# mprib/caliscope

Hardware: NVIDIA H100
Metric: lm_iterations_per_sec (higher is better)
Workload: dtype f64

## Files before the change

caliscope_b200/_lib.py:

```python
from __future__ import annotations

import ctypes as C
import os
from pathlib import Path

PKG_DIR = Path(__file__).resolve().parent
LIB_NAME = "libcaliscope_b200.so"

CB_CAM_FREE_INTRINSICS = 1
CB_CAM_FISHEYE = 2
LOSS_IDS = {"linear": 0, "soft_l1": 1, "huber": 2, "cauchy": 3, "arctan": 4}


class EngineUnavailable(RuntimeError):
    """libcaliscope_b200.so is missing / unloadable, or no CUDA device is usable."""


class EngineError(RuntimeError):
    def __init__(self, code: int, what: str, detail: str):
        super().__init__(f"{what} failed: {detail} (code {code})")
        self.code = code


class ProblemDesc(C.Structure):
    _fields_ = [
        ("n_cams", C.c_int32),
        ("n_pts", C.c_int32),
        ("n_obs", C.c_int64),
        ("cam_flags", C.c_void_p),
        ("cam_const", C.c_void_p),
        ("obs_cam", C.c_void_p),
        ("obs_pt", C.c_void_p),
        ("obs_xy", C.c_void_p),
        ("obs_on_device", C.c_int32),
        ("obs_cam_bits", C.c_int32),
        ("cam_order", C.c_void_p),
        ("n_constraints", C.c_int64),
        ("groups_a", C.c_void_p),
        ("groups_b", C.c_void_p),
        ("distances", C.c_void_p),
        ("weights", C.c_void_p),
    ]


ALLREDUCE_FN = C.CFUNCTYPE(C.c_int, C.c_void_p, C.c_void_p, C.c_int64, C.c_void_p)


class Options(C.Structure):
    _fields_ = [
        ("ftol", C.c_double),
        ("xtol", C.c_double),
        ("gtol", C.c_double),
        ("max_nfev", C.c_int64),
        ("loss", C.c_int32),
        ("f_scale", C.c_double),
        ("verbose", C.c_int32),
        ("use_bounds", C.c_int32),
        ("lambda0", C.c_double),
        ("pcg_tol", C.c_double),
        ("pcg_max_iter", C.c_int32),
        ("allreduce", ALLREDUCE_FN),
        ("allreduce_user", C.c_void_p),
        ("nccl_comm", C.c_void_p),
        ("peer_group", C.c_void_p),
        ("rank", C.c_int32),
        ("world_size", C.c_int32),
        ("time_kernels", C.c_int32),
        ("pad_", C.c_int32),
    ]


class Result(C.Structure):
    _fields_ = [
        ("status", C.c_int32),
        ("nfev", C.c_int64),
        ("njev", C.c_int64),
        ("nit", C.c_int64),
        ("cost", C.c_double),
        ("initial_cost", C.c_double),
        ("optimality", C.c_double),
        ("lambda_final", C.c_double),
        ("pcg_iterations", C.c_int64),
        ("kernel_launches", C.c_int64),
        ("solve_ms", C.c_double),
        ("rj_ms", C.c_double),
        ("rj_launches", C.c_int64),
        ("syrk_ms", C.c_double),
        ("syrk_launches", C.c_int64),
        ("trials_queued", C.c_int64),
        ("used_graph", C.c_int32),
        ("pad_", C.c_int32),
    ]


class TriStats(C.Structure):
    _fields_ = [
        ("group_ms", C.c_double),
        ("dlt_ms", C.c_double),
        ("total_ms", C.c_double),
        ("kernel_launches", C.c_int32),
        ("pad_", C.c_int32),
    ]


class TriRefineStats(C.Structure):
    _fields_ = [
        ("group_ms", C.c_double),
        ("dlt_ms", C.c_double),
        ("refine_ms", C.c_double),
        ("cov_ms", C.c_double),
        ("total_ms", C.c_double),
        ("kernel_launches", C.c_int32),
        ("pad_", C.c_int32),
    ]


class TriRobustStats(C.Structure):
    _fields_ = [
        ("group_ms", C.c_double),
        ("consensus_ms", C.c_double),
        ("refine_ms", C.c_double),
        ("cov_ms", C.c_double),
        ("total_ms", C.c_double),
        ("kernel_launches", C.c_int32),
        ("pad_", C.c_int32),
    ]


class ResectStats(C.Structure):
    _fields_ = [
        ("group_ms", C.c_double),
        ("consensus_ms", C.c_double),
        ("refine_ms", C.c_double),
        ("cov_ms", C.c_double),
        ("total_ms", C.c_double),
        ("kernel_launches", C.c_int32),
        ("pad_", C.c_int32),
    ]


_P = C.c_void_p
_D = C.POINTER(C.c_double)
SYMBOLS = {
    "cb_ba_abi_version": (C.c_int, []),
    "cb_ba_error_string": (C.c_char_p, [C.c_int]),
    "cb_ba_last_error": (C.c_char_p, []),
    "cb_ba_default_options": (None, [C.POINTER(Options)]),
    "cb_ba_problem_create": (C.c_int, [C.POINTER(ProblemDesc), C.c_int, _P, C.POINTER(_P)]),
    "cb_ba_problem_destroy": (C.c_int, [_P]),
    "cb_ba_problem_n_params": (C.c_int64, [_P]),
    "cb_ba_problem_stat": (C.c_double, [_P, C.c_int]),
    "cb_ba_constraint_rows": (C.c_int, [_P, _P, _P, _P, _P]),
    "cb_ba_solve": (C.c_int, [_P, C.POINTER(Options), _P, C.POINTER(Result), _P]),
    "cb_ba_residuals": (C.c_int, [_P, _P, _P, _P]),
    "cb_ba_jacobian_blocks": (C.c_int, [_P, _P, _P, _P, _P]),
    "cb_ba_reproj_errors_px": (C.c_int, [_P, _P, _P, _P]),
    "cb_ba_cam_stride": (C.c_int, [_P]),
    "cb_ba_normal_equations": (
        C.c_int,
        [_P, _P, C.c_double, C.c_int32, C.c_double, _P, _P, _P, _P, _P, _P, _P, _P, _P, _P],
    ),
    "cb_ba_covariance": (
        C.c_int,
        [_P, _P, C.c_int32, C.c_double, C.c_int32, _P, C.c_double, _P, _P, _P, _P, _P, _P],
    ),
    "cb_ba_error_order_stats": (C.c_int, [_P, _P, C.c_double, _P, _P, _P, _P, _P]),
    "cb_ba_rmse_px": (C.c_int, [_P, _P, _P, _P, _P]),
    "cb_ba_cull": (C.c_int, [_P, _P, _P, C.c_int32, C.POINTER(_P), _P, _P, _P]),
    "cb_ba_debug_pcg_time": (C.c_int, [_P, C.c_int, C.c_int, _P, _P]),
    "cb_debug_fp64_peak": (C.c_int, [C.c_int, _P, _P]),
    "cb_shard_select": (C.c_int, [C.c_int64, _P, _P, _P, C.c_int32, C.c_int32, C.c_int64, _P, _P, _P, _P, _P, C.c_int32]),
    "cb_csv_write_numeric": (C.c_int, [C.c_char_p, C.c_char_p, C.c_int64, C.c_int32, _P, _P, C.c_int32]),
    "cb_csv_scan": (C.c_int, [C.c_char_p, _P, _P]),
    "cb_csv_parse_numeric": (C.c_int, [C.c_char_p, C.c_int64, C.c_int32, _P, _P, _P, C.c_int32]),
    "cb_pnp_ippe": (C.c_int, [C.c_int32, _P, _P, _P, C.c_int64, _P, _P, _P, _P, C.c_int32, C.c_int32, _P, _P, _P, _P, _P, _P, _P,
                              _P, C.c_int, _P]),
    "cb_stereo_rmse": (C.c_int, [C.c_int32, _P, _P, _P, C.c_int32, _P, _P, _P, C.c_int64, _P, _P, _P, C.c_int32, _P, _P, _P,
                                 C.c_int, _P]),
    "cb_relative_pose_network": (C.c_int, [C.c_int32, C.c_int32, _P, _P, _P, _P, _P, C.c_double, C.c_double, C.c_int32, _P, _P, _P, _P,
                                           _P, _P, C.c_int64, _P, _P, _P, C.c_int, _P]),
    "cb_undistort_points": (C.c_int, [C.c_int32, _P, _P, _P, C.c_int64, _P, _P, C.c_int, C.c_int, _P, C.c_int, _P]),
    "cb_triangulate_dlt": (
        C.c_int,
        [C.c_int32, _P, C.c_int64, _P, _P, _P, C.c_int, C.c_int32, C.POINTER(C.c_int32), _P, _P, _P, _P,
         C.POINTER(TriStats), C.c_int, _P],
    ),
    "cb_undistort_triangulate": (
        C.c_int,
        [C.c_int32, _P, _P, _P, _P, C.c_int64, _P, _P, _P, C.c_int, C.c_int32, C.POINTER(C.c_int32), _P, _P, _P, _P,
         C.POINTER(TriStats), C.c_int, _P],
    ),
    "cb_triangulate_refine": (
        C.c_int,
        [C.c_int32, _P, _P, _P, _P, C.c_int64, _P, _P, _P, C.c_int, C.c_double, C.c_int32, C.c_double, C.c_int32,
         C.POINTER(C.c_int32), _P, _P, _P, _P, _P, _P, C.POINTER(TriRefineStats), C.c_int, _P],
    ),
    "cb_triangulate_robust": (
        C.c_int,
        [C.c_int32, _P, _P, _P, _P, C.c_int64, _P, _P, _P, C.c_int, C.c_double, C.c_int32, C.c_int32, C.c_double,
         C.c_int32, C.c_double, C.c_int32, C.POINTER(C.c_int32), _P, _P, _P, _P, _P, _P, _P, _P,
         C.POINTER(TriRobustStats), C.c_int, _P],
    ),
    "cb_resect_robust": (
        C.c_int,
        [C.c_int32, _P, _P, _P, C.c_int32, _P, _P, C.c_int64, _P, _P, _P, _P, C.c_int, C.c_double, C.c_int32, C.c_int32,
         C.c_int32, C.c_double, C.c_int32, C.c_double, C.c_int32, C.POINTER(C.c_int32), _P, _P, _P, _P, _P, _P, _P, _P,
         _P, C.POINTER(ResectStats), C.c_int, _P],
    ),
    "cb_peer_create": (C.c_int, [C.c_int, C.c_int, C.c_int, C.c_int64, C.POINTER(_P), _P]),
    "cb_peer_connect": (C.c_int, [_P, _P]),
    "cb_peer_destroy": (C.c_int, [_P]),
    "cb_nccl_unique_id": (C.c_int, [_P]),
    "cb_nccl_comm_create": (C.c_int, [_P, C.c_int, C.c_int, C.c_int, C.POINTER(_P)]),
    "cb_nccl_comm_destroy": (C.c_int, [_P]),
    "cb_ba_launch_count": (C.c_int64, []),
}

_lib = None


def lib_path() -> Path:
    return Path(os.environ.get("CALISCOPE_B200_LIB", PKG_DIR / LIB_NAME))


def load() -> C.CDLL:
    global _lib
    if _lib is not None:
        return _lib
    path = lib_path()
    if not path.exists():
        raise EngineUnavailable(
            f"{path} not found -- build it with `python -c 'import __graft_entry__ as g; g.build()'` "
            "(nvcc, sm_90a).  caliscope_b200 has no CPU fallback."
        )
    try:
        lib = C.CDLL(str(path))
    except OSError as e:
        raise EngineUnavailable(f"cannot load {path}: {e}") from e
    for name, (res, args) in SYMBOLS.items():
        fn = getattr(lib, name)
        fn.restype = res
        fn.argtypes = args
    _lib = lib
    return lib


def check(code: int, what: str) -> None:
    if code == 0:
        return
    lib = load()
    detail = (lib.cb_ba_last_error() or b"").decode() or (lib.cb_ba_error_string(code) or b"").decode()
    if code == -3:
        raise EngineUnavailable(f"{what}: {detail}")
    raise EngineError(code, what, detail)
```

caliscope_b200/csrc/cb_engine.cu:

```cuda
#include <cuda_runtime.h>
#include <dlfcn.h>
#if defined(__x86_64__)
#include <emmintrin.h>
#endif
#include <nvtx3/nvToolsExt.h>

#include <algorithm>
#include <atomic>
#include <chrono>
#include <cmath>
#include <cstdio>
#include <cstdlib>
#include <cstring>
#include <condition_variable>
#include <cub/cub.cuh>
#include <deque>
#include <functional>
#include <map>
#include <memory>
#include <mutex>
#include <string>
#include <thread>
#include <type_traits>
#include <vector>
// ... 314 lines not shown
      std::lock_guard<std::mutex> lk(mu_);
      q_.push_back(std::move(f));
    }
    cv_.notify_one();
  }

 private:
  WorkerPool() {
    unsigned hw = std::thread::hardware_concurrency();
    int n = (int)std::min<unsigned>(hw > 2 ? hw - 1 : 1, 12u);
    for (int i = 0; i < n; ++i) {
      threads_.emplace_back([this] {
        for (;;) {
          std::function<void()> f;
          {
            std::unique_lock<std::mutex> lk(mu_);
            cv_.wait(lk, [this] { return !q_.empty(); });
            f = std::move(q_.front());
            q_.pop_front();
          }
          f();
        }
      });
      threads_.back().detach();
    }
  }
  std::mutex mu_;
  std::condition_variable cv_;
  std::deque<std::function<void()>> q_;
  std::vector<std::thread> threads_;
};

int staged_h2d(void* d_dst, const void* h_src, size_t bytes, cudaStream_t st, ScopedFree& sf, int n_threads = 6) {
  if (bytes == 0) return CB_OK;
  char* pin = nullptr;
  CB_TRY(sf.alloc_pinned(&pin, bytes));
  const size_t unit = (size_t)512 << 10, units_per_block = 8;
  const size_t n_units = (bytes + unit - 1) / unit;
  const size_t n_blocks = (n_units + units_per_block - 1) / units_per_block;
  struct Shared {
    std::atomic<size_t> next{0};
    std::vector<std::atomic<unsigned char>> done;
    explicit Shared(size_t n) : done(n) { for (auto& d : done) d.store(0, std::memory_order_relaxed); }
  };
  auto sh = std::make_shared<Shared>(n_units);
  auto copy_one = [sh, pin, h_src, bytes, unit, n_units]() -> bool {
    const size_t c = sh->next.fetch_add(1);
    if (c >= n_units) return false;
    const size_t off = c * unit, sz = std::min(unit, bytes - off);
    stream_copy((char*)pin + off, (const char*)h_src + off, sz);
    sh->done[c].store(1, std::memory_order_release);
    return true;
  };
  static const bool prof = std::getenv("CB_PROFILE_CREATE") != nullptr;
  const auto t0 = std::chrono::steady_clock::now();
  const int helpers = (int)std::min<size_t>((size_t)std::max(0, std::min(n_threads, WorkerPool::get().size())), n_units > 1 ? n_units - 1 : 0);
  for (int t = 0; t < helpers; ++t)
    WorkerPool::get().submit([copy_one] { while (copy_one()) {} });
  bool failed = false;
  double wait_ms = 0.0, issue_ms = 0.0;
  size_t own = 0;
  cudaEvent_t pe0 = nullptr, pe1 = nullptr;
  if (prof) { cudaEventCreate(&pe0); cudaEventCreate(&pe1); cudaEventRecord(pe0, st); }
  for (size_t blk = 0; blk < n_blocks; ++blk) {
    const size_t u0 = blk * units_per_block, u1 = std::min(n_units, u0 + units_per_block);
    const auto a = std::chrono::steady_clock::now();
    for (size_t c = u0; c < u1; ++c)
      while (!sh->done[c].load(std::memory_order_acquire)) {
        if (copy_one()) ++own; else std::this_thread::yield();
      }
    const auto b = std::chrono::steady_clock::now();
    const size_t off = u0 * unit, sz = std::min(bytes, u1 * unit) - off;
    if (!failed && cudaMemcpyAsync((char*)d_dst + off, (char*)pin + off, sz, cudaMemcpyHostToDevice, st) != cudaSuccess) failed = true;
    if (prof) {
      const auto e = std::chrono::steady_clock::now();
      wait_ms += std::chrono::duration<double, std::milli>(b - a).count();
      issue_ms += std::chrono::duration<double, std::milli>(e - b).count();
    }
  }
  if (prof) {
    const double host_ms = std::chrono::duration<double, std::milli>(std::chrono::steady_clock::now() - t0).count();
    cudaEventRecord(pe1, st);
    cudaEventSynchronize(pe1);
    float dma_ms = 0.f;
    cudaEventElapsedTime(&dma_ms, pe0, pe1);
    const double all_ms = std::chrono::duration<double, std::milli>(std::chrono::steady_clock::now() - t0).count();
    cudaEventDestroy(pe0); cudaEventDestroy(pe1);
    std::fprintf(stderr, "[stage] %6.1f MB, %d helpers, %zu DMA blocks: host %.3f ms (units %.3f, %zu by the issuer; cudaMemcpyAsync calls %.3f); "
                         "device first->last copy %.3f ms = %.1f GB/s; staged + landed %.3f ms\n",
                 bytes / 1e6, helpers, n_blocks, host_ms, wait_ms, own, issue_ms, dma_ms, bytes / 1e6 / std::max(dma_ms, 1e-3f), all_ms);
  }
  if (failed) { g_last_error = std::string("staged host-to-device copy: ") + cudaGetErrorString(cudaGetLastError()); return CB_E_CUDA; }
  return CB_OK;
}

int select_device(int device) {
  int ndev = 0;
  if (cudaGetDeviceCount(&ndev) != cudaSuccess || ndev == 0) {
    cudaGetLastError();
    g_last_error = "no CUDA device";
    return CB_E_NO_DEVICE;
  }
  if (device < 0 || device >= ndev) { g_last_error = "device index out of range"; return CB_E_INVALID; }
  CB_CUDA(cudaSetDevice(device));
  return CB_OK;
}

}

struct TrialGraph {
  struct Key {
    void *nccl, *peer; int rank, world;
    bool operator==(const Key& o) const { return nccl == o.nccl && peer == o.peer && rank == o.rank && world == o.world; }
  };
  cudaGraph_t graph = nullptr;
  cudaGraphExec_t exec = nullptr;
  Key key = {};
  bool valid = false, failed = false;
  int n_kernels = 0;
};

struct CbBaProblem {
  int device = 0, num_sms = 132;
  int n_cams = 0, n_pts = 0, P = 6, nP = 0, n_obs = 0, n_params = 0;
  int LD = 0, n_blk = 0, n_tiles = 0, n_split = 1, k_chunks = 0, K_pad = 0;
  int n_chunks = 0, pt_grid = 0, pt_lanes = 32, n_dups = 0;
  int cam_in_smem = 0;
  size_t pt_smem = 0, bs_smem = 0;
  std::vector<int> h_cam_off;
  std::vector<int> h_perm, h_slot;
  std::vector<int> h_iflags;
  bool order_auto = false, order_identity = true;
  int ncp = 0;
  int *d_cam_xoff = nullptr, *d_cam_slot = nullptr, *d_klist = nullptr;
  bool schur_sparse = false;
  double schur_flop_issued = 0.0;
  std::vector<void*> allocs;
  int* d_cam_flags = nullptr;
  double* d_cam_const = nullptr;
  double2 *d_cm_xy = nullptr, *d_pm_xy = nullptr;
  int *d_cm_pt = nullptr, *d_cm_orig = nullptr, *d_cam_start = nullptr;
  int *d_chunk_cam = nullptr, *d_chunk_begin = nullptr, *d_chunk_end = nullptr, *d_cam_chunk_start = nullptr;
  int *d_pt_start = nullptr, *d_pm_orig = nullptr, *d_pm_cam = nullptr, *d_pm_pt = nullptr;
  const int *d_obs_cam = nullptr, *d_obs_pt = nullptr;
  const double* d_obs_xy = nullptr;
  std::vector<int> h_cam_flags;
  std::vector<double> h_cam_const;
  int *d_tile_of = nullptr, *d_tile_slot_start = nullptr, *d_tile_slots = nullptr;
  cb::SyItem* d_items = nullptr;
  int n_items = 0, n_slots = 0;
  CUtensorMap zt_map{};
  unsigned char* d_active = nullptr;
  double *d_lo = nullptr, *d_hi = nullptr;
  double *d_x = nullptr, *d_xc[2] = {nullptr, nullptr}, *d_xp4[2] = {nullptr, nullptr};
  double *d_camtab[2] = {nullptr, nullptr}, *d_Upk[2] = {nullptr, nullptr}, *d_gc[2] = {nullptr, nullptr},
         *d_costsum[2] = {nullptr, nullptr};
  double *d_partial = nullptr, *d_camcost = nullptr, *d_V6 = nullptr, *d_gp = nullptr, *d_Dp2 = nullptr,
         *d_Dc2 = nullptr, *d_Linv6 = nullptr, *d_tvec = nullptr, *d_Zt = nullptr, *d_part = nullptr,
         *d_tpart = nullptr, *d_red = nullptr, *d_Minv = nullptr, *d_dc = nullptr, *d_dp = nullptr,
         *d_bpart = nullptr, *d_sc = nullptr, *d_red2 = nullptr, *d_out2 = nullptr;
  unsigned long long* d_gmax = nullptr;
  unsigned int* d_counter = nullptr;
  cb::LmState* d_state = nullptr;
  cb::LmState* h_state = nullptr;
  cb::LmLogRow* d_log = nullptr;
  int log_cap = 4096;
  double* h_x = nullptr;
  cudaEvent_t ev0 = nullptr, ev1 = nullptr, ev2 = nullptr, ev3 = nullptr, ev_state[2] = {nullptr, nullptr};
  cudaEvent_t ev_pp[2][4] = {{nullptr, nullptr, nullptr, nullptr}, {nullptr, nullptr, nullptr, nullptr}};
  cudaStream_t cap_stream = nullptr;
  TrialGraph trial_graph;
  TrialGraph loop_graph;
  int pcg_cs = 1, pcg_rows = 0, pcg_mode = 2, pcg_cl = 1, pcg_npa = 0;
  bool direct_solve = false;
  size_t direct_smem = 0;
  size_t pcg_smem = 0;
  int n_c = 0, n_comp = 0, n_dim_max = 0, n_cblk = 0;
  cb::ConstraintTables ct = {};
  double *d_c_rs[2] = {nullptr, nullptr}, *d_c_dirw[2] = {nullptr, nullptr}, *d_compL = nullptr, *d_gpt = nullptr;
  int* d_pt_comp = nullptr;
  size_t comp_build_smem = 0, comp_back_smem = 0;
  std::vector<int> h_ga, h_gb;
  std::vector<double> h_cdist, h_cw;
  int red_slots = 64;
  CbPeerGroup* peer = nullptr;
  int cov_n = 0;
  double *d_covA = nullptr, *d_covC = nullptr, *d_covD = nullptr, *d_covS = nullptr, *d_covDiag = nullptr,
         *d_covR = nullptr, *d_covPt = nullptr;
  int *d_covRank = nullptr, *d_covFail = nullptr;
  unsigned char* d_covFree = nullptr;
  float cov_ms[3] = {0.f, 0.f, 0.f};
  size_t red_len() const { return (size_t)nP * nP + 3 * (size_t)nP + 1 + red_slots; }
  cb::CPtr2 c_camtab() const { return {{d_camtab[0], d_camtab[1]}}; }
  cb::Ptr2 m_camtab() const { return {{d_camtab[0], d_camtab[1]}}; }
  cb::CPtr2 c_xp() const { return {{d_xp4[0], d_xp4[1]}}; }
  cb::Ptr2 m_xp() const { return {{d_xp4[0], d_xp4[1]}}; }
  cb::Ptr2 m_xc() const { return {{d_xc[0], d_xc[1]}}; }
  cb::CPtr2 c_Upk() const { return {{d_Upk[0], d_Upk[1]}}; }
  cb::Ptr2 m_Upk() const { return {{d_Upk[0], d_Upk[1]}}; }
  cb::CPtr2 c_gc() const { return {{d_gc[0], d_gc[1]}}; }
  cb::Ptr2 m_gc() const { return {{d_gc[0], d_gc[1]}}; }
  cb::CPtr2 c_costsum() const { return {{d_costsum[0], d_costsum[1]}}; }
  cb::Ptr2 m_costsum() const { return {{d_costsum[0], d_costsum[1]}}; }
  cb::CPtr2 c_crs() const { return {{d_c_rs[0], d_c_rs[1]}}; }
  cb::Ptr2 m_crs() const { return {{d_c_rs[0], d_c_rs[1]}}; }
  cb::CPtr2 c_cdirw() const { return {{d_c_dirw[0], d_c_dirw[1]}}; }
  cb::Ptr2 m_cdirw() const { return {{d_c_dirw[0], d_c_dirw[1]}}; }
};

namespace {

template <typename T>
int palloc(CbBaProblem* p, T** ptr, size_t n) {
  CB_TRY(dalloc(ptr, n));
  p->allocs.push_back((void*)*ptr);
  return CB_OK;
}

int bits_for(unsigned long long v) {
  int b = 1;
  while (b < 64 && (v >> b) != 0ull) ++b;
  return b;
}

void destroy_graph(TrialGraph& g) {
  if (g.exec) cudaGraphExecDestroy(g.exec);
  if (g.graph) cudaGraphDestroy(g.graph);
  g.exec = nullptr; g.graph = nullptr; g.valid = false; g.n_kernels = 0;
}

cudaStream_t side_stream() {
  thread_local std::map<int, cudaStream_t> streams;
  int dev = 0;
  cudaGetDevice(&dev);
  auto it = streams.find(dev);
  if (it != streams.end()) return it->second;
  cudaStream_t s = nullptr;
  cudaStreamCreateWithFlags(&s, cudaStreamNonBlocking);
  streams[dev] = s;
  return s;
}

int choose_camera_order(CbBaProblem* p, const int* cam_order, cudaStream_t st) {
  const int nc = p->n_cams;
  p->h_perm.resize(nc); p->h_slot.resize(nc);
  for (int i = 0; i < nc; ++i) p->h_perm[i] = i;
  p->order_auto = false;
  if (cam_order) {
    std::vector<char> seen(nc, 0);
    for (int i = 0; i < nc; ++i) {
      const int c = cam_order[i];
      if (c < 0 || c >= nc || seen[c]) { g_last_error = "cam_order is not a permutation of 0..n_cams-1"; return CB_E_INVALID; }
      seen[c] = 1;
      p->h_perm[i] = c;
    }
  } else {
    const int cams_per_tile = std::max(1, cb::SY_TILE / p->P);
    const double avg = (double)p->n_obs / std::max(p->n_pts, 1);
    if (p->n_blk >= 3 && avg <= nc / 3.0) {
      p->order_auto = true;
      const int stride = std::max(1, p->n_pts / 8192), ns = cdiv(p->n_pts, stride);
      unsigned int* d_W;
      ScopedFree sf(st);
      CB_TRY(sf.alloc(&d_W, (size_t)nc * nc));
      CB_CUDA(cudaMemsetAsync(d_W, 0, sizeof(unsigned int) * nc * nc, st));
      CB_LAUNCH(cb::covis_kernel, cdiv((long long)ns * 32, 256), 256, 0, st, p->d_pt_start, p->d_pm_cam, p->n_pts, stride, nc, d_W);
      std::vector<unsigned int> W((size_t)nc * nc);
      CB_CUDA(cudaMemcpyAsync(W.data(), d_W, sizeof(unsigned int) * nc * nc, cudaMemcpyDeviceToHost, st));
      CB_CUDA(cudaStreamSynchronize(st));
      std::vector<char> placed(nc, 0);
      std::vector<int> order;
      int start = 0;
      unsigned long long best = ~0ull;
      for (int c = 0; c < nc; ++c) {
        unsigned long long tot = 0;
        for (int q = 0; q < nc; ++q) if (q != c) tot += W[(size_t)c * nc + q];
        if (tot < best) { best = tot; start = c; }
      }
      order.push_back(start); placed[start] = 1;
      while ((int)order.size() < nc) {
        int pick = -1;
        unsigned long long bw = 0;
        const int lo = std::max(0, (int)order.size() - cams_per_tile);
        for (int c = 0; c < nc; ++c) {
          if (placed[c]) continue;
          unsigned long long w = 0;
          for (int k = lo; k < (int)order.size(); ++k) w += W[(size_t)c * nc + order[k]];
          if (pick < 0 || w > bw) { pick = c; bw = w; }
        }
        order.push_back(pick); placed[pick] = 1;
      }
      auto off_mass = [&](const std::vector<int>& ord) {
        std::vector<int> tile(nc);
        for (int i = 0; i < nc; ++i) tile[ord[i]] = (i * p->P) / cb::SY_TILE;
        unsigned long long m = 0;
        for (int a = 0; a < nc; ++a)
          for (int b = 0; b < nc; ++b)
            if (tile[a] != tile[b]) m += W[(size_t)a * nc + b];
        return m;
      };
      std::vector<int> ident(nc);
      for (int i = 0; i < nc; ++i) ident[i] = i;
      if (off_mass(order) < 0.8 * off_mass(ident)) p->h_perm = order;
    }
  }
  p->order_identity = true;
  for (int i = 0; i < nc; ++i) {
    p->h_slot[p->h_perm[i]] = i;
    if (p->h_perm[i] != i) p->order_identity = false;
  }
  CB_CUDA(cudaMemcpyAsync(p->d_cam_slot, p->h_slot.data(), sizeof(int) * nc, cudaMemcpyHostToDevice, st));
  return CB_OK;
}

struct XyUpload {
  bool started = false;
  std::atomic<int> finished{0};
  cudaEvent_t ev = nullptr;
  int rc = CB_OK;
  std::string err;
  ScopedFree pinned;
  void join() {
    if (!started) return;
    while (!finished.load(std::memory_order_acquire)) std::this_thread::yield();
    started = false;
  }
  int wait(cudaStream_t st) {
    join();
    if (rc != CB_OK) { g_last_error = err; return rc; }
    if (ev) CB_CUDA(cudaStreamWaitEvent(st, ev, 0));
    return CB_OK;
  }
  ~XyUpload() {
    join();
    if (ev) { cudaEventSynchronize(ev); cudaEventDestroy(ev); }
  }
};

int build_indices(CbBaProblem* p, const int* d_obs_cam, const int* d_obs_pt, const double* d_obs_xy,
                  const int* cam_order, cudaStream_t st, XyUpload* xy_upload) {
  const int n = p->n_obs;
  const int TB = 256, G = cdiv(std::max(n, 1), TB);
  ScopedFree sf(st);
  int* d_bad;
// ... 87 lines not shown
            COV ? p->d_covRank : nullptr)
#define CB_PT_PASS2(LANES, DUPS) do { if (p->cam_in_smem) CB_PT_PASS(LANES, DUPS, true); else CB_PT_PASS(LANES, DUPS, false); } while (0)
  if (p->pt_lanes == 8) { if (p->n_dups) CB_PT_PASS2(8, true); else CB_PT_PASS2(8, false); }
  else { if (p->n_dups) CB_PT_PASS2(32, true); else CB_PT_PASS2(32, false); }
#undef CB_PT_PASS2
#undef CB_PT_PASS
}

template <int P>
void launch_pt_backsub(CbBaProblem* p, double* dp_out, cudaStream_t st) {
  const int bstride = p->pt_grid + p->n_comp;
#define CB_PT_BACK(LANES, SM)                                                                                         \
  CB_LAUNCH((cb::pt_backsub_kernel<P, LANES, SM>), p->pt_grid, cb::PT_WARPS * 32, p->bs_smem, st, p->d_state,         \
            p->d_pt_start, p->d_pm_cam, p->d_pm_xy, p->d_pt_comp, p->n_pts, p->n_cams, p->nP, p->c_camtab(),           \
            p->m_xp(), p->d_dc, p->d_Linv6, p->d_tvec, p->d_gp, p->d_Dp2, dp_out, p->d_bpart, bstride)
  if (p->pt_lanes == 8) { if (p->cam_in_smem) CB_PT_BACK(8, true); else CB_PT_BACK(8, false); }
  else { if (p->cam_in_smem) CB_PT_BACK(32, true); else CB_PT_BACK(32, false); }
#undef CB_PT_BACK
}

using PcgFn = void (*)(const cb::LmState*, const double*, const double*, const double*, int, int, int, double, int,
                       double*, double*);
PcgFn pcg_fn(int mode, int P, int cl) {
  if (mode == 2) {
    if (P == 6)
      return cl == 2 ? cb::pcg_cluster_kernel<2, 6, 2> : cl == 6 ? cb::pcg_cluster_kernel<2, 6, 6>
           : cl == 12 ? cb::pcg_cluster_kernel<2, 6, 12> : cb::pcg_cluster_kernel<2, 6, 18>;
    return cl == 2 ? cb::pcg_cluster_kernel<2, 9, 2> : cl == 6 ? cb::pcg_cluster_kernel<2, 9, 6>
         : cl == 12 ? cb::pcg_cluster_kernel<2, 9, 12> : cb::pcg_cluster_kernel<2, 9, 18>;
  }
  return P == 6 ? cb::pcg_cluster_kernel<1, 6, 1> : cb::pcg_cluster_kernel<1, 9, 1>;
}

int launch_pcg(CbBaProblem* p, const cb::LmState* st_dev, double tol2, int max_iter, cudaStream_t st) {
  cudaLaunchConfig_t cfg = {};
  cfg.gridDim = dim3(p->pcg_cs);
  cfg.blockDim = dim3(cb::PCG_THREADS);
  cfg.dynamicSmemBytes = p->pcg_smem;
  cfg.stream = st;
  cudaLaunchAttribute at[1];
  at[0].id = cudaLaunchAttributeClusterDimension;
  at[0].val.clusterDim.x = p->pcg_cs;
  at[0].val.clusterDim.y = 1;
  at[0].val.clusterDim.z = 1;
  cfg.attrs = at;
  cfg.numAttrs = 1;
  const double* S = p->d_red;
  const double* b = p->d_red + (size_t)p->nP * p->nP;
  auto fn = pcg_fn(p->pcg_mode, p->P, p->pcg_cl);
  CB_CUDA(cudaLaunchKernelEx(&cfg, fn, st_dev, S, b, (const double*)p->d_Minv, p->nP, p->pcg_npa, p->pcg_rows, tol2,
                             max_iter, p->d_dc, p->d_sc));
  g_launches.fetch_add(1);
  return CB_OK;
}

template <int P>
int camera_pass(CbBaProblem* p, int flip, int mode, cudaStream_t st) {
  const int loss = 0;
  const double fscale = 1.0;
  launch_resjac<P, 0>(p, p->d_state, flip, loss, fscale, nullptr, st);
  if (p->n_c)
    CB_LAUNCH((cb::constraint_eval_kernel<false>), p->n_cblk, cb::CC_THREADS, 0, st, (const cb::LmState*)p->d_state, flip,
              p->ct, p->c_xp(), loss, fscale, p->m_crs(), p->m_cdirw(), (double*)nullptr, p->d_camcost + p->n_cams);
  CB_LAUNCH((cb::trial_reduce_kernel<P>), p->n_cams + 1, 64, 0, st, p->d_state, mode, p->n_cams, p->d_cam_chunk_start,
            p->d_partial, p->m_Upk(), p->m_gc(), p->m_costsum(), p->d_camcost, p->n_cblk, p->d_bpart,
            p->pt_grid + p->n_comp, p->pt_grid + p->n_comp, p->d_red2, p->d_counter, p->d_sc, p->d_log);
  return CB_OK;
}

template <int P>
int build_system(CbBaProblem* p, const CbBaOptions* opt, cudaStream_t st, const cudaEvent_t* ev = nullptr, bool cov = false) {
  if (ev) CB_CUDA(cudaEventRecord(ev[0], st));
  if (cov) launch_pt_pass<P, true>(p, st);
  else launch_pt_pass<P>(p, st);
  if (ev) CB_CUDA(cudaEventRecord(ev[1], st));
  if (p->n_c)
    CB_LAUNCH((cb::comp_build_kernel<P>), p->n_comp, cb::CC_THREADS, p->comp_build_smem, st, (const cb::LmState*)p->d_state,
              p->ct, p->d_pt_start, p->d_pm_cam, p->d_V6, p->d_gp, p->d_Dp2, p->d_gpt, p->c_crs(), p->c_cdirw(), p->n_cams,
              p->d_compL, p->d_tvec, p->d_Zt, (size_t)p->LD, p->d_gmax);
  if (ev) CB_CUDA(cudaEventRecord(ev[2], st));
  CB_LAUNCH(cb::schur_syrk_kernel, p->n_items, cb::SY_THREADS, sizeof(cb::SyrkSmem), st, p->zt_map,
            (const cb::LmState*)p->d_state, p->d_Zt, (size_t)p->LD, p->d_tvec, p->d_items, (const int*)p->d_klist,
            p->d_part, p->d_tpart);
  if (ev) CB_CUDA(cudaEventRecord(ev[3], st));
  const size_t nfin = (size_t)p->nP * p->nP + p->nP + 1;
  const int rank = sharded(opt) ? std::min(std::max(opt->rank, 0), p->red_slots - 1) : 0;
  if (opt && opt->peer_group) {
    CbPeerGroup* g = (CbPeerGroup*)opt->peer_group;
    int nb = 0;
    CB_CUDA(cudaOccupancyMaxActiveBlocksPerMultiprocessor(&nb, cb::schur_finalize_peer_kernel<P>, cb::PEER_THREADS, 0));
    const int grid = std::max(1, std::min(nb, 2)) * p->num_sms;
    const cb::LmState* sd = p->d_state;
    int nP = p->nP, n_blk = p->n_blk, red_slots = p->red_slots, rk = rank;
    cb::CPtr2 upk = p->c_Upk(), gc = p->c_gc(), cs = p->c_costsum();
    const double* gmax = (const double*)p->d_gmax;
    void* args[] = {&sd, &nP, &n_blk, &p->d_tile_of, &p->d_tile_slot_start, &p->d_tile_slots, &p->d_part, &p->d_tpart,
                    &upk, &gc, &cs, &gmax, &red_slots, &rk, &g->tab, &p->d_red};
    CB_CUDA(cudaLaunchCooperativeKernel((const void*)cb::schur_finalize_peer_kernel<P>, dim3(grid), dim3(cb::PEER_THREADS),
                                        args, 0, st));
    g_launches.fetch_add(1);
  } else {
    CB_LAUNCH((cb::schur_finalize_kernel<P>), cdiv((long long)std::max<size_t>(nfin, p->red_slots), 256), 256, 0, st,
              (const cb::LmState*)p->d_state, p->nP, p->n_blk, p->d_tile_of, p->d_tile_slot_start, p->d_tile_slots,
              p->d_part, p->d_tpart, p->c_Upk(), p->c_gc(), p->c_costsum(), (const double*)p->d_gmax, p->red_slots, rank,
              p->d_red);
    if (sharded(opt)) CB_TRY(do_allreduce(opt, p->d_red, (long long)p->red_len(), st));
  }
  if (!p->direct_solve && !cov)
    CB_LAUNCH((cb::reduced_prep_kernel<P>), 1, 256, 0, st, p->d_state, p->nP, p->n_cams, p->red_slots, p->d_red, p->d_Dc2,
              p->d_active, p->d_Minv, p->d_gmax, p->d_sc);
  return CB_OK;
}

template <int P>
int solve_step(CbBaProblem* p, double* dp_out, cudaStream_t st) {
  const size_t nn = (size_t)p->nP * p->nP;
  if (p->direct_solve) {
    CB_LAUNCH((cb::small_rig_step_kernel<P>), 1, cb::DIRECT_THREADS, p->direct_smem, st, p->d_state, p->nP, p->n_cams,
              p->red_slots, p->d_red, p->d_Dc2, p->d_active, p->d_gmax, p->d_sc, p->m_xc(), p->d_dc, p->d_lo, p->d_hi,
              p->d_cam_flags, p->d_cam_const, p->m_camtab());
  } else {
    CB_TRY(launch_pcg(p, p->d_state, 0.0, 0, st));
    CB_LAUNCH(cb::cam_step_kernel, 1, 256, 0, st, (const cb::LmState*)p->d_state, p->nP, p->n_cams, p->P, p->m_xc(), p->d_dc,
              p->d_lo, p->d_hi, p->d_red + nn + p->nP, p->d_Dc2, p->d_active, p->d_cam_flags, p->d_cam_const, p->m_camtab(),
              p->d_sc);
  }
  launch_pt_backsub<P>(p, dp_out, st);
  if (p->n_c)
    CB_LAUNCH(cb::comp_backsub_kernel, p->n_comp, cb::CC_THREADS, p->comp_back_smem, st, (const cb::LmState*)p->d_state,
              p->ct, p->nP, p->d_Zt, (size_t)p->LD, p->d_dc, p->d_compL, p->d_tvec, p->d_gpt, p->d_Dp2, p->m_xp(), dp_out,
              p->d_bpart, p->pt_grid + p->n_comp, p->pt_grid);
  return CB_OK;
}

template <int P>
int enqueue_trial(CbBaProblem* p, const CbBaOptions* opt, cudaStream_t st, const cudaEvent_t* ev = nullptr) {
  CB_TRY(build_system<P>(p, opt, st, ev));
  CB_TRY(solve_step<P>(p, nullptr, st));
  const bool multi = sharded(opt);
  CB_TRY(camera_pass<P>(p, 1, multi ? 2 : 1, st));
  if (multi) {
    cb::PeerTable none = {};
    if (opt->peer_group) {
      CB_LAUNCH(cb::lm_decide_kernel, 1, 32, 0, st, p->d_state, (const double*)p->d_sc, p->d_red2, p->d_log,
                ((CbPeerGroup*)opt->peer_group)->tab, 1);
    } else {
      CB_TRY(do_allreduce(opt, p->d_red2, 4, st));
      CB_LAUNCH(cb::lm_decide_kernel, 1, 32, 0, st, p->d_state, (const double*)p->d_sc, p->d_red2, p->d_log, none, 0);
    }
  }
  return CB_OK;
}

int upload_x(CbBaProblem* p, const double* x, cudaStream_t st) {
  stream_copy(p->h_x, x, sizeof(double) * p->n_params);
  CB_CUDA(cudaMemcpyAsync(p->d_x, p->h_x, sizeof(double) * p->n_params, cudaMemcpyHostToDevice, st));
  const int n = std::max(p->n_cams * p->P, p->n_pts);
  CB_LAUNCH(cb::unpack_x_kernel, cdiv(std::max(n, 1), 256), 256, 0, st, p->d_x, p->d_cam_xoff, p->d_cam_flags,
            p->d_cam_const, p->n_cams, p->P, p->n_pts, p->ncp, p->d_xc[0], p->d_xp4[0]);
  return CB_OK;
}

int download_x(CbBaProblem* p, int cur, double* x, cudaStream_t st) {
  const int n = std::max(p->n_cams * p->P, p->n_pts);
  CB_LAUNCH(cb::pack_x_kernel, cdiv(std::max(n, 1), 256), 256, 0, st, p->d_x, p->d_cam_xoff, p->d_cam_flags, p->n_cams,
            p->P, p->n_pts, p->ncp, p->d_xc[cur], p->d_xp4[cur]);
  CB_CUDA(cudaMemcpyAsync(p->h_x, p->d_x, sizeof(double) * p->n_params, cudaMemcpyDeviceToHost, st));
  CB_CUDA(cudaStreamSynchronize(st));
  std::memcpy(x, p->h_x, sizeof(double) * p->n_params);
  return CB_OK;
}

int set_bounds(CbBaProblem* p, bool use_bounds, cudaStream_t st) {
  std::vector<double> lo((size_t)p->nP, -1e300), hi((size_t)p->nP, 1e300);
  if (use_bounds && p->P == 9) {
    for (int c = 0; c < p->n_cams; ++c)
      if (p->h_iflags[c] & CB_CAM_FREE_INTRINSICS) {
        lo[c * 9 + 6] = 0.5; hi[c * 9 + 6] = 2.0;
        lo[c * 9 + 7] = -1.0; hi[c * 9 + 7] = 1.0;
        lo[c * 9 + 8] = -2.0; hi[c * 9 + 8] = 2.0;
      }
  }
  CB_CUDA(cudaMemcpyAsync(p->d_lo, lo.data(), sizeof(double) * p->nP, cudaMemcpyHostToDevice, st));
  CB_CUDA(cudaMemcpyAsync(p->d_hi, hi.data(), sizeof(double) * p->nP, cudaMemcpyHostToDevice, st));
  CB_CUDA(cudaStreamSynchronize(st));
  return CB_OK;
}

int init_state(CbBaProblem* p, const CbBaOptions* opt, double lam, long long max_nfev, cudaStream_t st) {
  cb::LmState& h = p->h_state[3];
  std::memset(&h, 0, sizeof(h));
  h.lam = lam; h.nu = 2.0;
  h.ftol = opt->ftol; h.xtol = opt->xtol; h.gtol = opt->gtol;
  h.nfev = 1; h.njev = 1; h.nit = 0; h.max_nfev = max_nfev;
  h.new_lin = 1;
  h.log_cap = p->log_cap;
  h.loss = opt->loss;
  h.fscale = opt->f_scale > 0 ? opt->f_scale : 1.0;
  const double tol = opt->pcg_tol > 0 ? opt->pcg_tol : 1e-6;
  h.pcg_tol2 = tol * tol;
  h.pcg_max_iter = opt->pcg_max_iter > 0 ? opt->pcg_max_iter : 4 * p->nP;
  if (opt->peer_group) {
    CbPeerGroup* g = (CbPeerGroup*)opt->peer_group;
    h.epoch_big = g->epoch_big; h.epoch_small = g->epoch_small;
  }
  CB_CUDA(cudaMemcpyAsync(p->d_state, &h, sizeof(h), cudaMemcpyHostToDevice, st));
  CB_CUDA(cudaMemsetAsync(p->d_gmax, 0, 2 * sizeof(unsigned long long), st));
  CB_CUDA(cudaMemsetAsync(p->d_counter, 0, 4 * sizeof(unsigned int), st));
  CB_CUDA(cudaMemsetAsync(p->d_sc, 0, sizeof(double) * cb::SC_COUNT, st));
  CB_CUDA(cudaMemsetAsync(p->d_Dc2, 0, sizeof(double) * p->nP, st));
  CB_CUDA(cudaMemsetAsync(p->d_Dp2, 0, sizeof(double) * 3 * (size_t)std::max(p->n_pts, 1), st));
  return CB_OK;
}

template <int P>
int ensure_graph(CbBaProblem* p, const CbBaOptions* opt, bool loop) {
  TrialGraph& g = loop ? p->loop_graph : p->trial_graph;
  const TrialGraph::Key key{opt->nccl_comm, opt->peer_group, opt->rank, opt->world_size};
  if (g.key == key && (g.valid || g.failed)) return g.valid ? CB_OK : CB_E_UNSUPPORTED;
  destroy_graph(g);
  g.key = key;
  g.failed = false;
  auto fail = [&](const char* what) {
    g_last_error = std::string(loop ? "device-loop graph: " : "trial graph: ") + what + ": " +
                   cudaGetErrorString(cudaGetLastError());
    destroy_graph(g);
    g.failed = true;
    return CB_E_UNSUPPORTED;
  };
  if (!p->cap_stream && cudaStreamCreateWithFlags(&p->cap_stream, cudaStreamNonBlocking) != cudaSuccess)
    return fail("cudaStreamCreateWithFlags");
  cudaGraphConditionalHandle h = {};
  cudaError_t e;
  if (loop) {
    if (cudaGraphCreate(&g.graph, 0) != cudaSuccess) return fail("cudaGraphCreate");
    if (cudaGraphConditionalHandleCreate(&h, g.graph, 1, cudaGraphCondAssignDefault) != cudaSuccess)
      return fail("cudaGraphConditionalHandleCreate");
    cudaGraphNodeParams np = {};
    np.type = cudaGraphNodeTypeConditional;
    np.conditional.handle = h;
    np.conditional.type = cudaGraphCondTypeWhile;
    np.conditional.size = 1;
    cudaGraphNode_t node;
    if (cudaGraphAddNode(&node, g.graph, nullptr, 0, &np) != cudaSuccess) return fail("cudaGraphAddNode(conditional)");
    e = cudaStreamBeginCaptureToGraph(p->cap_stream, np.conditional.phGraph_out[0], nullptr, nullptr, 0,
                                      cudaStreamCaptureModeThreadLocal);
  } else {
    e = cudaStreamBeginCapture(p->cap_stream, cudaStreamCaptureModeThreadLocal);
  }
  if (e != cudaSuccess) return fail("begin capture");
  const long long l0 = g_launches.load();
  int rc = enqueue_trial<P>(p, opt, p->cap_stream);
  if (loop && rc == CB_OK) CB_LAUNCH(cb::lm_loop_cond_kernel, 1, 1, 0, p->cap_stream, (const cb::LmState*)p->d_state, h);
  g.n_kernels = (int)(g_launches.load() - l0);
  g_launches.store(l0);
  e = loop ? cudaStreamEndCapture(p->cap_stream, nullptr) : cudaStreamEndCapture(p->cap_stream, &g.graph);
  if (rc != CB_OK || e != cudaSuccess) return fail("capture of the trial");
  if (cudaGraphInstantiate(&g.exec, g.graph, 0) != cudaSuccess) return fail("cudaGraphInstantiate");
  g.valid = true;
  return CB_OK;
}

template <int P>
int lm_solve(CbBaProblem* p, const CbBaOptions* opt, double* x_inout, CbBaResult* res, cudaStream_t st) {
  NvtxRange nvtx_solve("cb_ba_solve");
  const long long max_nfev = opt->max_nfev > 0 ? opt->max_nfev : 100ll * p->n_params;
  const bool verbose = opt->verbose >= 2 && opt->rank == 0;
  const long long launches0 = g_launches.load();
  std::memset(res, 0, sizeof(*res));

  const bool direct = opt->allreduce != nullptr || opt->time_kernels;
  bool use_loop = !direct && !sharded(opt);
  if (use_loop && ensure_graph<P>(p, opt, true) != CB_OK) { cudaGetLastError(); use_loop = false; }
  bool use_graph = !direct && !use_loop;
  if (use_graph && ensure_graph<P>(p, opt, false) != CB_OK) { cudaGetLastError(); use_graph = false; }

  CB_TRY(set_bounds(p, opt->use_bounds != 0, st));
  CB_TRY(init_state(p, opt, opt->lambda0 > 0 ? opt->lambda0 : 1e-4, max_nfev, st));
  CB_TRY(upload_x(p, x_inout, st));
  CB_CUDA(cudaEventRecord(p->ev0, st));
  CB_TRY(run_cam_prep<P>(p, p->d_xc[0], p->d_camtab[0], st));
  CB_TRY(camera_pass<P>(p, 0, 0, st));

  double pp_ms_total = 0.0;
  long long pp_launches = 0, trials = 0;
  double sy_ms_total = 0.0;
  long long sy_launches = 0;
  auto read_pp = [&](long long t) {
    float ms = 0.f;
    const cudaEvent_t* ev = p->ev_pp[t & 1];
    if (cudaEventElapsedTime(&ms, ev[0], ev[1]) == cudaSuccess) { pp_ms_total += ms; ++pp_launches; }
    else cudaGetLastError();
    if (cudaEventElapsedTime(&ms, ev[2], ev[3]) == cudaSuccess) { sy_ms_total += ms; ++sy_launches; }
    else cudaGetLastError();
  };
  bool done = false;
  long long t = 0;
  int rc = CB_OK;
  if (use_loop) {
    cudaError_t e = cudaGraphLaunch(p->loop_graph.exec, st);
    if (e != cudaSuccess) {
      cudaGetLastError();
      p->loop_graph.failed = true;
      p->loop_graph.valid = false;
      use_loop = false;
    } else {
      cudaMemcpyAsync(&p->h_state[1], p->d_state, sizeof(cb::LmState), cudaMemcpyDeviceToHost, st);
      t = 2;
      done = true;
    }
  }
  while (!done) {
    if (use_graph) {
      cudaError_t e = cudaGraphLaunch(p->trial_graph.exec, st);
      if (e != cudaSuccess) { g_last_error = std::string("cudaGraphLaunch: ") + cudaGetErrorString(e); rc = CB_E_CUDA; break; }
      g_launches.fetch_add(p->trial_graph.n_kernels);
    } else {
      NvtxRange nvtx_trial("lm_trial (direct launches)");
      rc = enqueue_trial<P>(p, opt, st, p->ev_pp[t & 1]);
      if (rc != CB_OK) break;
    }
    cudaMemcpyAsync(&p->h_state[t & 1], p->d_state, sizeof(cb::LmState), cudaMemcpyDeviceToHost, st);
    cudaEventRecord(p->ev_state[t & 1], st);
    ++trials;
    if (t >= 1) {
      cudaError_t e = cudaEventSynchronize(p->ev_state[(t - 1) & 1]);
      if (e != cudaSuccess) { g_last_error = std::string("LM trial: ") + cudaGetErrorString(e); rc = CB_E_CUDA; break; }
      if (!use_graph) read_pp(t - 1);
      if (p->h_state[(t - 1) & 1].done) done = true;
    }
    ++t;
  }
  cudaError_t e = cudaStreamSynchronize(st);
  if (rc == CB_OK && e != cudaSuccess) { g_last_error = std::string("LM solve: ") + cudaGetErrorString(e); rc = CB_E_CUDA; }
  if (rc != CB_OK) { if (p->peer) p->peer->poisoned = true; return rc; }
  const cb::LmState fin = p->h_state[(t - 1) & 1];
  if (p->peer) {
    int peer_err = 0;
    CB_CUDA(cudaMemcpy(&peer_err, p->peer->tab.err, sizeof(int), cudaMemcpyDeviceToHost));
    p->peer->epoch_big = fin.epoch_big;
    p->peer->epoch_small = fin.epoch_small;
    if (peer_err) {
      p->peer->poisoned = true;
      g_last_error = "peer all-reduce timed out waiting for another rank";
      return CB_E_CALLBACK;
    }
  }
  if (fin.err == cb::LM_ERR_NONFINITE_X0) {
    g_last_error = "Residuals are not finite in the initial point.";
    return CB_E_INVALID;
  }
  if (verbose) {
    const int nl = std::min(fin.n_log, p->log_cap);
    std::vector<cb::LmLogRow> rows((size_t)std::max(nl, 1));
    if (nl) CB_CUDA(cudaMemcpy(rows.data(), p->d_log, sizeof(cb::LmLogRow) * nl, cudaMemcpyDeviceToHost));
    std::fprintf(stderr, "%5s %5s %22s %22s %9s %10s %10s %10s %5s\n", "nit", "nfev", "cost", "cost_new", "ratio", "lambda",
                 "|step|", "|g|inf", "pcg");
    for (int i = 0; i < nl; ++i)
      std::fprintf(stderr, "%5lld %5lld %22.15e %22.15e %+9.3f %10.2e %10.2e %10.2e %5d\n", (long long)rows[i].nit,
                   (long long)rows[i].nfev, rows[i].cost, rows[i].cost_new, rows[i].ratio, rows[i].lam, rows[i].step,
                   rows[i].gnorm, (int)rows[i].pcg);
  }
  CB_CUDA(cudaEventRecord(p->ev1, st));
  CB_TRY(download_x(p, fin.cur, x_inout, st));
  float ms = 0.f;
  CB_CUDA(cudaEventElapsedTime(&ms, p->ev0, p->ev1));
  res->status = fin.status;
  res->nfev = fin.nfev;
  res->njev = fin.njev;
  res->nit = fin.nit;
  res->cost = fin.cost;
  res->initial_cost = fin.initial_cost;
  res->optimality = fin.gnorm;
  res->lambda_final = fin.lam;
  res->pcg_iterations = fin.pcg_total;
  res->kernel_launches = g_launches.load() - launches0;
  res->solve_ms = ms;
  res->rj_ms = pp_ms_total;
  res->rj_launches = pp_launches;
  res->syrk_ms = sy_ms_total;
  res->syrk_launches = sy_launches;
  if (use_loop) {
    trials = fin.nfev - 1 + ((fin.status == 1 || fin.err) ? 1 : 0);
    g_launches.fetch_add((long long)p->loop_graph.n_kernels * trials);
    res->kernel_launches = g_launches.load() - launches0;
  }
  res->trials_queued = trials;
  res->used_graph = use_loop ? 2 : use_graph ? 1 : 0;
  if (fin.err == cb::LM_ERR_STUCK_NONFINITE)
    g_last_error = "every trial step is non-finite with the damping at its cap; stopped with status 0";
  if (opt->verbose >= 1 && opt->rank == 0)
    std::fprintf(stderr,
                 "[caliscope_b200] status %d nfev %lld njev %lld nit %lld cost %.15e -> %.15e |g| %.2e  %.3f ms (%lld trials queued, %s)\n",
                 fin.status, (long long)fin.nfev, (long long)fin.njev, (long long)fin.nit, fin.initial_cost, fin.cost,
                 fin.gnorm, ms, trials, use_loop ? "device loop" : use_graph ? "graph" : "direct");
  return CB_OK;
}

int choose_pcg_config(CbBaProblem* p) {
  const int nP = p->nP, P = p->P;
  int max_optin = 0;
  cudaDeviceGetAttribute(&max_optin, cudaDevAttrMaxSharedMemoryPerBlockOptin, p->device);
  const size_t budget = (size_t)std::max(max_optin, 48 * 1024);
  const size_t minv = (((size_t)(nP / P) * P * P + 7) & ~(size_t)7);
  const int nw = cb::PCG_THREADS / 32;
  auto try_config = [&](int mode, int cs, int cl) -> bool {
    const int rows = (nP + cs - 1) / cs;
    const int npa = std::max((nP + 7) & ~7, mode == 2 ? cl * 32 : 0);
    const size_t smem = (9 * (size_t)npa + 2 * nw + 2 * 16 * nw + minv) * sizeof(double);
    if (smem > budget) return false;
    if (mode == 2 && rows > 3 * nw) return false;
    const void* fn = (const void*)pcg_fn(mode, P, cl);
    cudaFuncSetAttribute(fn, cudaFuncAttributeNonPortableClusterSizeAllowed, 1);
    if (cudaFuncSetAttribute(fn, cudaFuncAttributeMaxDynamicSharedMemorySize, (int)smem) != cudaSuccess) {
      cudaGetLastError();
      return false;
    }
    cudaLaunchConfig_t cfg = {};
    cfg.gridDim = dim3(cs);
    cfg.blockDim = dim3(cb::PCG_THREADS);
    cfg.dynamicSmemBytes = smem;
    cudaLaunchAttribute at[1];
    at[0].id = cudaLaunchAttributeClusterDimension;
    at[0].val.clusterDim.x = cs; at[0].val.clusterDim.y = 1; at[0].val.clusterDim.z = 1;
    cfg.attrs = at;
    cfg.numAttrs = 1;
    int ncl = 0;
    if (cudaOccupancyMaxActiveClusters(&ncl, fn, &cfg) != cudaSuccess || ncl < 1) {
      cudaGetLastError();
      return false;
    }
    p->pcg_cs = cs; p->pcg_rows = rows; p->pcg_mode = mode; p->pcg_cl = cl; p->pcg_npa = npa; p->pcg_smem = smem;
    return true;
  };
  p->direct_solve = false;
  if (nP <= cb::DIRECT_MAX_N) {
    const size_t smem = ((size_t)(nP + 1) * (nP | 1) + nP) * sizeof(double);
    const void* fn = P == 6 ? (const void*)cb::small_rig_step_kernel<6> : (const void*)cb::small_rig_step_kernel<9>;
    if (smem <= budget && cudaFuncSetAttribute(fn, cudaFuncAttributeMaxDynamicSharedMemorySize, (int)smem) == cudaSuccess) {
      p->direct_solve = true;
      p->direct_smem = smem;
    } else {
      cudaGetLastError();
    }
  }
  if (nP <= 576) {
    const int cl = nP <= 64 ? 2 : nP <= 192 ? 6 : nP <= 384 ? 12 : 18;
    const int cs = (nP + 3 * nw - 1) / (3 * nw);
    if (cs <= 16 && try_config(2, cs, cl)) return CB_OK;
  }
  if (try_config(1, 8, 1)) return CB_OK;
  g_last_error = "no feasible PCG cluster configuration for n_camera_params = " + std::to_string(nP);
  return CB_E_UNSUPPORTED;
}

}

extern "C" {

int cb_ba_abi_version(void) { return CB_BA_ABI_VERSION; }

const char* cb_ba_error_string(int code) {
  switch (code) {
    case CB_OK: return "ok";
    case CB_E_INVALID: return "invalid argument";
    case CB_E_CUDA: return "CUDA runtime error";
    case CB_E_NO_DEVICE: return "no CUDA device";
    case CB_E_UNSUPPORTED: return "unsupported configuration";
    case CB_E_CALLBACK: return "all-reduce callback failed";
    case CB_E_NOMEM: return "out of device memory";
    default: return "unknown error";
  }
}

const char* cb_ba_last_error(void) { return g_last_error.c_str(); }

void cb_ba_default_options(CbBaOptions* o) {
  if (!o) return;
  std::memset(o, 0, sizeof(*o));
  o->ftol = 1e-8; o->xtol = 1e-8; o->gtol = 1e-8;
  o->max_nfev = 0;
  o->loss = CB_LOSS_LINEAR;
  o->f_scale = 1.0;
  o->verbose = 0;
  o->use_bounds = 1;
  o->lambda0 = 1e-4;
  o->pcg_tol = 1e-6;
  o->pcg_max_iter = 0;
  o->allreduce = nullptr;
  o->allreduce_user = nullptr;
  o->nccl_comm = nullptr;
  o->peer_group = nullptr;
  o->rank = 0;
  o->world_size = 1;
  o->time_kernels = 0;
}

int64_t cb_ba_launch_count(void) { return (int64_t)g_launches.load(); }

int cb_peer_create(int rank, int world_size, int device, int64_t capacity_doubles, CbPeerGroup** out,
                   char handle_out[64]) {
  static_assert(sizeof(cudaIpcMemHandle_t) == 64, "IPC handle size");
  if (!out || !handle_out || rank < 0 || rank >= world_size || world_size > cb::PEER_MAXW || capacity_doubles <= 0) {
    g_last_error = "cb_peer_create: bad argument (world_size <= 16)";
    return CB_E_INVALID;
  }
  int ndev = 0;
  if (cudaGetDeviceCount(&ndev) != cudaSuccess || ndev == 0) { cudaGetLastError(); g_last_error = "no CUDA device"; return CB_E_NO_DEVICE; }
  CB_CUDA(cudaSetDevice(device));
  auto* g = new CbPeerGroup();
  g->rank = rank; g->world = world_size; g->device = device;
  g->cap = ((size_t)capacity_doubles + 31) / 32 * 32;
  g->bytes = cb::PEER_OFF_DATA + 2 * g->cap * sizeof(double);
  cudaError_t e = cudaMalloc(&g->base, g->bytes);
  if (e != cudaSuccess) { g_last_error = std::string("cudaMalloc: ") + cudaGetErrorString(e); delete g; return CB_E_NOMEM; }
  e = cudaMemset(g->base, 0, g->bytes);
  if (e == cudaSuccess) e = cudaDeviceSynchronize();
  cudaIpcMemHandle_t h;
  if (e == cudaSuccess) e = cudaIpcGetMemHandle(&h, g->base);
  if (e != cudaSuccess) {
    g_last_error = std::string("cb_peer_create: ") + cudaGetErrorString(e);
    cudaFree(g->base);
    delete g;
    return CB_E_CUDA;
  }
  std::memcpy(handle_out, &h, 64);
  *out = g;
  return CB_OK;
}

int cb_peer_connect(CbPeerGroup* g, const char* handles) {
  if (!g || !handles) { g_last_error = "cb_peer_connect: null argument"; return CB_E_INVALID; }
  if (g->connected) return CB_OK;
  CB_CUDA(cudaSetDevice(g->device));
  for (int r = 0; r < g->world; ++r) {
    if (r == g->rank) { g->peer_base[r] = g->base; continue; }
    cudaIpcMemHandle_t h;
    std::memcpy(&h, handles + 64 * (size_t)r, 64);
    cudaError_t e = cudaIpcOpenMemHandle(&g->peer_base[r], h, cudaIpcMemLazyEnablePeerAccess);
    if (e != cudaSuccess) {
      g_last_error = "cudaIpcOpenMemHandle(rank " + std::to_string(r) + "): " + cudaGetErrorString(e);
      cudaGetLastError();
      for (int q = 0; q < r; ++q)
        if (q != g->rank && g->peer_base[q]) { cudaIpcCloseMemHandle(g->peer_base[q]); g->peer_base[q] = nullptr; }
      return CB_E_UNSUPPORTED;
    }
  }
  cb::PeerTable& t = g->tab;
  t.rank = g->rank; t.world = g->world;
  for (int r = 0; r < g->world; ++r) {
    char* b = (char*)g->peer_base[r];
    t.data[r][0] = (const double*)(b + cb::PEER_OFF_DATA);
    t.data[r][1] = (const double*)(b + cb::PEER_OFF_DATA) + g->cap;
    t.flags_big_of[r] = (unsigned long long*)(b + cb::PEER_OFF_FLAGS_BIG);
    t.flags_small_of[r] = (unsigned long long*)(b + cb::PEER_OFF_FLAGS_SMALL);
    t.small_of[r] = (double*)(b + cb::PEER_OFF_SMALL);
  }
  char* mine = (char*)g->base;
  t.my_data[0] = (double*)(mine + cb::PEER_OFF_DATA);
  t.my_data[1] = (double*)(mine + cb::PEER_OFF_DATA) + g->cap;
  t.my_flags_big = (unsigned long long*)(mine + cb::PEER_OFF_FLAGS_BIG);
  t.my_flags_small = (unsigned long long*)(mine + cb::PEER_OFF_FLAGS_SMALL);
  t.my_small = (double*)(mine + cb::PEER_OFF_SMALL);
  t.done = (unsigned int*)(mine + cb::PEER_OFF_DONE);
  t.err = (int*)(mine + cb::PEER_OFF_ERR);
  g->connected = true;
  return CB_OK;
}

int cb_peer_destroy(CbPeerGroup* g) {
  if (!g) return CB_OK;
  cudaSetDevice(g->device);
  cudaDeviceSynchronize();
  if (g->connected)
    for (int r = 0; r < g->world; ++r)
      if (r != g->rank && g->peer_base[r]) cudaIpcCloseMemHandle(g->peer_base[r]);
  if (g->base) cudaFree(g->base);
  cudaGetLastError();
  delete g;
  return CB_OK;
}

int cb_nccl_unique_id(char id_out[128]) {
  NcclApi& a = nccl();
  if (!a.ok) { g_last_error = a.err; return CB_E_UNSUPPORTED; }
  UidBlob u;
  const int rc = a.GetUniqueId(&u);
  if (rc != 0) { g_last_error = "ncclGetUniqueId failed"; return CB_E_CALLBACK; }
  std::memcpy(id_out, u.internal, 128);
  return CB_OK;
}

int cb_nccl_comm_create(const char id[128], int rank, int world_size, int device, void** comm_out) {
  if (!id || !comm_out || rank < 0 || rank >= world_size) { g_last_error = "cb_nccl_comm_create: bad argument"; return CB_E_INVALID; }
  NcclApi& a = nccl();
  if (!a.ok) { g_last_error = a.err; return CB_E_UNSUPPORTED; }
  CB_CUDA(cudaSetDevice(device));
  UidBlob u;
  std::memcpy(u.internal, id, 128);
  void* comm = nullptr;
  const int rc = a.CommInitRank(&comm, world_size, u, rank);
  if (rc != 0) {
    g_last_error = std::string("ncclCommInitRank: ") + (a.GetErrorString ? a.GetErrorString(rc) : "error");
    return CB_E_CALLBACK;
  }
  *comm_out = comm;
  return CB_OK;
}

int cb_nccl_comm_destroy(void* comm) {
  if (!comm) return CB_OK;
  NcclApi& a = nccl();
  if (!a.ok) return CB_E_UNSUPPORTED;
  return a.CommDestroy(comm) == 0 ? CB_OK : CB_E_CALLBACK;
}

int cb_ba_problem_destroy(CbBaProblem* p) {
  if (!p) return CB_OK;
  cudaSetDevice(p->device);
  destroy_graph(p->trial_graph);
  destroy_graph(p->loop_graph);
  if (p->cap_stream) cudaStreamDestroy(p->cap_stream);
  for (void* a : p->allocs) cached_free(a);
  cached_free_host(p->h_state);
  cached_free_host(p->h_x);
  for (cudaEvent_t e : {p->ev0, p->ev1, p->ev2, p->ev3, p->ev_state[0], p->ev_state[1], p->ev_pp[0][0], p->ev_pp[0][1],
                        p->ev_pp[0][2], p->ev_pp[0][3], p->ev_pp[1][0], p->ev_pp[1][1], p->ev_pp[1][2], p->ev_pp[1][3]})
    if (e) cudaEventDestroy(e);
  delete p;
  return CB_OK;
}

int64_t cb_ba_problem_n_params(const CbBaProblem* p) { return p ? p->n_params : -1; }
int cb_ba_cam_stride(const CbBaProblem* p) { return p ? p->P : -1; }
double cb_ba_problem_stat(const CbBaProblem* p, int what) {
  if (!p) return -1.0;
  switch (what) {
    case 0: return p->schur_sparse ? 1.0 : 0.0;
    case 1: return p->schur_flop_issued;
    case 2: return p->direct_solve ? 1.0 : 0.0;
    case 3: return (double)p->n_items;
    case 4: case 5: case 6: return (double)p->cov_ms[what - 4];
    case 7: return (double)p->pt_lanes;
    case 8: return p->n_dups ? 1.0 : 0.0;
    case 9: return (double)p->cam_in_smem;
    case 10: return p->direct_solve ? 0.0 : (double)p->pcg_mode;
    case 11: return (double)p->pcg_cs;
    case 12: return p->pcg_mode == 2 ? (double)p->pcg_cl : 0.0;
    case 13: return p->order_identity ? 0.0 : 1.0;
    default: return -1.0;
  }
}

static int build_schur_items(CbBaProblem* p, cudaStream_t st) {
  const int nb = p->n_blk;
  std::vector<int> tof((size_t)nb * nb, -1);
  int nt = 0;
  for (int I = 0; I < nb; ++I)
    for (int J = I; J < nb; ++J) tof[(size_t)I * nb + J] = nt++;
  const double w_pair = 2.07;
  const double w_single = 1.46;
  const double w_list_single = 1.04;

  std::vector<long long> pair_koff, pair_cnt;
  bool sparse = false;
  int want_sparse = -1;
  if (const char* ev = std::getenv("CB_SY_SPARSE")) want_sparse = std::atoi(ev);
  if (nb >= 2 && nb <= 64 && p->n_pts > 0 && want_sparse != 0) {
    unsigned long long* d_mask;
    ScopedFree sf(st);
    CB_TRY(sf.alloc(&d_mask, (size_t)p->n_pts));
    CB_LAUNCH(cb::pt_tile_mask_kernel, cdiv(p->n_pts, 256), 256, 0, st, p->d_pt_start, p->d_pm_cam, p->n_pts, p->P, d_mask);
    if (p->n_comp)
      CB_LAUNCH(cb::comp_tile_mask_kernel, cdiv(p->n_comp, 256), 256, 0, st, p->ct.comp_pt_start, p->ct.comp_pts, p->n_comp,
                d_mask);
    unsigned long long* d_cnt;
    CB_TRY(sf.alloc(&d_cnt, (size_t)nt));
    CB_CUDA(cudaMemsetAsync(d_cnt, 0, sizeof(unsigned long long) * nt, st));
    CB_LAUNCH(cb::tile_pair_count_kernel, cdiv(p->n_pts, 256), 256, sizeof(unsigned) * nt, st, d_mask, p->n_pts, nb, d_cnt);
    std::vector<unsigned long long> cnt_u((size_t)nt);
    CB_CUDA(cudaMemcpyAsync(cnt_u.data(), d_cnt, sizeof(unsigned long long) * nt, cudaMemcpyDeviceToHost, st));
    CB_CUDA(cudaStreamSynchronize(st));
    std::vector<long long> cnt(cnt_u.begin(), cnt_u.end());
    double listed = 0.0, dense = 0.0;
    for (int I = 0; I < nb; ++I)
      for (int J = I; J < nb; ++J) {
        const double w = (I == J) ? w_list_single : 1.0;
        listed += w * (double)cnt[tof[(size_t)I * nb + J]];
        dense += w * (double)p->n_pts;
      }
    sparse = want_sparse == 1 || listed < 0.7 * dense;
    if (sparse) {
      const int zero_row = p->K_pad;
      std::vector<long long> pair_start((size_t)nt + 1, 0), koff_h((size_t)nt, -1);
      long long klen = 0;
      for (int t = 0; t < nt; ++t) {
        pair_start[(size_t)t + 1] = pair_start[(size_t)t] + cnt[(size_t)t];
        if (cnt[(size_t)t] == 0) continue;
        koff_h[(size_t)t] = klen;
        klen += cdiv(3 * cnt[(size_t)t], (long long)cb::SY_KC) * cb::SY_KC;
      }
      const long long n_inc = pair_start[(size_t)nt];
      if (klen > 0x7fffffffLL || n_inc > 0x7fffffffLL) { g_last_error = "Schur row lists exceed 2^31 entries"; return CB_E_UNSUPPORTED; }
      pair_koff.assign(koff_h.begin(), koff_h.end());
      pair_cnt.assign(cnt.begin(), cnt.end());
      int *d_ninc = nullptr, *d_incoff = nullptr;
      unsigned long long *d_keys = nullptr, *d_keys_s = nullptr;
      long long *d_pair_start = nullptr, *d_koff = nullptr;
      CB_TRY(sf.alloc(&d_ninc, (size_t)p->n_pts + 1));
      CB_TRY(sf.alloc(&d_incoff, (size_t)p->n_pts + 1));
      CB_TRY(sf.alloc(&d_keys, (size_t)n_inc));
      CB_TRY(sf.alloc(&d_keys_s, (size_t)n_inc));
      CB_TRY(sf.alloc(&d_pair_start, (size_t)nt + 1));
      CB_TRY(sf.alloc(&d_koff, (size_t)nt));
      CB_TRY(palloc(p, &p->d_klist, (size_t)klen));
      CB_CUDA(cudaMemsetAsync(d_ninc + p->n_pts, 0, sizeof(int), st));
      CB_LAUNCH(cb::inc_count_kernel, cdiv(p->n_pts, 256), 256, 0, st, (const unsigned long long*)d_mask, p->n_pts, d_ninc);
      const int key_bits = bits_for((unsigned long long)nt * (unsigned long long)p->n_pts);
      CB_CUB(sf, cub::DeviceScan::ExclusiveSum, d_ninc, d_incoff, p->n_pts + 1, st);
      CB_LAUNCH(cb::inc_emit_kernel, cdiv(p->n_pts, 256), 256, 0, st, (const unsigned long long*)d_mask, (const int*)d_incoff,
                p->n_pts, nb, d_keys);
      CB_CUB(sf, cub::DeviceRadixSort::SortKeys, d_keys, d_keys_s, (int)n_inc, 0, key_bits, st);
      g_launches.fetch_add(5);
      CB_CUDA(cudaMemcpyAsync(d_pair_start, pair_start.data(), sizeof(long long) * pair_start.size(), cudaMemcpyHostToDevice, st));
      CB_CUDA(cudaMemcpyAsync(d_koff, koff_h.data(), sizeof(long long) * koff_h.size(), cudaMemcpyHostToDevice, st));
      CB_LAUNCH(cb::fill_int_kernel, cdiv(klen, 256), 256, 0, st, p->d_klist, klen, zero_row);
      CB_LAUNCH(cb::klist_expand_kernel, cdiv(n_inc, 256), 256, 0, st, (const unsigned long long*)d_keys_s, n_inc, p->n_pts,
                (const long long*)d_pair_start, (const long long*)d_koff, p->d_klist);
      CB_CUDA(cudaStreamSynchronize(st));
    }
  }
  p->schur_sparse = sparse;

  struct Group { int kind, I, J; double w; int chunks; int koff; };
  std::vector<Group> groups;
  if (!sparse) {
    for (int I = 0; I < nb; ++I)
      for (int J = I + 1; J < nb; ++J) groups.push_back({0, I, J, 1.0, p->k_chunks, -1});
    for (int I = 0; I < nb; I += 2) {
      if (I + 1 < nb) groups.push_back({1, I, I + 1, w_pair, p->k_chunks, -1});
      else groups.push_back({1, I, -1, w_single, p->k_chunks, -1});
    }
  } else {
    for (int I = 0; I < nb; ++I)
      for (int J = I; J < nb; ++J) {
        const int t = tof[(size_t)I * nb + J];
        if (pair_cnt[(size_t)t] == 0) continue;
        const int koff = (int)pair_koff[(size_t)t];
        const int chunks = (int)cdiv(3 * pair_cnt[(size_t)t], (long long)cb::SY_KC);
        if (I == J) groups.push_back({1, I, -1, w_list_single, chunks, koff});
        else groups.push_back({0, I, J, 1.0, chunks, koff});
      }
  }
  double W = 0.0;
  for (auto& g : groups) W += g.w * g.chunks;
  p->schur_flop_issued = 0.0;
  for (auto& g : groups) {
    const double cols2 = g.kind == 0 ? 96.0 * 96.0 : (g.J >= 0 ? 2.0 : 1.0) * 42.0 * 16.0 * 8.0;
    p->schur_flop_issued += 2.0 * cols2 * (double)g.chunks * cb::SY_KC;
  }
  std::vector<cb::SyItem> items;
  std::vector<std::vector<int>> slots_of(nt);
  int slot = 0;
  constexpr int SY_MIN_CHUNKS = 8;
  auto cap_of = [&](const Group& g) { return std::max(1, g.chunks / SY_MIN_CHUNKS); };
  std::vector<int> n_of(groups.size(), 1);
  {
    int used = 0;
    for (size_t gi = 0; gi < groups.size(); ++gi) {
      const Group& g = groups[gi];
      int n = (int)std::floor(p->num_sms * (g.w * g.chunks) / std::max(W, 1.0));
      n_of[gi] = std::max(1, std::min(n, cap_of(g)));
      used += n_of[gi];
    }
    while (used < p->num_sms) {
      int best = -1;
      double load = 0.0;
      for (size_t gi = 0; gi < groups.size(); ++gi) {
        if (n_of[gi] >= cap_of(groups[gi])) continue;
        const double l = groups[gi].w * groups[gi].chunks / n_of[gi];
        if (l > load) { load = l; best = (int)gi; }
      }
      if (best < 0) break;
      ++n_of[(size_t)best];
      ++used;
    }
  }
  for (size_t gi = 0; gi < groups.size(); ++gi) {
    const Group& g = groups[gi];
    const int n = n_of[gi];
    for (int s2 = 0; s2 < n; ++s2) {
      cb::SyItem it;
      it.kind = g.kind; it.I = g.I; it.J = g.J; it.koff = g.koff;
      it.c0 = (int)(((long long)g.chunks * s2) / n);
      it.c1 = (int)(((long long)g.chunks * (s2 + 1)) / n);
      it.slotA = slot++;
      it.slotB = -1;
      if (g.kind == 0) {
        slots_of[tof[(size_t)g.I * nb + g.J]].push_back(it.slotA);
      } else {
        slots_of[tof[(size_t)g.I * nb + g.I]].push_back(it.slotA);
        if (g.J >= 0) {
// ... 161 lines not shown
  bool any_free = false;
  for (int c = 0; c < p->n_cams; ++c) {
    const int f = d->cam_flags[c];
    if ((f & CB_CAM_FREE_INTRINSICS) && (f & CB_CAM_FISHEYE)) {
      g_last_error = "fisheye cameras cannot have free intrinsics (bundle_parameterization.py:76-94)";
      return CB_E_INVALID;
    }
    any_free = any_free || (f & CB_CAM_FREE_INTRINSICS);
    p->h_cam_off[c + 1] = p->h_cam_off[c] + ((f & CB_CAM_FREE_INTRINSICS) ? 9 : 6);
    if (!(d->cam_const[c * 9] != 0.0)) { g_last_error = "fx_initial must be non-zero"; return CB_E_INVALID; }
  }
  p->P = any_free ? 9 : 6;
  p->nP = p->n_cams * p->P;
  p->ncp = p->h_cam_off[p->n_cams];
  p->n_params = p->ncp + 3 * p->n_pts;
  p->n_blk = cdiv(p->nP, cb::SY_TILE);
  p->LD = p->n_blk * cb::SY_TILE;
  p->n_tiles = p->n_blk * (p->n_blk + 1) / 2;
  p->K_pad = cdiv(3ll * std::max(p->n_pts, 1), cb::SY_KC) * cb::SY_KC;
  p->k_chunks = p->K_pad / cb::SY_KC;
  p->n_split = std::max(1, std::min(p->k_chunks, p->num_sms / std::max(p->n_tiles, 1)));
  p->pt_lanes = ((double)p->n_obs / std::max(p->n_pts, 1) <= 96.0) ? 8 : 32;
  {
    const int per_block = cb::PT_WARPS * (32 / p->pt_lanes);
    p->pt_grid = std::max(1, std::min(cdiv(std::max(p->n_pts, 1), per_block), 2 * p->num_sms));
    const size_t tab_bytes = sizeof(double) * cb::CT_SMEM * (size_t)p->n_cams;
    p->cam_in_smem = tab_bytes <= 64 * 1024 ? 1 : 0;
    p->pt_smem = p->cam_in_smem ? tab_bytes : 0;
    p->bs_smem = sizeof(double) * (((size_t)p->nP + 3) & ~(size_t)3) + (p->cam_in_smem ? tab_bytes : 0);
  }

  const int n = p->n_obs;
  CB_TRY(palloc(p, &p->d_cam_xoff, p->n_cams)); CB_TRY(palloc(p, &p->d_cam_slot, p->n_cams));
  CB_TRY(palloc(p, &p->d_cam_flags, p->n_cams));
  CB_TRY(palloc(p, &p->d_cam_const, (size_t)p->n_cams * 9));
  CB_TRY(palloc(p, &p->d_cm_xy, n)); CB_TRY(palloc(p, &p->d_cm_pt, n)); CB_TRY(palloc(p, &p->d_pm_xy, n));
  CB_TRY(palloc(p, &p->d_cm_orig, n)); CB_TRY(palloc(p, &p->d_cam_start, p->n_cams + 1));
  CB_TRY(palloc(p, &p->d_cam_chunk_start, p->n_cams + 1));
  CB_TRY(palloc(p, &p->d_pt_start, p->n_pts + 1)); CB_TRY(palloc(p, &p->d_pm_orig, n));
  CB_TRY(palloc(p, &p->d_pm_cam, n));
  CB_TRY(palloc(p, &p->d_pm_pt, n));
  const int *d_cam = d->obs_cam, *d_pt = d->obs_pt;
  const double* d_xy = d->obs_xy;
  int *t_cam = nullptr, *t_pt = nullptr;
  double* t_xy = nullptr;
  ScopedFree stage(st);
  XyUpload xy_up;
  if (!d->obs_on_device) {
    CB_TRY(dalloc(&t_cam, n)); CB_TRY(dalloc(&t_pt, n)); CB_TRY(dalloc(&t_xy, 2 * (size_t)n));
    p->allocs.push_back(t_cam); p->allocs.push_back(t_pt); p->allocs.push_back(t_xy);
    CB_CUDA(cudaEventCreateWithFlags(&xy_up.ev, cudaEventDisableTiming));
    {
      cudaStream_t side = side_stream();
      const double* src = d->obs_xy;
      const size_t bytes = sizeof(double) * 2 * (size_t)n;
      const int dev = p->device;
      xy_up.started = true;
      WorkerPool::get().submit([&xy_up, t_xy, src, bytes, side, dev] {
        cudaSetDevice(dev);
        xy_up.rc = staged_h2d(t_xy, src, bytes, side, xy_up.pinned, 8);
        if (xy_up.rc == CB_OK && cudaEventRecord(xy_up.ev, side) != cudaSuccess) xy_up.rc = CB_E_CUDA;
        if (xy_up.rc != CB_OK) xy_up.err = "staged upload of obs_xy failed";
        xy_up.finished.store(1, std::memory_order_release);
      });
    }
    if (d->obs_cam_bits == 16) {
      short* t16 = nullptr;
      CB_TRY(stage.alloc(&t16, n));
      CB_TRY(staged_h2d(t16, d->obs_cam, sizeof(short) * (size_t)n, st, stage));
      CB_LAUNCH(cb::widen_i16_kernel, cdiv(n, 256), 256, 0, st, (const short*)t16, n, t_cam);
    } else {
      CB_TRY(staged_h2d(t_cam, d->obs_cam, sizeof(int) * (size_t)n, st, stage));
    }
    CB_TRY(staged_h2d(t_pt, d->obs_pt, sizeof(int) * (size_t)n, st, stage));
    d_cam = t_cam; d_pt = t_pt; d_xy = t_xy;
  } else if (d->obs_cam_bits == 16) {
    CB_TRY(dalloc(&t_cam, n));
    p->allocs.push_back(t_cam);
    CB_LAUNCH(cb::widen_i16_kernel, cdiv(n, 256), 256, 0, st, (const short*)d->obs_cam, n, t_cam);
    d_cam = t_cam;
  }
  p->d_obs_cam = d_cam; p->d_obs_pt = d_pt; p->d_obs_xy = d_xy;
  p->h_cam_flags.assign(d->cam_flags, d->cam_flags + p->n_cams);
  p->h_cam_const.assign(d->cam_const, d->cam_const + 9 * (size_t)p->n_cams);
  lap("alloc + staged upload");
  CB_TRY(build_indices(p, d_cam, d_pt, d_xy, d->cam_order, st, xy_up.started ? &xy_up : nullptr));
  if (!p->n_dups)
    p->pt_smem += p->P == 6 ? (p->pt_lanes == 8 ? cb::pt_stage_bytes<6, 8>() : cb::pt_stage_bytes<6, 32>())
                            : (p->pt_lanes == 8 ? cb::pt_stage_bytes<9, 8>() : cb::pt_stage_bytes<9, 32>());
  {
    std::vector<int> xoff(p->n_cams);
    std::vector<double> iconst((size_t)p->n_cams * 9);
    p->h_iflags.resize(p->n_cams);
    for (int i = 0; i < p->n_cams; ++i) {
      const int c = p->h_perm[i];
      xoff[i] = p->h_cam_off[c];
      p->h_iflags[i] = d->cam_flags[c];
      std::memcpy(&iconst[(size_t)i * 9], d->cam_const + (size_t)c * 9, 9 * sizeof(double));
    }
    CB_CUDA(cudaMemcpyAsync(p->d_cam_xoff, xoff.data(), sizeof(int) * p->n_cams, cudaMemcpyHostToDevice, st));
    CB_CUDA(cudaMemcpyAsync(p->d_cam_flags, p->h_iflags.data(), sizeof(int) * p->n_cams, cudaMemcpyHostToDevice, st));
    CB_CUDA(cudaMemcpyAsync(p->d_cam_const, iconst.data(), sizeof(double) * 9 * p->n_cams, cudaMemcpyHostToDevice, st));
    CB_CUDA(cudaStreamSynchronize(st));
  }

  lap("index build + camera tables");
  CB_TRY(build_components(p, d, st));
  CB_TRY(build_schur_items(p, st));
  lap("schur work items");
  std::vector<unsigned char> act((size_t)p->nP, 0);
  for (int c = 0; c < p->n_cams; ++c)
    for (int a = 0; a < ((p->h_iflags[c] & CB_CAM_FREE_INTRINSICS) ? 9 : 6); ++a) act[(size_t)c * p->P + a] = 1;
  CB_TRY(palloc(p, &p->d_active, p->nP));
  CB_CUDA(cudaMemcpyAsync(p->d_active, act.data(), p->nP, cudaMemcpyHostToDevice, st));
  CB_CUDA(cudaStreamSynchronize(st));
  CB_TRY(palloc(p, &p->d_lo, p->nP)); CB_TRY(palloc(p, &p->d_hi, p->nP));

  const int NACC = (p->P == 6) ? 28 : 55, NU = (p->P == 6) ? 21 : 45;
  const size_t npts = (size_t)std::max(p->n_pts, 1);
  CB_TRY(palloc(p, &p->d_x, (size_t)p->n_params + 1));
  for (int k = 0; k < 2; ++k) {
    CB_TRY(palloc(p, &p->d_xc[k], p->nP)); CB_TRY(palloc(p, &p->d_xp4[k], 4 * npts));
    CB_TRY(palloc(p, &p->d_camtab[k], (size_t)p->n_cams * cb::CT_SIZE));
    CB_TRY(palloc(p, &p->d_Upk[k], (size_t)p->n_cams * NU)); CB_TRY(palloc(p, &p->d_gc[k], p->nP));
    CB_TRY(palloc(p, &p->d_costsum[k], 4));
  }
  CB_TRY(palloc(p, &p->d_partial, (size_t)std::max(p->n_chunks, 1) * NACC + p->n_cblk));
  CB_TRY(palloc(p, &p->d_camcost, (size_t)p->n_cams + p->n_cblk));
  CB_TRY(palloc(p, &p->d_gpt, 3 * npts));
  CB_TRY(palloc(p, &p->d_V6, 6 * npts)); CB_TRY(palloc(p, &p->d_gp, 3 * npts)); CB_TRY(palloc(p, &p->d_Dp2, 3 * npts));
  CB_TRY(palloc(p, &p->d_Dc2, p->nP)); CB_TRY(palloc(p, &p->d_Linv6, 6 * npts));
  CB_TRY(palloc(p, &p->d_tvec, (size_t)p->K_pad + cb::SY_KC));
  CB_TRY(palloc(p, &p->d_Zt, ((size_t)p->K_pad + cb::SY_KC) * p->LD));
  CB_CUDA(cb::make_zt_tensor_map(&p->zt_map, p->d_Zt, (size_t)p->LD, (size_t)p->K_pad + cb::SY_KC));
  CB_TRY(palloc(p, &p->d_part, (size_t)p->n_slots * cb::SY_TILE * cb::SY_TILE));
  CB_TRY(palloc(p, &p->d_tpart, (size_t)p->n_slots * cb::SY_TILE));
  CB_TRY(palloc(p, &p->d_red, p->red_len()));
  CB_TRY(palloc(p, &p->d_Minv, (size_t)p->n_cams * p->P * p->P));
  CB_TRY(palloc(p, &p->d_dc, p->nP)); CB_TRY(palloc(p, &p->d_dp, 3 * npts));
  CB_TRY(palloc(p, &p->d_bpart, 3 * ((size_t)p->pt_grid + p->n_comp)));
  CB_TRY(palloc(p, &p->d_sc, cb::SC_COUNT)); CB_TRY(palloc(p, &p->d_red2, 8));
  CB_TRY(palloc(p, &p->d_gmax, 2));
  CB_TRY(palloc(p, &p->d_counter, 4));
  CB_TRY(palloc(p, &p->d_state, 1));
  CB_TRY(palloc(p, &p->d_log, (size_t)p->log_cap));
  CB_TRY(palloc(p, &p->d_out2, 2 * (size_t)std::max(n, 1)));
  CB_CUDA(cudaMemsetAsync(p->d_Zt, 0, sizeof(double) * ((size_t)p->K_pad + cb::SY_KC) * p->LD, st));
  CB_CUDA(cudaMemsetAsync(p->d_tvec, 0, sizeof(double) * ((size_t)p->K_pad + cb::SY_KC), st));
  CB_CUDA(cudaMemsetAsync(p->d_tpart, 0, sizeof(double) * (size_t)p->n_slots * cb::SY_TILE, st));
  CB_CUDA(cudaMemsetAsync(p->d_part, 0, sizeof(double) * (size_t)p->n_slots * cb::SY_TILE * cb::SY_TILE, st));
  CB_CUDA(cudaMemsetAsync(p->d_red2, 0, sizeof(double) * 8, st));
  CB_CUDA(cudaMemsetAsync(p->d_Linv6, 0, sizeof(double) * 6 * npts, st));
  CB_TRY(cached_malloc_host((void**)&p->h_state, sizeof(cb::LmState) * 4));
  CB_TRY(cached_malloc_host((void**)&p->h_x, sizeof(double) * ((size_t)p->n_params + 1)));
  for (cudaEvent_t* e : {&p->ev0, &p->ev1, &p->ev2, &p->ev3, &p->ev_pp[0][0], &p->ev_pp[0][1], &p->ev_pp[0][2], &p->ev_pp[0][3],
                         &p->ev_pp[1][0], &p->ev_pp[1][1], &p->ev_pp[1][2], &p->ev_pp[1][3]})
    CB_CUDA(cudaEventCreate(e));
  for (cudaEvent_t* e : {&p->ev_state[0], &p->ev_state[1]}) CB_CUDA(cudaEventCreateWithFlags(e, cudaEventDisableTiming));
  CB_CUDA(cudaFuncSetAttribute(cb::schur_syrk_kernel, cudaFuncAttributeMaxDynamicSharedMemorySize,
                               (int)sizeof(cb::SyrkSmem)));
  if (p->pt_smem > 48 * 1024 || p->bs_smem > 48 * 1024) {
    const int a = (int)p->pt_smem, b2 = (int)p->bs_smem;
#define CB_SMEM_ATTR(PP)                                                                                           \
    do {                                                                                                             \
      cudaFuncSetAttribute(cb::pt_pass_kernel<PP, 8, false, true>, cudaFuncAttributeMaxDynamicSharedMemorySize, a);  \
      cudaFuncSetAttribute(cb::pt_pass_kernel<PP, 8, true, true>, cudaFuncAttributeMaxDynamicSharedMemorySize, a);   \
      cudaFuncSetAttribute(cb::pt_pass_kernel<PP, 32, false, true>, cudaFuncAttributeMaxDynamicSharedMemorySize, a); \
      cudaFuncSetAttribute(cb::pt_pass_kernel<PP, 32, true, true>, cudaFuncAttributeMaxDynamicSharedMemorySize, a);  \
      cudaFuncSetAttribute(cb::pt_pass_kernel<PP, 8, false, true, true>, cudaFuncAttributeMaxDynamicSharedMemorySize, a); \
      cudaFuncSetAttribute(cb::pt_pass_kernel<PP, 8, true, true, true>, cudaFuncAttributeMaxDynamicSharedMemorySize, a); \
      cudaFuncSetAttribute(cb::pt_pass_kernel<PP, 32, false, true, true>, cudaFuncAttributeMaxDynamicSharedMemorySize, a); \
      cudaFuncSetAttribute(cb::pt_pass_kernel<PP, 32, true, true, true>, cudaFuncAttributeMaxDynamicSharedMemorySize, a); \
      cudaFuncSetAttribute(cb::pt_pass_kernel<PP, 8, false, false>, cudaFuncAttributeMaxDynamicSharedMemorySize, a); \
      cudaFuncSetAttribute(cb::pt_pass_kernel<PP, 8, true, false>, cudaFuncAttributeMaxDynamicSharedMemorySize, a);  \
      cudaFuncSetAttribute(cb::pt_pass_kernel<PP, 32, false, false>, cudaFuncAttributeMaxDynamicSharedMemorySize, a); \
      cudaFuncSetAttribute(cb::pt_pass_kernel<PP, 32, true, false>, cudaFuncAttributeMaxDynamicSharedMemorySize, a); \
      cudaFuncSetAttribute(cb::pt_pass_kernel<PP, 8, false, false, true>, cudaFuncAttributeMaxDynamicSharedMemorySize, a); \
      cudaFuncSetAttribute(cb::pt_pass_kernel<PP, 8, true, false, true>, cudaFuncAttributeMaxDynamicSharedMemorySize, a); \
      cudaFuncSetAttribute(cb::pt_pass_kernel<PP, 32, false, false, true>, cudaFuncAttributeMaxDynamicSharedMemorySize, a); \
      cudaFuncSetAttribute(cb::pt_pass_kernel<PP, 32, true, false, true>, cudaFuncAttributeMaxDynamicSharedMemorySize, a); \
      cudaFuncSetAttribute(cb::pt_backsub_kernel<PP, 8, true>, cudaFuncAttributeMaxDynamicSharedMemorySize, b2);     \
      cudaFuncSetAttribute(cb::pt_backsub_kernel<PP, 32, true>, cudaFuncAttributeMaxDynamicSharedMemorySize, b2);    \
      cudaFuncSetAttribute(cb::pt_backsub_kernel<PP, 8, false>, cudaFuncAttributeMaxDynamicSharedMemorySize, b2);    \
      cudaFuncSetAttribute(cb::pt_backsub_kernel<PP, 32, false>, cudaFuncAttributeMaxDynamicSharedMemorySize, b2);   \
    } while (0)
    if (p->P == 6) CB_SMEM_ATTR(6); else CB_SMEM_ATTR(9);
#undef CB_SMEM_ATTR
    CB_CUDA(cudaGetLastError());
  }
  lap("work buffers + memsets");
  CB_TRY(choose_pcg_config(p));
  CB_CUDA(cudaStreamSynchronize(st));
  lap("pcg config");
  return CB_OK;
}

int cb_ba_problem_create(const CbBaProblemDesc* d, int device, void* stream, CbBaProblem** out) {
  if (d && d->n_obs == 0) {
    g_last_error = "No image observations provided";
    return CB_E_INVALID;
  }
  if (d && d->obs_cam_bits != 0 && d->obs_cam_bits != 16 && d->obs_cam_bits != 32) {
    g_last_error = "obs_cam_bits must be 0, 16 or 32";
    return CB_E_INVALID;
  }
  if (!d || !out || d->n_cams <= 0 || d->n_pts <= 0 || d->n_obs < 0 || d->n_obs > (1ll << 30) || !d->cam_flags ||
      !d->cam_const || (d->n_obs > 0 && (!d->obs_cam || !d->obs_pt || !d->obs_xy)) || d->n_constraints < 0 ||
      (d->n_constraints > 0 && (!d->groups_a || !d->groups_b || !d->distances || !d->weights))) {
    g_last_error = "cb_ba_problem_create: bad descriptor";
    return CB_E_INVALID;
  }
  *out = nullptr;
  CbBaProblem* p = new CbBaProblem();
  int rc = problem_create_impl(d, device, (cudaStream_t)stream, p);
  if (rc != CB_OK) {
    std::string keep = g_last_error;
    cb_ba_problem_destroy(p);
    g_last_error = keep;
    return rc;
  }
  *out = p;
  return CB_OK;
}

int cb_ba_solve(CbBaProblem* p, const CbBaOptions* opt, double* x_inout, CbBaResult* result, void* stream) {
  if (!p || !opt || !x_inout || !result) { g_last_error = "cb_ba_solve: null argument"; return CB_E_INVALID; }
  if (opt->loss < 0 || opt->loss > CB_LOSS_ARCTAN) { g_last_error = "unknown loss id"; return CB_E_INVALID; }
  CB_CUDA(cudaSetDevice(p->device));
  cudaStream_t st = (cudaStream_t)stream;
  p->peer = nullptr;
  if (opt->peer_group) {
    CbPeerGroup* g = (CbPeerGroup*)opt->peer_group;
    if (!g->connected || g->device != p->device) { g_last_error = "peer group is not connected on this device"; return CB_E_INVALID; }
    if (g->cap < p->red_len()) {
      g_last_error = "peer group capacity " + std::to_string(g->cap) + " doubles < " + std::to_string(p->red_len());
      return CB_E_INVALID;
    }
    if (opt->rank != g->rank || opt->world_size != g->world) { g_last_error = "rank / world_size differ from the peer group's"; return CB_E_INVALID; }
    if (g->poisoned) {
      g_last_error = "peer group is unusable after a failed solve (the ranks' sequence numbers may differ): re-create it";
      return CB_E_INVALID;
    }
    p->peer = g;
  }
  if (sharded(opt) && p->order_auto && !p->order_identity) {
    g_last_error = "sharded solve on a problem whose camera order was chosen from this rank's observations only: pass "
                   "CbBaProblemDesc.cam_order (the same on every rank)";
    return CB_E_INVALID;
  }
  const int rc = p->P == 6 ? lm_solve<6>(p, opt, x_inout, result, st) : lm_solve<9>(p, opt, x_inout, result, st);
  p->peer = nullptr;
  return rc;
}

}
namespace {
template <int P, int MODE>
int eval_mode(CbBaProblem* p, const double* x, cudaStream_t st) {
  CB_TRY(upload_x(p, x, st));
  CB_TRY(run_cam_prep<P>(p, p->d_xc[0], p->d_camtab[0], st));
  launch_resjac<P, MODE>(p, nullptr, 0, 0, 1.0, p->d_out2, st);
  return CB_OK;
}
}
extern "C" {

int cb_ba_residuals(CbBaProblem* p, const double* x, double* r_out, void* stream) {
  if (!p || !x || !r_out) { g_last_error = "cb_ba_residuals: null argument"; return CB_E_INVALID; }
  CB_CUDA(cudaSetDevice(p->device));
  cudaStream_t st = (cudaStream_t)stream;
  CB_TRY(p->P == 6 ? (eval_mode<6, 2>(p, x, st)) : (eval_mode<9, 2>(p, x, st)));
  CB_CUDA(cudaMemcpyAsync(r_out, p->d_out2, sizeof(double) * 2 * (size_t)p->n_obs, cudaMemcpyDeviceToHost, st));
  CB_CUDA(cudaStreamSynchronize(st));
  return CB_OK;
}

int cb_ba_reproj_errors_px(CbBaProblem* p, const double* x, double* err_xy, void* stream) {
  if (!p || !x || !err_xy) { g_last_error = "cb_ba_reproj_errors_px: null argument"; return CB_E_INVALID; }
  CB_CUDA(cudaSetDevice(p->device));
  cudaStream_t st = (cudaStream_t)stream;
  CB_TRY(p->P == 6 ? (eval_mode<6, 3>(p, x, st)) : (eval_mode<9, 3>(p, x, st)));
  CB_CUDA(cudaMemcpyAsync(err_xy, p->d_out2, sizeof(double) * 2 * (size_t)p->n_obs, cudaMemcpyDeviceToHost, st));
  CB_CUDA(cudaStreamSynchronize(st));
  return CB_OK;
}

int cb_ba_jacobian_blocks(CbBaProblem* p, const double* x, double* Jc, double* Jp, void* stream) {
  if (!p || !x || !Jc || !Jp) { g_last_error = "cb_ba_jacobian_blocks: null argument"; return CB_E_INVALID; }
  CB_CUDA(cudaSetDevice(p->device));
  cudaStream_t st = (cudaStream_t)stream;
  const int n = p->n_obs;
  CB_TRY(upload_x(p, x, st));
  ScopedFree sf(st);
  double *dJc, *dJp;
  CB_TRY(sf.alloc(&dJc, 18 * (size_t)std::max(n, 1)));
  CB_TRY(sf.alloc(&dJp, 6 * (size_t)std::max(n, 1)));
  if (p->P == 6) {
    CB_TRY(run_cam_prep<6>(p, p->d_xc[0], p->d_camtab[0], st));
    if (n) CB_LAUNCH((cb::jac_blocks_kernel<6>), cdiv(n, 128), 128, 0, st, p->d_obs_cam, (const int*)p->d_cam_slot, p->d_obs_pt,
                     reinterpret_cast<const double2*>(p->d_obs_xy), n, (const double*)p->d_camtab[0], (const double*)p->d_xp4[0], dJc, dJp);
  } else {
    CB_TRY(run_cam_prep<9>(p, p->d_xc[0], p->d_camtab[0], st));
    if (n) CB_LAUNCH((cb::jac_blocks_kernel<9>), cdiv(n, 128), 128, 0, st, p->d_obs_cam, (const int*)p->d_cam_slot, p->d_obs_pt,
                     reinterpret_cast<const double2*>(p->d_obs_xy), n, (const double*)p->d_camtab[0], (const double*)p->d_xp4[0], dJc, dJp);
  }
  CB_CUDA(cudaMemcpyAsync(Jc, dJc, sizeof(double) * 18 * (size_t)n, cudaMemcpyDeviceToHost, st));
  CB_CUDA(cudaMemcpyAsync(Jp, dJp, sizeof(double) * 6 * (size_t)n, cudaMemcpyDeviceToHost, st));
  CB_CUDA(cudaStreamSynchronize(st));
  return CB_OK;
}

}
namespace {
template <int P>
int normal_eq_impl(CbBaProblem* p, const double* x, double lam, int loss, double fs, double* cost, double* U,
                          double* gc, double* V, double* gp, double* S, double* b, double* dc, double* dp,
                          cudaStream_t st) {
  using RT = cb::RowT<P>;
  CbBaOptions opt;
  cb_ba_default_options(&opt);
  opt.loss = loss; opt.f_scale = fs;
  opt.ftol = opt.xtol = opt.gtol = 0.0;
  CB_TRY(set_bounds(p, false, st));
  CB_TRY(init_state(p, &opt, lam, 1ll << 40, st));
  CB_TRY(upload_x(p, x, st));
  CB_TRY(run_cam_prep<P>(p, p->d_xc[0], p->d_camtab[0], st));
  CB_TRY(camera_pass<P>(p, 0, 0, st));
  CB_TRY(build_system<P>(p, &opt, st));
  CB_TRY(solve_step<P>(p, p->d_dp, st));
  const size_t nn = (size_t)p->nP * p->nP;
  std::vector<double> hS(nn + 3 * (size_t)p->nP + 1);
  CB_CUDA(cudaMemcpyAsync(hS.data(), p->d_red, sizeof(double) * hS.size(), cudaMemcpyDeviceToHost, st));
  std::vector<double> hU((size_t)p->n_cams * RT::NU), hV(6 * (size_t)std::max(p->n_pts, 1));
  CB_CUDA(cudaMemcpyAsync(hU.data(), p->d_Upk[0], sizeof(double) * hU.size(), cudaMemcpyDeviceToHost, st));
  CB_CUDA(cudaMemcpyAsync(hV.data(), p->d_V6, sizeof(double) * hV.size(), cudaMemcpyDeviceToHost, st));
  if (gc) CB_CUDA(cudaMemcpyAsync(gc, p->d_gc[0], sizeof(double) * p->nP, cudaMemcpyDeviceToHost, st));
  if (gp) CB_CUDA(cudaMemcpyAsync(gp, p->d_gp, sizeof(double) * 3 * (size_t)p->n_pts, cudaMemcpyDeviceToHost, st));
  if (dc) CB_CUDA(cudaMemcpyAsync(dc, p->d_dc, sizeof(double) * p->nP, cudaMemcpyDeviceToHost, st));
  if (dp) CB_CUDA(cudaMemcpyAsync(dp, p->d_dp, sizeof(double) * 3 * (size_t)p->n_pts, cudaMemcpyDeviceToHost, st));
  CB_CUDA(cudaStreamSynchronize(st));
  if (cost) *cost = hS[nn + 3 * (size_t)p->nP];
  const int nP = p->nP;
  if (S)
    for (int i = 0; i < nP; ++i)
      for (int j = 0; j < nP; ++j)
        S[((size_t)p->h_perm[i / P] * P + i % P) * nP + (size_t)p->h_perm[j / P] * P + j % P] = hS[(size_t)i * nP + j];
  if (b)
    for (int i = 0; i < nP; ++i) b[(size_t)p->h_perm[i / P] * P + i % P] = hS[nn + i];
  if (!p->order_identity) {
    std::vector<double> tmp(nP);
    for (double* v : {gc, dc})
      if (v) {
        std::memcpy(tmp.data(), v, sizeof(double) * nP);
        for (int i = 0; i < nP; ++i) v[(size_t)p->h_perm[i / P] * P + i % P] = tmp[i];
      }
  }
  if (U)
    for (int i = 0; i < p->n_cams; ++i) {
      const int c = p->h_perm[i];
      int u = 0;
      for (int a = 0; a < P; ++a)
        for (int bb = a; bb < P; ++bb, ++u) {
          U[((size_t)c * P + a) * P + bb] = hU[(size_t)i * RT::NU + u];
          U[((size_t)c * P + bb) * P + a] = hU[(size_t)i * RT::NU + u];
        }
    }
  if (V)
    for (int j = 0; j < p->n_pts; ++j) {
      const double* v = &hV[6 * (size_t)j];
      double* o = V + 9 * (size_t)j;
      o[0] = v[0]; o[1] = v[1]; o[2] = v[2]; o[3] = v[1]; o[4] = v[3]; o[5] = v[4]; o[6] = v[2]; o[7] = v[4]; o[8] = v[5];
    }
  return CB_OK;
}
}
extern "C" {

int cb_ba_normal_equations(CbBaProblem* p, const double* x, double lambda, int32_t loss, double f_scale, double* cost,
                           double* U, double* gc, double* V, double* gp, double* S, double* b, double* dc, double* dp,
                           void* stream) {
  if (!p || !x) { g_last_error = "cb_ba_normal_equations: null argument"; return CB_E_INVALID; }
  CB_CUDA(cudaSetDevice(p->device));
  cudaStream_t st = (cudaStream_t)stream;
  return p->P == 6 ? normal_eq_impl<6>(p, x, lambda, loss, f_scale, cost, U, gc, V, gp, S, b, dc, dp, st)
                   : normal_eq_impl<9>(p, x, lambda, loss, f_scale, cost, U, gc, V, gp, S, b, dc, dp, st);
}

}
namespace {
template <int P>
int covariance_impl(CbBaProblem* p, const double* x, int loss, double fs, int n_fixed, const int32_t* fixed, double vf,
                    double* cam_cov, double* pt_cov, double* s2_out, int64_t* dof_out, int32_t* pt_rank, cudaStream_t st) {
  const int nP = p->nP, nc = p->n_cams, npts = std::max(p->n_pts, 1);
  const size_t nn = (size_t)nP * nP;
  std::vector<int> cs(nc + 1);
  CB_CUDA(cudaMemcpyAsync(cs.data(), p->d_cam_start, sizeof(int) * (nc + 1), cudaMemcpyDeviceToHost, st));
  CB_CUDA(cudaStreamSynchronize(st));
  std::vector<char> is_fixed((size_t)p->ncp, 0);
  for (int i = 0; i < n_fixed; ++i) is_fixed[fixed[i]] = 1;
  std::vector<unsigned char> fr((size_t)nP, 0);
  std::vector<int> xidx((size_t)nP, -1);
  long long n_masked = 0, n_fix = 0;
  for (int i = 0; i < nc; ++i) {
    const int c = p->h_perm[i], w = p->h_cam_off[c + 1] - p->h_cam_off[c];
    const bool observed = cs[i + 1] > cs[i];
    for (int a = 0; a < w; ++a) {
      const int xi = p->h_cam_off[c] + a;
      xidx[(size_t)i * P + a] = xi;
      if (!observed) ++n_masked;
      else if (is_fixed[xi]) ++n_fix;
      else fr[(size_t)i * P + a] = 1;
    }
  }
  if (!p->d_covA) {
    const int n = (int)cdiv(nP, cb::CV_B) * cb::CV_B;
    CB_TRY(palloc(p, &p->d_covA, (size_t)n * n));
    CB_TRY(palloc(p, &p->d_covC, (size_t)n * cb::CV_B));
    CB_TRY(palloc(p, &p->d_covD, (size_t)cb::CV_B * cb::CV_B));
    CB_TRY(palloc(p, &p->d_covDiag, (size_t)n));
    CB_TRY(palloc(p, &p->d_covS, nn));
    CB_TRY(palloc(p, &p->d_covR, 9 * (size_t)npts));
    CB_TRY(palloc(p, &p->d_covPt, 9 * (size_t)npts));
    CB_TRY(palloc(p, &p->d_covRank, (size_t)npts));
    CB_TRY(palloc(p, &p->d_covFail, 2));
    CB_TRY(palloc(p, &p->d_covFree, (size_t)nP));
    p->cov_n = n;
  }
  const int n = p->cov_n;
  CbBaOptions opt;
  cb_ba_default_options(&opt);
  opt.loss = loss; opt.f_scale = fs;
  opt.ftol = opt.xtol = opt.gtol = 0.0;
  CB_CUDA(cudaEventRecord(p->ev0, st));
  CB_TRY(init_state(p, &opt, 0.0, 1ll << 40, st));
  CB_CUDA(cudaMemsetAsync(p->d_covRank, 0, sizeof(int) * npts, st));
  const int big[2] = {INT32_MAX, INT32_MAX};
  CB_CUDA(cudaMemcpyAsync(p->d_covFail, big, sizeof(big), cudaMemcpyHostToDevice, st));
  CB_CUDA(cudaMemcpyAsync(p->d_covFree, fr.data(), nP, cudaMemcpyHostToDevice, st));
  CB_TRY(upload_x(p, x, st));
  CB_TRY(run_cam_prep<P>(p, p->d_xc[0], p->d_camtab[0], st));
  CB_TRY(camera_pass<P>(p, 0, 0, st));
  CB_TRY(build_system<P>(p, &opt, st, nullptr, true));
  if (p->n_c) CB_LAUNCH(cb::comp_failed_kernel, cdiv(p->n_comp, 128), 128, 0, st, p->ct, (const double*)p->d_compL, p->d_covFail + 1);
  CB_CUDA(cudaEventRecord(p->ev1, st));
  CB_LAUNCH(cb::cov_prep_kernel, cdiv((long long)n * n, 256), 256, 0, st, (const double*)p->d_red, nP,
            (const unsigned char*)p->d_covFree, n, p->d_covA, p->d_covDiag);
  for (int kb = 0; kb < n; kb += cb::CV_B) {
    CB_LAUNCH(cb::cov_sweep_pivot_kernel, 1, cb::CV_B * cb::CV_B, 0, st, (const double*)p->d_covA, n, kb,
              (const double*)p->d_covDiag, CB_COV_PIVOT_RTOL, p->d_covD, p->d_covC, p->d_covFail);
    CB_LAUNCH(cb::cov_sweep_update_kernel, dim3(n / cb::CV_B, n / cb::CV_B), cb::CV_B * cb::CV_B, 0, st, p->d_covA, n, kb,
              (const double*)p->d_covD, (const double*)p->d_covC);
  }
  CB_LAUNCH(cb::cov_finish_kernel, cdiv((long long)nn, 256), 256, 0, st, (const double*)p->d_covA, n, nP,
            (const unsigned char*)p->d_covFree, p->d_covS);
  CB_CUDA(cudaEventRecord(p->ev2, st));
  double cost = 0.0;
  int fail[2];
  std::vector<int> rank((size_t)npts);
  CB_CUDA(cudaMemcpyAsync(&cost, p->d_red + nn + 3 * (size_t)nP, sizeof(double), cudaMemcpyDeviceToHost, st));
  CB_CUDA(cudaMemcpyAsync(fail, p->d_covFail, sizeof(fail), cudaMemcpyDeviceToHost, st));
  CB_CUDA(cudaMemcpyAsync(rank.data(), p->d_covRank, sizeof(int) * npts, cudaMemcpyDeviceToHost, st));
  CB_CUDA(cudaStreamSynchronize(st));
  char msg[256];
  if (fail[1] != INT32_MAX) {
    std::snprintf(msg, sizeof msg, "cb_ba_covariance: constraint component %d is not positive definite at lambda = 0", fail[1]);
    g_last_error = msg;
    return CB_E_INVALID;
  }
  if (fail[0] != INT32_MAX) {
    const int slot = fail[0] / P, a = fail[0] % P;
    std::snprintf(msg, sizeof msg,
                  "cb_ba_covariance: the gauge-fixed reduced camera system is singular: the pivot of camera %d parameter %d "
                  "(x index %d) collapsed below %.0e of its diagonal; fix more parameters (see default_gauge)",
                  p->h_perm[slot], a, xidx[fail[0]], CB_COV_PIVOT_RTOL);
    g_last_error = msg;
    return CB_E_INVALID;
  }
  long long null_pts = 0;
  for (int j = 0; j < p->n_pts; ++j)
    if (rank[j] >= 0) null_pts += 3 - rank[j];
  const long long m = 2ll * p->n_obs + p->n_c;
  const long long rk = (long long)p->n_params - n_fix - n_masked - null_pts;
  const long long dof = m - rk;
  const double s2 = vf > 0.0 ? vf : (dof > 0 ? 2.0 * cost / (double)dof : std::nan(""));
  if (s2_out) *s2_out = s2;
  if (dof_out) *dof_out = dof;
  if (pt_rank) std::memcpy(pt_rank, rank.data(), sizeof(int) * p->n_pts);
  if (pt_cov && p->n_pts > 0) {
    CB_LAUNCH((cb::cov_point_kernel<P>), 4 * p->num_sms, 256, 0, st, (const int*)p->d_pt_start, (const int*)p->d_pm_cam,
              p->n_pts, (const double*)p->d_Zt, (size_t)p->LD, (const double*)p->d_covS, nP, (const double*)p->d_covR,
              (const int*)p->d_covRank, s2, p->d_covPt);
  }
  CB_CUDA(cudaEventRecord(p->ev3, st));
  if (pt_cov && p->n_pts > 0)
    CB_CUDA(cudaMemcpyAsync(pt_cov, p->d_covPt, sizeof(double) * 9 * p->n_pts, cudaMemcpyDeviceToHost, st));
  std::vector<double> hS;
  if (cam_cov) {
    hS.resize(nn);
    CB_CUDA(cudaMemcpyAsync(hS.data(), p->d_covS, sizeof(double) * nn, cudaMemcpyDeviceToHost, st));
  }
  CB_CUDA(cudaStreamSynchronize(st));
  CB_CUDA(cudaEventElapsedTime(&p->cov_ms[0], p->ev0, p->ev1));
  CB_CUDA(cudaEventElapsedTime(&p->cov_ms[1], p->ev1, p->ev2));
  CB_CUDA(cudaEventElapsedTime(&p->cov_ms[2], p->ev2, p->ev3));
  if (cam_cov) {
    const size_t ncp = (size_t)p->ncp;
    std::vector<double> rowv(ncp);
    for (int i = 0; i < nc; ++i) {
      const bool observed = cs[i + 1] > cs[i];
      const int c = p->h_perm[i];
      for (int a = p->h_cam_off[c]; a < p->h_cam_off[c + 1]; ++a) rowv[a] = observed ? 0.0 : std::nan("");
    }
    for (size_t i = 0; i < ncp; ++i)
      for (size_t j = 0; j < ncp; ++j) cam_cov[i * ncp + j] = std::isnan(rowv[i]) ? rowv[i] : rowv[j];
    for (int i = 0; i < nP; ++i) {
      if (!fr[i]) continue;
      for (int j = 0; j < nP; ++j)
        if (fr[j]) cam_cov[(size_t)xidx[i] * ncp + xidx[j]] = s2 * hS[(size_t)i * nP + j];
    }
  }
  return CB_OK;
}
}
extern "C" {

int cb_ba_covariance(CbBaProblem* p, const double* x, int32_t loss, double f_scale, int32_t n_fixed, const int32_t* fixed,
                     double variance_factor, double* cam_cov, double* pt_cov, double* s2_out, int64_t* dof_out,
                     int32_t* pt_rank, void* stream) {
  if (!p || !x || (n_fixed > 0 && !fixed) || n_fixed < 0) { g_last_error = "cb_ba_covariance: null argument"; return CB_E_INVALID; }
  if (loss < CB_LOSS_LINEAR || loss > CB_LOSS_ARCTAN) { g_last_error = "cb_ba_covariance: unknown loss"; return CB_E_INVALID; }
  for (int i = 0; i < n_fixed; ++i)
    if (fixed[i] < 0 || fixed[i] >= p->ncp) {
      g_last_error = "cb_ba_covariance: fixed index " + std::to_string(fixed[i]) + " is outside the camera section of x";
      return CB_E_INVALID;
    }
  CB_CUDA(cudaSetDevice(p->device));
  cudaStream_t st = (cudaStream_t)stream;
  return p->P == 6 ? covariance_impl<6>(p, x, loss, f_scale, n_fixed, fixed, variance_factor, cam_cov, pt_cov, s2_out, dof_out, pt_rank, st)
                   : covariance_impl<9>(p, x, loss, f_scale, n_fixed, fixed, variance_factor, cam_cov, pt_cov, s2_out, dof_out, pt_rank, st);
}

int cb_ba_debug_pcg_time(CbBaProblem* p, int max_iter, int reps, double* ms_per_launch, void* stream) {
  if (!p || !ms_per_launch || reps <= 0) { g_last_error = "cb_ba_debug_pcg_time: bad argument"; return CB_E_INVALID; }
  if (p->direct_solve) { g_last_error = "cb_ba_debug_pcg_time: this problem is solved directly, not by PCG"; return CB_E_UNSUPPORTED; }
  CB_CUDA(cudaSetDevice(p->device));
  cudaStream_t st = (cudaStream_t)stream;
  CB_TRY(launch_pcg(p, nullptr, 0.0, max_iter, st));
  CB_CUDA(cudaEventRecord(p->ev2, st));
  for (int r = 0; r < reps; ++r) CB_TRY(launch_pcg(p, nullptr, 0.0, max_iter, st));
  CB_CUDA(cudaEventRecord(p->ev3, st));
  CB_CUDA(cudaEventSynchronize(p->ev3));
  float ms = 0.f;
  CB_CUDA(cudaEventElapsedTime(&ms, p->ev2, p->ev3));
  *ms_per_launch = ms / reps;
  double t[cb::SC_COUNT];
  CB_CUDA(cudaMemcpy(t, p->d_sc, sizeof(t), cudaMemcpyDeviceToHost));
  std::fprintf(stderr, "[pcg profile] cycles/iteration on CTA 0 thread 0: A(update+precond) %.0f block-barrier %.0f B(matvec) %.0f cluster-barrier %.0f C(dots) %.0f\n",
               t[cb::SC_PCG_T0] / max_iter, t[cb::SC_PCG_T0 + 1] / max_iter, t[cb::SC_PCG_T0 + 2] / max_iter,
               t[cb::SC_PCG_T0 + 3] / max_iter, t[cb::SC_PCG_T0 + 4] / max_iter);
  return CB_OK;
}

}
namespace {
template <int NT>
__global__ void fp64_dmma_peak_kernel(double* out, int iters, double a0, double b0) {
  double c[NT][2];
#pragma unroll
  for (int i = 0; i < NT; ++i) { c[i][0] = threadIdx.x; c[i][1] = i; }
  double a = a0 + threadIdx.x * 1e-9, b = b0;
  for (int it = 0; it < iters; ++it) {
#pragma unroll
    for (int i = 0; i < NT; ++i) cb::dmma884(c[i][0], c[i][1], a, b);
  }
  double s = 0;
#pragma unroll
  for (int i = 0; i < NT; ++i) s += c[i][0] + c[i][1];
  out[blockIdx.x * blockDim.x + threadIdx.x] = s;
}
template <int NT>
__global__ void fp64_dmma16816_peak_kernel(double* out, int iters, double a0, double b0) {
  double c[NT][4], a[8], b[4];
#pragma unroll
  for (int i = 0; i < NT; ++i) { c[i][0] = threadIdx.x; c[i][1] = i; c[i][2] = 0.0; c[i][3] = 1.0; }
#pragma unroll
  for (int i = 0; i < 8; ++i) a[i] = a0 + threadIdx.x * 1e-9 + i * 1e-12;
#pragma unroll
  for (int j = 0; j < 4; ++j) b[j] = b0;
  for (int it = 0; it < iters; ++it) {
#pragma unroll
    for (int i = 0; i < NT; ++i) cb::dmma16816(c[i], a, b);
  }
// ... 392 lines not shown
  const int* d_cam = nullptr;
  const long long* d_key = nullptr;
  const double* d_xy = nullptr;
  CB_TRY(to_device(obs_cam, (size_t)n, obs_on_device, &d_cam, sf, st));
  CB_TRY(to_device((const long long*)obs_key, (size_t)n, obs_on_device, &d_key, sf, st));
  CB_TRY(validate_rows(d_cam, d_key, n, n_cams, who, sf, st));
  if (undist) {
    const cb::UndistCam* d_tab = nullptr;
    CB_TRY(upload_undist_table(*undist, sf, st, &d_tab));
    double* d_und = nullptr;
    CB_TRY(sf.alloc(&d_und, 2 * (size_t)n));
    if (obs_on_device) {
      CB_LAUNCH(cb::undistort_kernel<double>, G, TB, 0, st, d_tab, d_cam, obs_xy, d_und, (long long)n, 0);
    } else {
      const float* d_px = nullptr;
      CB_TRY(to_device_f32(obs_xy, 2 * (size_t)n, &d_px, sf, st));
      CB_LAUNCH(cb::undistort_kernel<float>, G, TB, 0, st, d_tab, d_cam, d_px, d_und, (long long)n, 0);
    }
    d_xy = d_und;
  } else {
    CB_TRY(to_device(obs_xy, 2 * (size_t)n, obs_on_device, &d_xy, sf, st));
  }

  int *v_out = nullptr, *d_start = nullptr, n_groups = 0;
  CB_TRY(group_by_key(d_key, n, st, sf, &v_out, &d_start, &n_groups));
  CB_CUDA(cudaEventRecord(ev, st));
  *n_groups_out = n_groups;
  if (n_groups > max_groups) {
    g_last_error = std::string(who) + ": " + std::to_string(n_groups) + " groups but room for " + std::to_string(max_groups);
    return CB_E_INVALID;
  }
  out->cam = d_cam;
  out->xy = d_xy;
  out->rows = v_out;
  out->start = d_start;
  out->n_groups = n_groups;
  return CB_OK;
}

int tri_lanes(int n, int n_groups) { return (n / std::max(n_groups, 1) > 96) ? 32 : 8; }

template <typename F>
void with_lanes(int lanes, F&& f) {
  if (lanes == 32) f(std::integral_constant<int, 32>{});
  else f(std::integral_constant<int, 8>{});
}

struct TriDlt {
  double* xyz = nullptr;
  int* count = nullptr;
  int* rep = nullptr;
  unsigned long long* sig = nullptr;
};

int tri_dlt_launch(int32_t n_cams, const double* d_proj, const ObsGroups& g, int lanes, cudaEvent_t ev_a,
                   cudaEvent_t ev_b, ScopedFree& sf, cudaStream_t st, TriDlt* t) {
  const int n_groups = g.n_groups;
  CB_TRY(sf.alloc(&t->xyz, 3 * (size_t)n_groups));
  CB_TRY(sf.alloc(&t->count, (size_t)n_groups));
  CB_TRY(sf.alloc(&t->rep, (size_t)n_groups));
  CB_TRY(sf.alloc(&t->sig, 2 * (size_t)n_groups));
  const size_t proj_bytes = sizeof(double) * 13 * (size_t)n_cams;
  const int in_smem = proj_bytes <= 40 * 1024 ? 1 : 0;
  const long long threads = (long long)n_groups * lanes;
  CB_CUDA(cudaEventRecord(ev_a, st));
  with_lanes(lanes, [&](auto L) {
    CB_LAUNCH(cb::tri_dlt_kernel<L.value>, cdiv(threads, cb::TRI_THREADS), cb::TRI_THREADS, in_smem ? proj_bytes : 0, st,
              d_proj, n_cams, in_smem, g.start, g.rows, g.cam, g.xy, n_groups, t->xyz, t->count, t->rep, t->sig);
  });
  CB_CUDA(cudaGetLastError());
  CB_CUDA(cudaEventRecord(ev_b, st));
  return CB_OK;
}

struct TriCams {
  std::vector<int> xoff;
  int ncp = 0;
  int P = 6;
  std::vector<double> proj;
  std::vector<cb::UndistCam> tab;
  double* camtab = nullptr;
};

int tri_cams_prepare(int32_t n_cams, const int32_t* cam_flags, const double* cam_const, const double* cam_x,
                     const char* who, TriCams* out) {
  std::vector<int>& xoff = out->xoff;
  xoff.assign(n_cams + 1, 0);
  bool any_free = false;
  for (int c = 0; c < n_cams; ++c) {
    if (cam_flags[c] < 0 || cam_flags[c] > 3) {
      g_last_error = std::string(who) + ": camera flags must be a combination of bits 0 and 1";
      return CB_E_INVALID;
    }
    any_free = any_free || (cam_flags[c] & 1);
    xoff[c + 1] = xoff[c] + ((cam_flags[c] & 1) ? 9 : 6);
  }
  out->ncp = xoff[n_cams];
  out->P = any_free ? 9 : 6;
  std::vector<double>& proj = out->proj;
  std::vector<cb::UndistCam>& tab = out->tab;
  proj.assign(12 * (size_t)n_cams, 0.0);
  tab.assign(n_cams, cb::UndistCam{});
  for (int c = 0; c < n_cams; ++c) {
    const double* q = cam_x + xoff[c];
    const double* k = cam_const + 9 * (size_t)c;
    const bool free_i = cam_flags[c] & 1;
    const double th = std::sqrt(q[0] * q[0] + q[1] * q[1] + q[2] * q[2]);
    double R[9];
    if (th < 1e-12) {
      const double r[9] = {1, -q[2], q[1], q[2], 1, -q[0], -q[1], q[0], 1};
      std::memcpy(R, r, sizeof(R));
    } else {
      const double kx = q[0] / th, ky = q[1] / th, kz = q[2] / th, s = std::sin(th), co = std::cos(th), c1 = 1.0 - co;
      const double r[9] = {co + c1 * kx * kx,      c1 * kx * ky - s * kz, c1 * kx * kz + s * ky,
                           c1 * ky * kx + s * kz, co + c1 * ky * ky,      c1 * ky * kz - s * kx,
                           c1 * kz * kx - s * ky, c1 * kz * ky + s * kx, co + c1 * kz * kz};
      std::memcpy(R, r, sizeof(R));
    }
    for (int i = 0; i < 3; ++i) {
      for (int j = 0; j < 3; ++j) proj[12 * (size_t)c + 4 * i + j] = R[3 * i + j];
      proj[12 * (size_t)c + 4 * i + 3] = q[3 + i];
    }
    const double sc = free_i ? q[6] : 1.0, k1 = free_i ? q[7] : k[4], k2 = free_i ? q[8] : k[5];
    cb::UndistCam& u = tab[c];
    std::memset(&u, 0, sizeof(u));
    u.fx = sc * k[0]; u.fy = sc * k[1]; u.cx = k[2]; u.cy = k[3]; u.skew = 0.0;
    u.fisheye = (cam_flags[c] & 2) ? 1 : 0;
    u.d[0] = k1; u.d[1] = k2; u.d[2] = k[6]; u.d[3] = k[7];
    if (!u.fisheye) u.d[4] = k[8];
    if (!(k[0] != 0.0) || !(u.fx != 0.0) || !(u.fy != 0.0)) {
      g_last_error = std::string(who) + ": zero focal length in the camera table";
      return CB_E_INVALID;
    }
  }
  return CB_OK;
}

int tri_cams_upload(int32_t n_cams, const int32_t* cam_flags, const double* cam_const, const double* cam_x,
                    TriCams* c, ScopedFree& sf, cudaStream_t st) {
  const int P = c->P, ncp = c->ncp;
  int *d_flags = nullptr, *d_xoff = nullptr;
  double *d_const = nullptr, *d_x = nullptr, *d_xc = nullptr, *d_camtab = nullptr;
  CB_TRY(sf.alloc(&d_flags, (size_t)n_cams));
  CB_TRY(sf.alloc(&d_xoff, (size_t)n_cams));
  CB_TRY(sf.alloc(&d_const, 9 * (size_t)n_cams));
  CB_TRY(sf.alloc(&d_x, (size_t)ncp));
  CB_TRY(sf.alloc(&d_xc, (size_t)P * n_cams));
  CB_TRY(sf.alloc(&d_camtab, (size_t)cb::CT_SIZE * n_cams));
  CB_CUDA(cudaMemcpyAsync(d_flags, cam_flags, sizeof(int) * n_cams, cudaMemcpyHostToDevice, st));
  CB_CUDA(cudaMemcpyAsync(d_xoff, c->xoff.data(), sizeof(int) * n_cams, cudaMemcpyHostToDevice, st));
  CB_CUDA(cudaMemcpyAsync(d_const, cam_const, sizeof(double) * 9 * n_cams, cudaMemcpyHostToDevice, st));
  CB_CUDA(cudaMemcpyAsync(d_x, cam_x, sizeof(double) * ncp, cudaMemcpyHostToDevice, st));
  CB_LAUNCH(cb::unpack_x_kernel, cdiv((long long)n_cams * P, 256), 256, 0, st, d_x, d_xoff, d_flags, d_const, n_cams, P,
            0, ncp, d_xc, nullptr);
  CB_LAUNCH(cb::cam_prep_kernel, cdiv(n_cams, 64), 64, 0, st, d_xc, d_flags, d_const, n_cams, P, d_camtab);
  c->camtab = d_camtab;
  return CB_OK;
}

size_t tri_camtab_smem(int32_t n_cams) {
  const size_t cam_bytes = sizeof(double) * cb::CT_SMEM * (size_t)n_cams;
  return cam_bytes <= 40 * 1024 ? cam_bytes : 0;
}

struct TriConsensusArgs {
  double threshold_px;
  int32_t min_inliers, max_pairs;
  int32_t* n_inliers_out;
  uint8_t* inlier_out;
};

struct Consensus {
  double* hyp = nullptr;
  int* cam = nullptr;
  int *count = nullptr, *rep = nullptr, *status = nullptr;
  int* nin = nullptr;
  unsigned char* flag = nullptr;
  unsigned char* inl = nullptr;
  int *rows = nullptr, *start = nullptr;
  int* n_rows = nullptr;
};

int consensus_alloc(int n_groups, int n, int hyp_width, bool with_cam, ScopedFree& sf, cudaStream_t st, Consensus* c) {
  CB_TRY(sf.alloc(&c->hyp, (size_t)hyp_width * n_groups));
  if (with_cam) CB_TRY(sf.alloc(&c->cam, (size_t)n_groups));
  CB_TRY(sf.alloc(&c->count, (size_t)n_groups));
  CB_TRY(sf.alloc(&c->rep, (size_t)n_groups));
  CB_TRY(sf.alloc(&c->nin, (size_t)n_groups + 1));
  CB_TRY(sf.alloc(&c->status, (size_t)n_groups));
  CB_TRY(sf.alloc(&c->flag, (size_t)n));
  CB_TRY(sf.alloc(&c->inl, (size_t)n));
  CB_TRY(sf.alloc(&c->rows, (size_t)n));
  CB_TRY(sf.alloc(&c->start, (size_t)n_groups + 1));
  CB_TRY(sf.alloc(&c->n_rows, 1));
  CB_CUDA(cudaMemsetAsync(c->nin + n_groups, 0, sizeof(int), st));
  return CB_OK;
}

int consensus_compact(int* rows, int n, int n_groups, ScopedFree& sf, cudaStream_t st, Consensus* c) {
  CB_CUB(sf, cub::DeviceSelect::Flagged, rows, c->flag, c->rows, c->n_rows, n, st);
  CB_CUB(sf, cub::DeviceScan::ExclusiveSum, c->nin, c->start, n_groups + 1, st);
  g_launches.fetch_add(4);
  return CB_OK;
}

int tri_consensus_launch(int32_t n_cams, const TriCams& cams, const double* d_proj, const ObsGroups& g, int lanes, int n,
                         const double* px, const TriConsensusArgs& a, cudaEvent_t ev_a, cudaEvent_t ev_b, ScopedFree& sf,
                         cudaStream_t st, Consensus* c) {
  const int n_groups = g.n_groups;
  CB_TRY(consensus_alloc(n_groups, n, 3, false, sf, st, c));

  const size_t cam_smem = tri_camtab_smem(n_cams);
  const size_t proj_bytes = sizeof(double) * 13 * (size_t)n_cams;
  const size_t proj_smem = proj_bytes <= 40 * 1024 ? proj_bytes : 0;
  const size_t smem = cam_smem + proj_smem;
  if (smem > 48 * 1024) {
    CB_CUDA(cudaFuncSetAttribute(cb::tri_consensus_kernel<8>, cudaFuncAttributeMaxDynamicSharedMemorySize, (int)smem));
    CB_CUDA(cudaFuncSetAttribute(cb::tri_consensus_kernel<32>, cudaFuncAttributeMaxDynamicSharedMemorySize, (int)smem));
  }
  const int blocks = cdiv((long long)n_groups * lanes, cb::TRI_THREADS);
  CB_CUDA(cudaEventRecord(ev_a, st));
  with_lanes(lanes, [&](auto L) {
    CB_LAUNCH(cb::tri_consensus_kernel<L.value>, blocks, cb::TRI_THREADS, smem, st, cams.camtab, cam_smem ? 1 : 0,
              d_proj, proj_smem ? 1 : 0, n_cams, g.start, g.rows, g.cam, g.xy, px, n_groups, a.threshold_px,
              a.min_inliers, a.max_pairs, c->hyp, c->count, c->rep, c->nin, c->status, c->flag, c->inl);
  });
  CB_CUDA(cudaGetLastError());
  CB_TRY(consensus_compact(g.rows, n, n_groups, sf, st, c));
  CB_CUDA(cudaEventRecord(ev_b, st));
  return CB_OK;
}

int tri_refine_launch(int32_t n_cams, const TriCams& c, int lanes, const int* start, const int* rows, const int* cam,
                      const double* px, int n_groups, const double* xyz0, int32_t max_iter, double xtol, double* xyz,
                      double* rmse, int* status, cudaStream_t st) {
  const size_t smem = tri_camtab_smem(n_cams);
  const int cam_in_smem = smem ? 1 : 0;
  const int blocks = cdiv((long long)n_groups * lanes, cb::TRI_THREADS);
  with_lanes(lanes, [&](auto L) {
    CB_LAUNCH(cb::tri_refine_kernel<L.value>, blocks, cb::TRI_THREADS, smem, st, c.camtab, n_cams, cam_in_smem, start,
              rows, cam, px, n_groups, xyz0, max_iter, xtol, xyz, rmse, status);
  });
  CB_CUDA(cudaGetLastError());
  return CB_OK;
}

int tri_cov_launch(int32_t n_cams, const TriCams& c, const double* cam_cov, double pixel_sigma, int lanes,
                   const int* start, const int* rows, const int* cam, const double* px, int n, int n_groups,
                   const double* xyz, const int* status, cudaEvent_t ev_a, cudaEvent_t ev_b, ScopedFree& sf,
                   cudaStream_t st, double** d_cov_out) {
  const int P = c.P, ncp = c.ncp;
  const std::vector<int>& xoff = c.xoff;
  double* d_sig = nullptr;
  double* d_B = nullptr;
  int* d_first = nullptr;
  if (cam_cov) {
    const size_t nP = (size_t)n_cams * P;
    std::vector<double> sig(nP * nP, 0.0);
    for (int a = 0; a < n_cams; ++a)
      for (int p = 0; p < xoff[a + 1] - xoff[a]; ++p)
        for (int d = 0; d < n_cams; ++d)
          for (int q = 0; q < xoff[d + 1] - xoff[d]; ++q)
            sig[((size_t)a * P + p) * nP + (size_t)d * P + q] = cam_cov[(size_t)(xoff[a] + p) * ncp + xoff[d] + q];
    CB_TRY(sf.alloc(&d_sig, nP * nP));
    CB_CUDA(cudaMemcpyAsync(d_sig, sig.data(), sizeof(double) * nP * nP, cudaMemcpyHostToDevice, st));
    CB_TRY(sf.alloc(&d_B, 3 * (size_t)P * n));
    CB_TRY(sf.alloc(&d_first, (size_t)n));
    CB_CUDA(cudaStreamSynchronize(st));
  }
  double* d_cov = nullptr;
  CB_TRY(sf.alloc(&d_cov, 9 * (size_t)n_groups));
  const double s2 = pixel_sigma * pixel_sigma;
  const size_t smem = tri_camtab_smem(n_cams);
  const int cam_in_smem = smem ? 1 : 0;
  const int blocks = cdiv((long long)n_groups * lanes, cb::TRI_THREADS);
  CB_CUDA(cudaEventRecord(ev_a, st));
  with_lanes(lanes, [&](auto L) {
    if (P == 9)
      CB_LAUNCH((cb::tri_cov_kernel<9, L.value>), blocks, cb::TRI_THREADS, smem, st, c.camtab, n_cams, cam_in_smem,
                start, rows, cam, px, n_groups, xyz, status, d_sig, s2, d_B, d_first, d_cov);
    else
      CB_LAUNCH((cb::tri_cov_kernel<6, L.value>), blocks, cb::TRI_THREADS, smem, st, c.camtab, n_cams, cam_in_smem,
                start, rows, cam, px, n_groups, xyz, status, d_sig, s2, d_B, d_first, d_cov);
  });
  CB_CUDA(cudaGetLastError());
  CB_CUDA(cudaEventRecord(ev_b, st));
  *d_cov_out = d_cov;
  return CB_OK;
}

int triangulate_impl(int32_t n_cams, const std::vector<cb::UndistCam>* undist, const double* proj, int64_t n_obs,
                     const int32_t* obs_cam, const int64_t* obs_key, const double* obs_xy, int obs_on_device,
                     int32_t max_groups, int32_t* n_groups_out, double* xyz_out, int32_t* count_out,
                     int32_t* rep_row_out, uint64_t* camset_sig_out, CbTriStats* stats, int device, void* stream) {
  if (n_cams <= 0 || !proj || n_obs < 0 || n_obs > 0x7fffffffLL || !n_groups_out || max_groups < 0 ||
      (n_obs > 0 && (!obs_cam || !obs_key || !obs_xy)) ||
      (max_groups > 0 && (!xyz_out || !count_out || !rep_row_out || !camset_sig_out))) {
    g_last_error = "cb_triangulate_dlt: bad argument";
    return CB_E_INVALID;
  }
  CB_TRY(select_device(device));
  *n_groups_out = 0;
  if (stats) std::memset(stats, 0, sizeof(*stats));
  if (n_obs == 0) return CB_OK;
  const long long launches0 = g_launches.load();
  const int n = (int)n_obs;
  cudaStream_t st = (cudaStream_t)stream;
// ... 966 lines not shown
```

caliscope_b200/csrc/cb_kernels.cuh:

```cuda
#pragma once
#include <cooperative_groups.h>

#include "cb_device.cuh"

namespace cb {
namespace cg = cooperative_groups;

constexpr int RJ_THREADS = 128;
constexpr int RJ_CHUNK = 2048;
constexpr int PT_WARPS = 8;
constexpr int SY_TILE = 96;
constexpr int SY_KC = 32;
constexpr int SY_STAGES = 4;
constexpr int SY_CONSUMER_WARPS = 8;
constexpr int SY_THREADS = 32 * (SY_CONSUMER_WARPS + 1);
constexpr int PCG_THREADS = 512;

template <int P>
struct RowT {
  static constexpr int NU = P * (P + 1) / 2;
  static constexpr int NACC = NU + P + 1;
};

enum {
  SC_COST = 0, SC_GNORM_C, SC_COST_NEW, SC_PRED_C, SC_STEP2_C, SC_X2_C, SC_PRED_P, SC_STEP2_P, SC_X2_P,
  SC_PCG_ITS, SC_PCG_REL, SC_PCG_FLAG, SC_GNORM_P, SC_PCG_T0 = 16, SC_COUNT = 24
};

__global__ void unpack_x_kernel(const double* __restrict__ x, const int* __restrict__ cam_xoff,
                                const int* __restrict__ cam_flags, const double* __restrict__ cam_const,
                                int n_cams, int P, int n_pts, int ncp, double* __restrict__ xc, double* __restrict__ xp4) {
  int i = blockIdx.x * blockDim.x + threadIdx.x;
  if (i < n_cams * P) {
    int c = i / P, p = i % P;
    int w = (cam_flags[c] & 1) ? 9 : 6;
    double v;
    if (p < w) v = x[cam_xoff[c] + p];
    else v = (p == 6) ? 1.0 : cam_const[c * 9 + 4 + (p - 7)];
    xc[i] = v;
  }
  if (i < n_pts) {
    xp4[4 * (size_t)i + 0] = x[ncp + 3 * (size_t)i + 0];
    xp4[4 * (size_t)i + 1] = x[ncp + 3 * (size_t)i + 1];
    xp4[4 * (size_t)i + 2] = x[ncp + 3 * (size_t)i + 2];
    xp4[4 * (size_t)i + 3] = 0.0;
  }
}

__global__ void pack_x_kernel(double* __restrict__ x, const int* __restrict__ cam_xoff, const int* __restrict__ cam_flags,
                              int n_cams, int P, int n_pts, int ncp, const double* __restrict__ xc,
                              const double* __restrict__ xp4) {
  int i = blockIdx.x * blockDim.x + threadIdx.x;
  if (i < n_cams * P) {
    int c = i / P, p = i % P;
    if (p < ((cam_flags[c] & 1) ? 9 : 6)) x[cam_xoff[c] + p] = xc[i];
  }
  if (i < n_pts) {
    x[ncp + 3 * (size_t)i + 0] = xp4[4 * (size_t)i + 0];
    x[ncp + 3 * (size_t)i + 1] = xp4[4 * (size_t)i + 1];
    x[ncp + 3 * (size_t)i + 2] = xp4[4 * (size_t)i + 2];
  }
}

struct LmState {
  double lam, nu, cost, gnorm, initial_cost;
  double ftol, xtol, gtol;
  long long nfev, njev, nit, max_nfev, pcg_total;
  unsigned long long epoch_big, epoch_small;
  double fscale, pcg_tol2;
  int cur, done, status, new_lin, err, bad_streak, n_log, log_cap;
  int loss, pcg_max_iter;
};
struct Ptr2 {
  double* p[2];
};
struct CPtr2 {
  const double* p[2];
};

__device__ __forceinline__ void cam_prep_rot(double r0, double r1, double r2, double* __restrict__ o) {
  const double th2 = r0 * r0 + r1 * r1 + r2 * r2, th = sqrt(th2);
  double R[9];
  double s = 0.0, co = 1.0;
  if (th >= 1e-12) sincos(th, &s, &co);
  if (th < 1e-12) {
    R[0] = 1; R[1] = -r2; R[2] = r1; R[3] = r2; R[4] = 1; R[5] = -r0; R[6] = -r1; R[7] = r0; R[8] = 1;
  } else {
    const double it = 1.0 / th, kx = r0 * it, ky = r1 * it, kz = r2 * it, c1 = 1.0 - co;
    R[0] = co + c1 * kx * kx;      R[1] = c1 * kx * ky - s * kz; R[2] = c1 * kx * kz + s * ky;
    R[3] = c1 * ky * kx + s * kz;  R[4] = co + c1 * ky * ky;     R[5] = c1 * ky * kz - s * kx;
    R[6] = c1 * kz * kx - s * ky;  R[7] = c1 * kz * ky + s * kx; R[8] = co + c1 * kz * kz;
  }
  double B, C;
  if (th < 1e-4) {
    B = 0.5 - th2 / 24.0 + th2 * th2 / 720.0;
    C = 1.0 / 6.0 - th2 / 120.0 + th2 * th2 / 5040.0;
  } else {
    B = (1.0 - co) / th2;
    C = (th - s) / (th2 * th);
  }
  const double K2[9] = {r0 * r0 - th2, r0 * r1, r0 * r2, r1 * r0, r1 * r1 - th2, r1 * r2, r2 * r0, r2 * r1, r2 * r2 - th2};
  const double Km[9] = {0, -r2, r1, r2, 0, -r0, -r1, r0, 0};
#pragma unroll
  for (int i = 0; i < 9; ++i) {
    o[CT_R + i] = R[i];
    o[CT_JR + i] = ((i % 4 == 0) ? 1.0 : 0.0) - B * Km[i] + C * K2[i];
  }
}

__device__ __forceinline__ void cam_prep_one(const double* __restrict__ q, const double* __restrict__ k, int flags,
                                             double* __restrict__ o) {
  const bool free_i = (flags & 1) != 0;
  cam_prep_rot(q[0], q[1], q[2], o);
  o[CT_T + 0] = q[3]; o[CT_T + 1] = q[4]; o[CT_T + 2] = q[5];
  double sc = 1.0, k1 = k[4], k2 = k[5];
  if (free_i) { sc = q[6]; k1 = q[7]; k2 = q[8]; }
  const double fx = sc * k[0], fy = sc * k[1];
  o[CT_FX] = fx; o[CT_FY] = fy; o[CT_CX] = k[2]; o[CT_CY] = k[3];
  o[CT_D + 0] = k1; o[CT_D + 1] = k2; o[CT_D + 2] = k[6]; o[CT_D + 3] = k[7]; o[CT_D + 4] = k[8];
  o[CT_IFX0] = 1.0 / k[0];
  o[CT_SX] = fx / k[0];
  o[CT_SY] = fy / k[0];
  o[CT_FYR] = k[1] / k[0];
  o[CT_FLAGS] = (double)flags;
  o[CT_FX0] = k[0];
}

__global__ void cam_prep_kernel(const double* __restrict__ xc, const int* __restrict__ cam_flags,
                                const double* __restrict__ cam_const, int n_cams, int P,
                                double* __restrict__ camtab) {
  int c = blockIdx.x * blockDim.x + threadIdx.x;
  if (c >= n_cams) return;
  cam_prep_one(xc + (size_t)c * P, cam_const + (size_t)c * 9, cam_flags[c], camtab + (size_t)c * CT_SIZE);
}

template <int P, int MODE>
__global__ void __launch_bounds__(RJ_THREADS, (MODE == 0 && P == 6) ? 3 : 1)
resjac_kernel(const LmState* __restrict__ st, int flip, const int* __restrict__ chunk_cam,
              const int* __restrict__ chunk_begin, const int* __restrict__ chunk_end,
              const double2* __restrict__ cm_xy, const int* __restrict__ cm_pt, const int* __restrict__ cm_orig,
              CPtr2 camtab2, CPtr2 xp2, int loss, double fscale, double* __restrict__ partial,
              double* __restrict__ out2) {
  using RT = RowT<P>;
  __shared__ double cam[CT_SIZE];
  __shared__ double red[(MODE == 0 ? RT::NACC : 1) * (RJ_THREADS / 32)];
  int sel = 0;
  if (st != nullptr) {
    if (st->done) return;
    sel = st->cur ^ flip;
    loss = st->loss;
    fscale = st->fscale;
  }
  const double* __restrict__ camtab = camtab2.p[sel];
  const double* __restrict__ xp4 = xp2.p[sel];
  const int chunk = blockIdx.x;
  const int c = chunk_cam[chunk];
  const int begin = chunk_begin[chunk], end = chunk_end[chunk];
  if (threadIdx.x < CT_SIZE) cam[threadIdx.x] = camtab[(size_t)c * CT_SIZE + threadIdx.x];
  __syncthreads();
  const int flags = (int)cam[CT_FLAGS];
  const bool fish = (flags & 2) != 0;

  double acc[(MODE == 0) ? RT::NACC : 1];
#pragma unroll
  for (int k = 0; k < ((MODE == 0) ? RT::NACC : 1); ++k) acc[k] = 0.0;

  int q = begin + threadIdx.x;
  double2 xy_a = make_double2(0.0, 0.0), xy_b = xy_a;
  int pt_a = 0, org_a = 0, pt_b = 0, org_b = 0;
  double Xn0 = 0.0, Xn1 = 0.0, Xn2 = 0.0, Xn3 = 0.0;
  auto load_idx = [&](int qq, double2& xy, int& pt, int& org) {
    if (qq < end) {
      xy = cm_xy[qq];
      pt = cm_pt[qq];
      if constexpr (MODE == 2 || MODE == 3) org = cm_orig[qq];
    }
  };
  load_idx(q, xy_a, pt_a, org_a);
  load_idx(q + RJ_THREADS, xy_b, pt_b, org_b);
  if (q < end) ld256nc(xp4 + 4 * (size_t)pt_a, Xn0, Xn1, Xn2, Xn3);
  for (; q < end; q += RJ_THREADS) {
    const double2 xy = xy_a;
    const int org = org_a;
    const double X0 = Xn0, X1 = Xn1, X2 = Xn2;
    (void)org;
    xy_a = xy_b; pt_a = pt_b; org_a = org_b;
    if (q + RJ_THREADS < end) ld256nc(xp4 + 4 * (size_t)pt_a, Xn0, Xn1, Xn2, Xn3);
    load_idx(q + 2 * RJ_THREADS, xy_b, pt_b, org_b);
    if constexpr (MODE == 0) {
      double f[2], JX[6], Jc[2 * P];
      acc[RT::NACC - 1] += obs_jac<P>(cam, X0, X1, X2, xy.x, xy.y, loss, fscale, f, JX, Jc);
      int u = 0;
#pragma unroll
      for (int a = 0; a < P; ++a)
#pragma unroll
        for (int b = a; b < P; ++b) {
          acc[u] = fma(Jc[a], Jc[b], fma(Jc[P + a], Jc[P + b], acc[u]));
          ++u;
        }
#pragma unroll
      for (int a = 0; a < P; ++a) acc[RT::NU + a] = fma(Jc[a], f[0], fma(Jc[P + a], f[1], acc[RT::NU + a]));
    } else {
      ProjOut o;
      project_obs<false>(cam, fish, X0, X1, X2, o);
      const double ex = o.u - xy.x, ey = o.v - xy.y;
      if constexpr (MODE == 3) {
        const size_t i = (size_t)org;
        out2[2 * i] = ex; out2[2 * i + 1] = ey;
      } else if constexpr (MODE == 4) {
        out2[q] = sqrt(__dadd_rn(__dmul_rn(ex, ex), __dmul_rn(ey, ey)));
      } else {
        const double f0 = ex * cam[CT_IFX0], f1 = ey * cam[CT_IFX0];
        if constexpr (MODE == 2) {
          const size_t i = (size_t)org;
          out2[2 * i] = f0; out2[2 * i + 1] = f1;
        } else {
          acc[0] += robust_cost_only(loss, fscale, f0) + robust_cost_only(loss, fscale, f1);
        }
      }
    }
  }
  if constexpr (MODE == 0 || MODE == 1) {
    constexpr int NA = (MODE == 0) ? RT::NACC : 1;
    const int lane = threadIdx.x & 31, wid = threadIdx.x >> 5;
#pragma unroll
    for (int k = 0; k < NA; ++k) {
      double v = warp_sum(acc[k]);
      if (lane == 0) red[wid * NA + k] = v;
    }
    __syncthreads();
    if (threadIdx.x < NA) {
// ... 913 lines not shown
```

caliscope_b200/problem.py:

```python
from __future__ import annotations

import ctypes as C
from dataclasses import dataclass

import numpy as np

from . import _lib as L


def _ptr(a: np.ndarray) -> int:
    return a.ctypes.data


def _check_device_obs(obs_cam, obs_pt, obs_xy, device: int) -> int:
    dtypes = {"obs_cam": ("torch.int32", "torch.int16"), "obs_pt": ("torch.int32",), "obs_xy": ("torch.float64",)}
    arrays = {"obs_cam": obs_cam, "obs_pt": obs_pt, "obs_xy": obs_xy}
    for name, a in arrays.items():
        dev = getattr(a, "device", None)
        if getattr(dev, "type", None) != "cuda" or dev.index != device:
            raise ValueError(f"{name} must be a CUDA tensor on cuda:{device}, got device {dev}")
        if str(getattr(a, "dtype", None)) not in dtypes[name]:
            raise ValueError(f"{name} must have dtype {' or '.join(dtypes[name])}, got {getattr(a, 'dtype', None)}")
        if not a.is_contiguous():
            raise ValueError(f"{name} must be contiguous")
# ... 163 lines not shown
    def residuals(self, x, stream: int = 0) -> np.ndarray:
        x = self._x(x)
        out = np.empty(2 * self.n_obs + self.n_constraints)
        L.check(self._lib.cb_ba_residuals(self._h, _ptr(x), _ptr(out), C.c_void_p(stream)), "residuals")
        if self.n_constraints:
            tail = out[2 * self.n_obs :]
            L.check(self._lib.cb_ba_constraint_rows(self._h, _ptr(x), _ptr(tail), None, C.c_void_p(stream)), "constraint_rows")
        return out

    def constraint_rows(self, x, stream: int = 0) -> tuple[np.ndarray, np.ndarray]:
        x = self._x(x)
        r = np.empty(self.n_constraints)
        d = np.empty((self.n_constraints, 3))
        L.check(self._lib.cb_ba_constraint_rows(self._h, _ptr(x), _ptr(r), _ptr(d), C.c_void_p(stream)), "constraint_rows")
        return r, d

    def jacobian_blocks(self, x, stream: int = 0) -> tuple[np.ndarray, np.ndarray]:
        x = self._x(x)
        Jc = np.empty((self.n_obs, 2, 9))
        Jp = np.empty((self.n_obs, 2, 3))
        L.check(
            self._lib.cb_ba_jacobian_blocks(self._h, _ptr(x), _ptr(Jc), _ptr(Jp), C.c_void_p(stream)), "jacobian_blocks"
        )
        return Jc, Jp

    def reproj_errors_px(self, x, stream: int = 0) -> np.ndarray:
        x = self._x(x)
        out = np.empty((self.n_obs, 2))
        L.check(self._lib.cb_ba_reproj_errors_px(self._h, _ptr(x), _ptr(out), C.c_void_p(stream)), "reproj_errors_px")
        return out

    def rmse_px(self, x, stream: int = 0) -> tuple[float, np.ndarray]:
        x = self._x(x)
        overall = C.c_double()
        per_cam = np.empty(self.n_cams)
        L.check(self._lib.cb_ba_rmse_px(self._h, _ptr(x), C.addressof(overall), _ptr(per_cam), C.c_void_p(stream)), "rmse_px")
        return overall.value, per_cam

    def overall_rmse_px(self, x) -> float:
        return self.rmse_px(x)[0]

    def cull(self, x, thresholds, min_per_camera: int = 10, want_mask: bool = True, stream: int = 0):
        x = self._x(x)
        thr = np.ascontiguousarray(thresholds, dtype=np.float64)
        if thr.shape != (self.n_cams,):
            raise ValueError(f"thresholds must have shape ({self.n_cams},)")
        if min_per_camera < 0:
            raise ValueError(f"min_per_camera must be >= 0 (0: thresholds only), got {min_per_camera}")
        mask = np.empty(self.n_obs, np.uint8) if want_mask else None
        h = C.c_void_p()
        n_kept = C.c_int64()
        L.check(
            self._lib.cb_ba_cull(self._h, _ptr(x), _ptr(thr), int(min_per_camera), C.byref(h), C.addressof(n_kept),
                                 _ptr(mask) if want_mask else None, C.c_void_p(stream)),
            "cull",
        )
        new = BAProblem.__new__(BAProblem)
        new._lib, new._h, new._keep = self._lib, h, ()
        new.cam_flags, new.cam_const = self.cam_flags, self.cam_const
        new.n_cams, new.n_pts, new.device, new.n_obs = self.n_cams, self.n_pts, self.device, int(n_kept.value)
        new.cam_offsets, new.n_camera_params, new.n_params = self.cam_offsets, self.n_camera_params, self.n_params
        new.cam_stride = self.cam_stride
        new.n_constraints = self.n_constraints
        if self.n_constraints:
            new.constraints = self.constraints
        return new, (mask.astype(bool) if want_mask else None)

    def normal_equations(self, x, lam: float, loss: str = "linear", f_scale: float = 1.0, stream: int = 0) -> dict:
        x = self._x(x)
        P, nc, npt = self.cam_stride, self.n_cams, self.n_pts
        nP = nc * P
        out = {
            "U": np.empty((nc, P, P)), "gc": np.empty((nc, P)), "V": np.empty((npt, 3, 3)), "gp": np.empty((npt, 3)),
            "S": np.empty((nP, nP)), "b": np.empty(nP), "dc": np.empty((nc, P)), "dp": np.empty((npt, 3)),
        }
        cost = C.c_double()
        L.check(
            self._lib.cb_ba_normal_equations(
                self._h, _ptr(x), float(lam), L.LOSS_IDS[loss], float(f_scale), C.addressof(cost),
                _ptr(out["U"]), _ptr(out["gc"]), _ptr(out["V"]), _ptr(out["gp"]), _ptr(out["S"]), _ptr(out["b"]),
                _ptr(out["dc"]), _ptr(out["dp"]), C.c_void_p(stream),
            ),
            "normal_equations",
        )
        out["cost"] = cost.value
        return out

    def covariance(self, x, *, loss: str = "linear", f_scale: float = 1.0, fixed=None, variance_factor=None,
                   points: bool = True, stream: int = 0) -> Covariance:
        from . import uncertainty

        if loss not in L.LOSS_IDS:
            raise ValueError(f"`loss` must be one of {list(L.LOSS_IDS)}")
        x = self._x(x)
        if fixed is None:
            observed = self.error_order_stats(x, 50.0, stream, want_err=False)[3] > 0
            fixed = uncertainty.default_gauge(x, self.cam_offsets, observed, self.n_constraints > 0)
        fixed = np.ascontiguousarray(fixed, dtype=np.int32).ravel()
        cam = np.empty((self.n_camera_params, self.n_camera_params))
        pts = np.empty((self.n_pts, 3, 3)) if points else None
        rank = np.empty(self.n_pts, np.int32)
        s2 = C.c_double()
        dof = C.c_int64()
        L.check(
            self._lib.cb_ba_covariance(
                self._h, _ptr(x), L.LOSS_IDS[loss], float(f_scale), len(fixed), _ptr(fixed) if len(fixed) else None,
                float(variance_factor) if variance_factor is not None else 0.0, _ptr(cam), _ptr(pts) if points else None,
                C.addressof(s2), C.addressof(dof), _ptr(rank), C.c_void_p(stream),
            ),
            "covariance",
        )
        return Covariance(cameras=cam, points=pts, point_rank=rank, variance_factor=s2.value, dof=int(dof.value),
                          fixed=fixed)

    def error_order_stats(self, x, q_percent: float, stream: int = 0, want_err: bool = True):
        x = self._x(x)
        err = np.empty(self.n_obs) if want_err else None
        lo = np.empty(self.n_cams)
        hi = np.empty(self.n_cams)
        cnt = np.empty(self.n_cams, np.int64)
        L.check(
            self._lib.cb_ba_error_order_stats(
                self._h, _ptr(x), float(q_percent), _ptr(err) if want_err else None, _ptr(lo), _ptr(hi), _ptr(cnt),
                C.c_void_p(stream)
            ),
            "error_order_stats",
        )
        return err, lo, hi, cnt

    def solve(
        self,
        x0,
        *,
        ftol: float = 1e-8,
        xtol: float = 1e-8,
        gtol: float = 1e-8,
        max_nfev: int | None = None,
        loss: str = "linear",
        f_scale: float = 1.0,
        verbose: int = 0,
        use_bounds: bool = True,
        lambda0: float = 1e-4,
        pcg_tol: float = 1e-6,
        allreduce=None,
        nccl_comm=None,
        peer_group=None,
        rank: int = 0,
        world_size: int = 1,
        stream: int = 0,
        time_kernels: bool = False,
    ) -> SolveResult:
        if loss not in L.LOSS_IDS:
            raise ValueError(f"`loss` must be one of {list(L.LOSS_IDS)}")
        x = self._x(x0).copy()
        opt = L.Options()
        self._lib.cb_ba_default_options(C.byref(opt))
        opt.ftol, opt.xtol, opt.gtol = float(ftol), float(xtol), float(gtol)
        opt.max_nfev = 0 if max_nfev is None else int(max_nfev)
        opt.loss = L.LOSS_IDS[loss]
        opt.f_scale = float(f_scale)
        opt.verbose = int(verbose)
        opt.use_bounds = 1 if use_bounds else 0
        opt.lambda0 = float(lambda0)
        opt.pcg_tol = float(pcg_tol)
        cb = None
        if allreduce is not None:
            cb = L.ALLREDUCE_FN(allreduce)
            opt.allreduce = cb
        if nccl_comm is not None:
            opt.nccl_comm = C.c_void_p(getattr(nccl_comm, "handle", nccl_comm))
        if peer_group is not None:
            opt.peer_group = C.c_void_p(getattr(peer_group, "handle", peer_group))
        opt.rank, opt.world_size = int(rank), int(world_size)
        opt.time_kernels = 1 if time_kernels else 0
        res = L.Result()
        try:
            L.check(self._lib.cb_ba_solve(self._h, C.byref(opt), _ptr(x), C.byref(res), C.c_void_p(stream)), "solve")
        except Exception:
            if peer_group is not None and hasattr(peer_group, "poisoned"):
                peer_group.poisoned = True
            raise
        del cb
        return SolveResult(
            x=x, status=res.status, nfev=res.nfev, njev=res.njev, nit=res.nit, cost=res.cost,
            initial_cost=res.initial_cost, optimality=res.optimality, lambda_final=res.lambda_final,
            pcg_iterations=res.pcg_iterations, kernel_launches=res.kernel_launches, solve_ms=res.solve_ms,
            rj_ms=res.rj_ms, rj_launches=res.rj_launches, syrk_ms=res.syrk_ms, syrk_launches=res.syrk_launches,
            trials_queued=res.trials_queued, used_graph=bool(res.used_graph), used_graph_mode=int(res.used_graph),
        )
```

include/caliscope_b200.h:

```cpp
#ifndef CALISCOPE_B200_H
#define CALISCOPE_B200_H

#include <stdint.h>

#ifdef __cplusplus
extern "C" {
#endif

#define CB_BA_ABI_VERSION 3

#define CB_CAM_FREE_INTRINSICS 1
#define CB_CAM_FISHEYE 2

#define CB_LOSS_LINEAR 0
#define CB_LOSS_SOFT_L1 1
#define CB_LOSS_HUBER 2
#define CB_LOSS_CAUCHY 3
#define CB_LOSS_ARCTAN 4

#define CB_OK 0
#define CB_E_INVALID (-1)
#define CB_E_CUDA (-2)
#define CB_E_NO_DEVICE (-3)
#define CB_E_UNSUPPORTED (-4)
#define CB_E_CALLBACK (-5)
#define CB_E_NOMEM (-6)

typedef struct CbBaProblem CbBaProblem;

typedef struct {
  int32_t n_cams;
  int32_t n_pts;
  int64_t n_obs;
  const int32_t* cam_flags;
  const double* cam_const;
  const int32_t* obs_cam;
  const int32_t* obs_pt;
  const double* obs_xy;
  int32_t obs_on_device;
  int32_t obs_cam_bits;
  const int32_t* cam_order;
  int64_t n_constraints;
  const int32_t* groups_a;
  const int32_t* groups_b;
  const double* distances;
  const double* weights;
} CbBaProblemDesc;

typedef int (*CbAllReduceSum)(void* user, double* device_buf, int64_t n, void* stream);

typedef struct {
  double ftol;
  double xtol;
  double gtol;
  int64_t max_nfev;
  int32_t loss;
  double f_scale;
  int32_t verbose;
  int32_t use_bounds;
  double lambda0;
  double pcg_tol;
  int32_t pcg_max_iter;
  CbAllReduceSum allreduce;
  void* allreduce_user;
  void* nccl_comm;
  void* peer_group;
  int32_t rank;
  int32_t world_size;
  int32_t time_kernels;
  int32_t pad_;
} CbBaOptions;

typedef struct {
  int32_t status;
  int64_t nfev;
  int64_t njev;
  int64_t nit;
  double cost;
  double initial_cost;
  double optimality;
  double lambda_final;
  int64_t pcg_iterations;
  int64_t kernel_launches;
  double solve_ms;
  double rj_ms;
  int64_t rj_launches;
  double syrk_ms;
  int64_t syrk_launches;
  int64_t trials_queued;
  int32_t used_graph;
  int32_t pad_;
} CbBaResult;

int cb_ba_abi_version(void);
const char* cb_ba_error_string(int code);
const char* cb_ba_last_error(void);
void cb_ba_default_options(CbBaOptions* opt);

int cb_ba_problem_create(const CbBaProblemDesc* desc, int device, void* stream, CbBaProblem** out);
int cb_ba_problem_destroy(CbBaProblem* p);
int64_t cb_ba_problem_n_params(const CbBaProblem* p);
double cb_ba_problem_stat(const CbBaProblem* p, int what);

int cb_ba_constraint_rows(CbBaProblem* p, const double* x, double* r_out, double* dir_out, void* stream);

int cb_ba_solve(CbBaProblem* p, const CbBaOptions* opt, double* x_inout, CbBaResult* result, void* stream);

int cb_ba_residuals(CbBaProblem* p, const double* x, double* r_out, void* stream);

int cb_ba_jacobian_blocks(CbBaProblem* p, const double* x, double* Jc, double* Jp, void* stream);

int cb_ba_reproj_errors_px(CbBaProblem* p, const double* x, double* err_xy, void* stream);

int cb_ba_cam_stride(const CbBaProblem* p);
int cb_ba_normal_equations(CbBaProblem* p, const double* x, double lambda, int32_t loss, double f_scale,
                           double* cost, double* U, double* gc, double* V, double* gp, double* S, double* b,
                           double* dc, double* dp, void* stream);

#define CB_COV_PIVOT_RTOL 1e-10
int cb_ba_covariance(CbBaProblem* p, const double* x, int32_t loss, double f_scale, int32_t n_fixed, const int32_t* fixed,
                     double variance_factor, double* cam_cov, double* pt_cov, double* s2_out, int64_t* dof_out,
                     int32_t* pt_rank, void* stream);

int cb_ba_error_order_stats(CbBaProblem* p, const double* x, double q_percent, double* err, double* lo,
                            double* hi, int64_t* count, void* stream);

int cb_ba_rmse_px(CbBaProblem* p, const double* x, double* overall, double* per_camera, void* stream);

int cb_ba_cull(CbBaProblem* p, const double* x, const double* thresholds, int32_t min_per_camera, CbBaProblem** out,
               int64_t* n_kept, uint8_t* keep_mask, void* stream);

int cb_ba_debug_pcg_time(CbBaProblem* p, int max_iter, int reps, double* ms_per_launch, void* stream);

int cb_debug_fp64_peak(int device, double* dmma_tflops, double* dfma_tflops);


int cb_undistort_points(int32_t n_cams, const int32_t* cam_fisheye, const double* cam_k, const double* cam_dist,
                        int64_t n, const int32_t* obs_cam, const double* xy_in, int on_device, int to_pixels,
                        double* xy_out, int device, void* stream);

typedef struct CbTriStats {
  double group_ms;
  double dlt_ms;
  double total_ms;
  int32_t kernel_launches;
  int32_t pad_;
} CbTriStats;

int cb_triangulate_dlt(int32_t n_cams, const double* proj, int64_t n_obs, const int32_t* obs_cam,
                       const int64_t* obs_key, const double* obs_xy, int obs_on_device, int32_t max_groups,
                       int32_t* n_groups_out, double* xyz_out, int32_t* count_out, int32_t* rep_row_out,
                       uint64_t* camset_sig_out, CbTriStats* stats, int device, void* stream);

int cb_undistort_triangulate(int32_t n_cams, const int32_t* cam_fisheye, const double* cam_k, const double* cam_dist,
                             const double* proj, int64_t n_obs, const int32_t* obs_cam, const int64_t* obs_key,
                             const double* obs_px, int obs_on_device, int32_t max_groups, int32_t* n_groups_out,
                             double* xyz_out, int32_t* count_out, int32_t* rep_row_out, uint64_t* camset_sig_out,
                             CbTriStats* stats, int device, void* stream);

typedef struct CbTriRefineStats {
  double group_ms;
  double dlt_ms;
  double refine_ms;
  double cov_ms;
  double total_ms;
  int32_t kernel_launches;
  int32_t pad_;
} CbTriRefineStats;

int cb_triangulate_refine(int32_t n_cams, const int32_t* cam_flags, const double* cam_const, const double* cam_x,
                          const double* cam_cov, int64_t n_obs, const int32_t* obs_cam, const int64_t* obs_key,
                          const double* obs_px, int obs_on_device, double pixel_sigma, int32_t max_iter, double xtol,
                          int32_t max_groups, int32_t* n_groups_out, double* xyz_out, double* cov_out,
                          double* rmse_px_out, int32_t* count_out, int32_t* rep_row_out, int32_t* status_out,
                          CbTriRefineStats* stats, int device, void* stream);

typedef struct CbTriRobustStats {
  double group_ms;
  double consensus_ms;
  double refine_ms;
  double cov_ms;
  double total_ms;
  int32_t kernel_launches;
  int32_t pad_;
} CbTriRobustStats;

int cb_triangulate_robust(int32_t n_cams, const int32_t* cam_flags, const double* cam_const, const double* cam_x,
                          const double* cam_cov, int64_t n_obs, const int32_t* obs_cam, const int64_t* obs_key,
                          const double* obs_px, int obs_on_device, double threshold_px, int32_t min_inliers,
                          int32_t max_pairs, double pixel_sigma, int32_t max_iter, double xtol, int32_t max_groups,
                          int32_t* n_groups_out, double* xyz_out, double* cov_out, double* rmse_px_out,
                          int32_t* count_out, int32_t* n_inliers_out, int32_t* rep_row_out, int32_t* status_out,
                          uint8_t* inlier_out, CbTriRobustStats* stats, int device, void* stream);

typedef struct CbResectStats {
  double group_ms;
  double consensus_ms;
  double refine_ms;
  double cov_ms;
  double total_ms;
  int32_t kernel_launches;
  int32_t pad_;
} CbResectStats;

int cb_resect_robust(int32_t n_cams, const int32_t* cam_flags, const double* cam_const, const double* cam_x,
                     int32_t n_pts, const double* pts_xyz, const double* pts_cov, int64_t n_obs, const int32_t* obs_cam,
                     const int64_t* obs_key, const int32_t* obs_pt, const double* obs_px, int obs_on_device,
                     double threshold_px, int32_t min_inliers, int32_t max_samples, int32_t use_prior,
                     double pixel_sigma, int32_t max_iter, double xtol, int32_t max_groups, int32_t* n_groups_out,
                     int32_t* cam_out, double* pose_out, double* cov_out, double* rmse_px_out, int32_t* count_out,
                     int32_t* n_inliers_out, int32_t* rep_row_out, int32_t* status_out, uint8_t* inlier_out,
                     CbResectStats* stats, int device, void* stream);

int cb_nccl_unique_id(char id_out[128]);
int cb_nccl_comm_create(const char id[128], int rank, int world_size, int device, void** comm_out);
int cb_nccl_comm_destroy(void* comm);

typedef struct CbPeerGroup CbPeerGroup;
int cb_peer_create(int rank, int world_size, int device, int64_t capacity_doubles, CbPeerGroup** out,
                   char handle_out[64]);
int cb_peer_connect(CbPeerGroup* group, const char* handles );
int cb_peer_destroy(CbPeerGroup* group);

int64_t cb_ba_launch_count(void);


int cb_pnp_ippe(int32_t n_cams, const int32_t* cam_fisheye, const double* cam_k, const double* cam_dist, int64_t n_obs,
                const int32_t* obs_cam, const int64_t* obs_key, const double* obs_px, const double* obs_obj,
                int32_t min_points, int32_t max_groups, int32_t* n_groups_out, double* R_out, double* t_out,
                double* rmse_out, int32_t* status_out, int32_t* count_out, int32_t* rep_row_out, CbTriStats* stats,
                int device, void* stream);

int cb_stereo_rmse(int32_t n_cams, const int32_t* cam_fisheye, const double* cam_k, const double* cam_dist,
                   int32_t n_pairs, const int32_t* pair_a, const int32_t* pair_b, const double* pair_Rt, int64_t n_obs,
                   const int32_t* obs_cam, const int64_t* obs_key, const double* obs_px, int32_t min_common,
                   double* rmse_out, int64_t* count_out, CbTriStats* stats, int device, void* stream);

int cb_relative_pose_network(int32_t n_groups, int32_t n_frames, const int32_t* frame_start, const int32_t* cam_id,
                             const int32_t* cam_pos, const double* R, const double* t, double rot_mult, double tr_mult,
                             int32_t max_pairs, int32_t* n_pairs_out, int32_t* pair_a, int32_t* pair_b, double* R_out,
                             double* t_out, int64_t* count_out, int64_t n_rel, uint8_t* rel_valid, uint8_t* rel_keep,
                             CbTriStats* stats, int device, void* stream);


int cb_shard_select(int64_t n_obs, const int32_t* obs_cam, const int32_t* obs_pt, const double* obs_xy, int32_t pt_lo,
                    int32_t pt_hi, int64_t capacity, int64_t* n_sel_out, int64_t* sel_index, int32_t* cam_out,
                    int32_t* pt_out, double* xy_out, int32_t n_threads);

int cb_csv_write_numeric(const char* path, const char* header, int64_t n_rows, int32_t n_cols, const int32_t* col_kind,
                         const void* const* col_data, int32_t n_threads);
int cb_csv_scan(const char* path, int64_t* n_rows, int32_t* n_cols);
int cb_csv_parse_numeric(const char* path, int64_t n_rows, int32_t n_cols, double* out, int32_t* col_all_int,
                         int32_t* col_has_empty, int32_t n_threads);

#ifdef __cplusplus
}
#endif
#endif
```

Before: 819.9.

## Trim solve prologue/epilogue host syncs, staging copies and memsets

```diff
diff --git a/caliscope_b200/_lib.py b/caliscope_b200/_lib.py
--- a/caliscope_b200/_lib.py
+++ b/caliscope_b200/_lib.py
@@ -152,6 +152,7 @@
     "cb_ba_problem_stat": (C.c_double, [_P, C.c_int]),
     "cb_ba_constraint_rows": (C.c_int, [_P, _P, _P, _P, _P]),
     "cb_ba_solve": (C.c_int, [_P, C.POINTER(Options), _P, C.POINTER(Result), _P]),
+    "cb_ba_solve_from": (C.c_int, [_P, C.POINTER(Options), _P, _P, C.POINTER(Result), _P]),
     "cb_ba_residuals": (C.c_int, [_P, _P, _P, _P]),
     "cb_ba_jacobian_blocks": (C.c_int, [_P, _P, _P, _P, _P]),
     "cb_ba_reproj_errors_px": (C.c_int, [_P, _P, _P, _P]),
diff --git a/caliscope_b200/csrc/cb_engine.cu b/caliscope_b200/csrc/cb_engine.cu
--- a/caliscope_b200/csrc/cb_engine.cu
+++ b/caliscope_b200/csrc/cb_engine.cu
@@ -490,6 +490,7 @@
   CUtensorMap zt_map{};
   unsigned char* d_active = nullptr;
   double *d_lo = nullptr, *d_hi = nullptr;
+  int bounds_for = -1;
   double *d_x = nullptr, *d_xc[2] = {nullptr, nullptr}, *d_xp4[2] = {nullptr, nullptr};
   double *d_camtab[2] = {nullptr, nullptr}, *d_Upk[2] = {nullptr, nullptr}, *d_gc[2] = {nullptr, nullptr},
          *d_costsum[2] = {nullptr, nullptr};
@@ -503,7 +504,6 @@
   cb::LmState* h_state = nullptr;
   cb::LmLogRow* d_log = nullptr;
   int log_cap = 4096;
-  double* h_x = nullptr;
   cudaEvent_t ev0 = nullptr, ev1 = nullptr, ev2 = nullptr, ev3 = nullptr, ev_state[2] = {nullptr, nullptr};
   cudaEvent_t ev_pp[2][4] = {{nullptr, nullptr, nullptr, nullptr}, {nullptr, nullptr, nullptr, nullptr}};
   cudaStream_t cap_stream = nullptr;
@@ -528,6 +528,7 @@
   int *d_covRank = nullptr, *d_covFail = nullptr;
   unsigned char* d_covFree = nullptr;
   float cov_ms[3] = {0.f, 0.f, 0.f};
+  double solve_host_us[4] = {0.0, 0.0, 0.0, 0.0};
   size_t red_len() const { return (size_t)nP * nP + 3 * (size_t)nP + 1 + red_slots; }
   cb::CPtr2 c_camtab() const { return {{d_camtab[0], d_camtab[1]}}; }
   cb::Ptr2 m_camtab() const { return {{d_camtab[0], d_camtab[1]}}; }
@@ -921,26 +922,25 @@
   return CB_OK;
 }
 
-int upload_x(CbBaProblem* p, const double* x, cudaStream_t st) {
-  stream_copy(p->h_x, x, sizeof(double) * p->n_params);
-  CB_CUDA(cudaMemcpyAsync(p->d_x, p->h_x, sizeof(double) * p->n_params, cudaMemcpyHostToDevice, st));
-  const int n = std::max(p->n_cams * p->P, p->n_pts);
-  CB_LAUNCH(cb::unpack_x_kernel, cdiv(std::max(n, 1), 256), 256, 0, st, p->d_x, p->d_cam_xoff, p->d_cam_flags,
-            p->d_cam_const, p->n_cams, p->P, p->n_pts, p->ncp, p->d_xc[0], p->d_xp4[0]);
-  return CB_OK;
-}
-
-int download_x(CbBaProblem* p, int cur, double* x, cudaStream_t st) {
+int upload_x(CbBaProblem* p, const double* x, cudaStream_t st, bool fresh = false) {
+  CB_CUDA(cudaMemcpyAsync(p->d_x, x, sizeof(double) * p->n_params, cudaMemcpyHostToDevice, st));
+  const int n = std::max(std::max(p->n_cams * p->P, p->n_pts), fresh ? (int)cb::SC_COUNT : 1);
+  const cb::FreshState z = fresh ? cb::FreshState{p->d_gmax, p->d_counter, p->d_sc, p->d_Dc2, p->d_Dp2} : cb::FreshState{};
+  CB_LAUNCH(cb::unpack_x_kernel, cdiv(n, 256), 256, 0, st, p->d_x, p->d_cam_xoff, p->d_cam_flags, p->d_cam_const,
+            p->n_cams, p->P, p->n_pts, p->ncp, p->d_xc[0], p->d_xp4[0], z);
+  return CB_OK;
+}
+
+int download_x(CbBaProblem* p, double* x, cudaStream_t st) {
   const int n = std::max(p->n_cams * p->P, p->n_pts);
   CB_LAUNCH(cb::pack_x_kernel, cdiv(std::max(n, 1), 256), 256, 0, st, p->d_x, p->d_cam_xoff, p->d_cam_flags, p->n_cams,
-            p->P, p->n_pts, p->ncp, p->d_xc[cur], p->d_xp4[cur]);
-  CB_CUDA(cudaMemcpyAsync(p->h_x, p->d_x, sizeof(double) * p->n_params, cudaMemcpyDeviceToHost, st));
-  CB_CUDA(cudaStreamSynchronize(st));
-  std::memcpy(x, p->h_x, sizeof(double) * p->n_params);
+            p->P, p->n_pts, p->ncp, (const cb::LmState*)p->d_state, cb::CPtr2{{p->d_xc[0], p->d_xc[1]}}, p->c_xp());
+  CB_CUDA(cudaMemcpyAsync(x, p->d_x, sizeof(double) * p->n_params, cudaMemcpyDeviceToHost, st));
   return CB_OK;
 }
 
 int set_bounds(CbBaProblem* p, bool use_bounds, cudaStream_t st) {
+  if (p->bounds_for == (use_bounds ? 1 : 0)) return CB_OK;
   std::vector<double> lo((size_t)p->nP, -1e300), hi((size_t)p->nP, 1e300);
   if (use_bounds && p->P == 9) {
     for (int c = 0; c < p->n_cams; ++c)
@@ -952,7 +952,7 @@
   }
   CB_CUDA(cudaMemcpyAsync(p->d_lo, lo.data(), sizeof(double) * p->nP, cudaMemcpyHostToDevice, st));
   CB_CUDA(cudaMemcpyAsync(p->d_hi, hi.data(), sizeof(double) * p->nP, cudaMemcpyHostToDevice, st));
-  CB_CUDA(cudaStreamSynchronize(st));
+  p->bounds_for = use_bounds ? 1 : 0;
   return CB_OK;
 }
 
@@ -974,11 +974,6 @@
     h.epoch_big = g->epoch_big; h.epoch_small = g->epoch_small;
   }
   CB_CUDA(cudaMemcpyAsync(p->d_state, &h, sizeof(h), cudaMemcpyHostToDevice, st));
-  CB_CUDA(cudaMemsetAsync(p->d_gmax, 0, 2 * sizeof(unsigned long long), st));
-  CB_CUDA(cudaMemsetAsync(p->d_counter, 0, 4 * sizeof(unsigned int), st));
-  CB_CUDA(cudaMemsetAsync(p->d_sc, 0, sizeof(double) * cb::SC_COUNT, st));
-  CB_CUDA(cudaMemsetAsync(p->d_Dc2, 0, sizeof(double) * p->nP, st));
-  CB_CUDA(cudaMemsetAsync(p->d_Dp2, 0, sizeof(double) * 3 * (size_t)std::max(p->n_pts, 1), st));
   return CB_OK;
 }
 
@@ -1031,7 +1026,7 @@
 }
 
 template <int P>
-int lm_solve(CbBaProblem* p, const CbBaOptions* opt, double* x_inout, CbBaResult* res, cudaStream_t st) {
+int lm_solve(CbBaProblem* p, const CbBaOptions* opt, const double* x0, double* x_out, CbBaResult* res, cudaStream_t st) {
   NvtxRange nvtx_solve("cb_ba_solve");
   const long long max_nfev = opt->max_nfev > 0 ? opt->max_nfev : 100ll * p->n_params;
   const bool verbose = opt->verbose >= 2 && opt->rank == 0;
@@ -1044,9 +1039,18 @@
   bool use_graph = !direct && !use_loop;
   if (use_graph && ensure_graph<P>(p, opt, false) != CB_OK) { cudaGetLastError(); use_graph = false; }
 
+  auto t_mark = std::chrono::steady_clock::now();
+  auto host_span = [&](int i) {
+    const auto now = std::chrono::steady_clock::now();
+    p->solve_host_us[i] = std::chrono::duration<double, std::micro>(now - t_mark).count();
+    t_mark = now;
+  };
   CB_TRY(set_bounds(p, opt->use_bounds != 0, st));
+  host_span(0);
   CB_TRY(init_state(p, opt, opt->lambda0 > 0 ? opt->lambda0 : 1e-4, max_nfev, st));
-  CB_TRY(upload_x(p, x_inout, st));
+  host_span(1);
+  CB_TRY(upload_x(p, x0, st, true));
+  host_span(2);
   CB_CUDA(cudaEventRecord(p->ev0, st));
   CB_TRY(run_cam_prep<P>(p, p->d_xc[0], p->d_camtab[0], st));
   CB_TRY(camera_pass<P>(p, 0, 0, st));
@@ -1100,7 +1104,12 @@
     }
     ++t;
   }
+  if (rc == CB_OK) {
+    cudaEventRecord(p->ev1, st);
+    rc = download_x(p, x_out, st);
+  }
   cudaError_t e = cudaStreamSynchronize(st);
+  host_span(3);
   if (rc == CB_OK && e != cudaSuccess) { g_last_error = std::string("LM solve: ") + cudaGetErrorString(e); rc = CB_E_CUDA; }
   if (rc != CB_OK) { if (p->peer) p->peer->poisoned = true; return rc; }
   const cb::LmState fin = p->h_state[(t - 1) & 1];
@@ -1130,8 +1139,6 @@
                    (long long)rows[i].nfev, rows[i].cost, rows[i].cost_new, rows[i].ratio, rows[i].lam, rows[i].step,
                    rows[i].gnorm, (int)rows[i].pcg);
   }
-  CB_CUDA(cudaEventRecord(p->ev1, st));
-  CB_TRY(download_x(p, fin.cur, x_inout, st));
   float ms = 0.f;
   CB_CUDA(cudaEventElapsedTime(&ms, p->ev0, p->ev1));
   res->status = fin.status;
@@ -1392,7 +1399,6 @@
   if (p->cap_stream) cudaStreamDestroy(p->cap_stream);
   for (void* a : p->allocs) cached_free(a);
   cached_free_host(p->h_state);
-  cached_free_host(p->h_x);
   for (cudaEvent_t e : {p->ev0, p->ev1, p->ev2, p->ev3, p->ev_state[0], p->ev_state[1], p->ev_pp[0][0], p->ev_pp[0][1],
                         p->ev_pp[0][2], p->ev_pp[0][3], p->ev_pp[1][0], p->ev_pp[1][1], p->ev_pp[1][2], p->ev_pp[1][3]})
     if (e) cudaEventDestroy(e);
@@ -1417,6 +1423,7 @@
     case 11: return (double)p->pcg_cs;
     case 12: return p->pcg_mode == 2 ? (double)p->pcg_cl : 0.0;
     case 13: return p->order_identity ? 0.0 : 1.0;
+    case 14: case 15: case 16: case 17: return p->solve_host_us[what - 14];
     default: return -1.0;
   }
 }
@@ -1884,7 +1891,6 @@
   CB_CUDA(cudaMemsetAsync(p->d_red2, 0, sizeof(double) * 8, st));
   CB_CUDA(cudaMemsetAsync(p->d_Linv6, 0, sizeof(double) * 6 * npts, st));
   CB_TRY(cached_malloc_host((void**)&p->h_state, sizeof(cb::LmState) * 4));
-  CB_TRY(cached_malloc_host((void**)&p->h_x, sizeof(double) * ((size_t)p->n_params + 1)));
   for (cudaEvent_t* e : {&p->ev0, &p->ev1, &p->ev2, &p->ev3, &p->ev_pp[0][0], &p->ev_pp[0][1], &p->ev_pp[0][2], &p->ev_pp[0][3],
                          &p->ev_pp[1][0], &p->ev_pp[1][1], &p->ev_pp[1][2], &p->ev_pp[1][3]})
     CB_CUDA(cudaEventCreate(e));
@@ -1956,7 +1962,12 @@
 }
 
 int cb_ba_solve(CbBaProblem* p, const CbBaOptions* opt, double* x_inout, CbBaResult* result, void* stream) {
-  if (!p || !opt || !x_inout || !result) { g_last_error = "cb_ba_solve: null argument"; return CB_E_INVALID; }
+  return cb_ba_solve_from(p, opt, x_inout, x_inout, result, stream);
+}
+
+int cb_ba_solve_from(CbBaProblem* p, const CbBaOptions* opt, const double* x0, double* x_out, CbBaResult* result,
+                     void* stream) {
+  if (!p || !opt || !x0 || !x_out || !result) { g_last_error = "cb_ba_solve: null argument"; return CB_E_INVALID; }
   if (opt->loss < 0 || opt->loss > CB_LOSS_ARCTAN) { g_last_error = "unknown loss id"; return CB_E_INVALID; }
   CB_CUDA(cudaSetDevice(p->device));
   cudaStream_t st = (cudaStream_t)stream;
@@ -1980,7 +1991,7 @@
                    "CbBaProblemDesc.cam_order (the same on every rank)";
     return CB_E_INVALID;
   }
-  const int rc = p->P == 6 ? lm_solve<6>(p, opt, x_inout, result, st) : lm_solve<9>(p, opt, x_inout, result, st);
+  const int rc = p->P == 6 ? lm_solve<6>(p, opt, x0, x_out, result, st) : lm_solve<9>(p, opt, x0, x_out, result, st);
   p->peer = nullptr;
   return rc;
 }
@@ -2055,7 +2066,7 @@
   opt.ftol = opt.xtol = opt.gtol = 0.0;
   CB_TRY(set_bounds(p, false, st));
   CB_TRY(init_state(p, &opt, lam, 1ll << 40, st));
-  CB_TRY(upload_x(p, x, st));
+  CB_TRY(upload_x(p, x, st, true));
   CB_TRY(run_cam_prep<P>(p, p->d_xc[0], p->d_camtab[0], st));
   CB_TRY(camera_pass<P>(p, 0, 0, st));
   CB_TRY(build_system<P>(p, &opt, st));
@@ -2169,7 +2180,7 @@
   const int big[2] = {INT32_MAX, INT32_MAX};
   CB_CUDA(cudaMemcpyAsync(p->d_covFail, big, sizeof(big), cudaMemcpyHostToDevice, st));
   CB_CUDA(cudaMemcpyAsync(p->d_covFree, fr.data(), nP, cudaMemcpyHostToDevice, st));
-  CB_TRY(upload_x(p, x, st));
+  CB_TRY(upload_x(p, x, st, true));
   CB_TRY(run_cam_prep<P>(p, p->d_xc[0], p->d_camtab[0], st));
   CB_TRY(camera_pass<P>(p, 0, 0, st));
   CB_TRY(build_system<P>(p, &opt, st, nullptr, true));
@@ -2868,7 +2879,7 @@
   CB_CUDA(cudaMemcpyAsync(d_const, cam_const, sizeof(double) * 9 * n_cams, cudaMemcpyHostToDevice, st));
   CB_CUDA(cudaMemcpyAsync(d_x, cam_x, sizeof(double) * ncp, cudaMemcpyHostToDevice, st));
   CB_LAUNCH(cb::unpack_x_kernel, cdiv((long long)n_cams * P, 256), 256, 0, st, d_x, d_xoff, d_flags, d_const, n_cams, P,
-            0, ncp, d_xc, nullptr);
+            0, ncp, d_xc, nullptr, cb::FreshState{});
   CB_LAUNCH(cb::cam_prep_kernel, cdiv(n_cams, 64), 64, 0, st, d_xc, d_flags, d_const, n_cams, P, d_camtab);
   c->camtab = d_camtab;
   return CB_OK;
diff --git a/caliscope_b200/csrc/cb_kernels.cuh b/caliscope_b200/csrc/cb_kernels.cuh
--- a/caliscope_b200/csrc/cb_kernels.cuh
+++ b/caliscope_b200/csrc/cb_kernels.cuh
@@ -27,10 +27,24 @@
   SC_PCG_ITS, SC_PCG_REL, SC_PCG_FLAG, SC_GNORM_P, SC_PCG_T0 = 16, SC_COUNT = 24
 };
 
+struct FreshState {
+  unsigned long long* gmax;
+  unsigned int* counter;
+  double *sc, *Dc2, *Dp2;
+};
+
 __global__ void unpack_x_kernel(const double* __restrict__ x, const int* __restrict__ cam_xoff,
                                 const int* __restrict__ cam_flags, const double* __restrict__ cam_const,
-                                int n_cams, int P, int n_pts, int ncp, double* __restrict__ xc, double* __restrict__ xp4) {
+                                int n_cams, int P, int n_pts, int ncp, double* __restrict__ xc, double* __restrict__ xp4,
+                                FreshState z) {
   int i = blockIdx.x * blockDim.x + threadIdx.x;
+  if (z.Dp2 != nullptr) {
+    if (i < 2) z.gmax[i] = 0ull;
+    if (i < 4) z.counter[i] = 0u;
+    if (i < SC_COUNT) z.sc[i] = 0.0;
+    if (i < n_cams * P) z.Dc2[i] = 0.0;
+    if (i < n_pts) { z.Dp2[3 * (size_t)i] = 0.0; z.Dp2[3 * (size_t)i + 1] = 0.0; z.Dp2[3 * (size_t)i + 2] = 0.0; }
+  }
   if (i < n_cams * P) {
     int c = i / P, p = i % P;
     int w = (cam_flags[c] & 1) ? 9 : 6;
@@ -44,21 +58,6 @@
     xp4[4 * (size_t)i + 1] = x[ncp + 3 * (size_t)i + 1];
     xp4[4 * (size_t)i + 2] = x[ncp + 3 * (size_t)i + 2];
     xp4[4 * (size_t)i + 3] = 0.0;
-  }
-}
-
-__global__ void pack_x_kernel(double* __restrict__ x, const int* __restrict__ cam_xoff, const int* __restrict__ cam_flags,
-                              int n_cams, int P, int n_pts, int ncp, const double* __restrict__ xc,
-                              const double* __restrict__ xp4) {
-  int i = blockIdx.x * blockDim.x + threadIdx.x;
-  if (i < n_cams * P) {
-    int c = i / P, p = i % P;
-    if (p < ((cam_flags[c] & 1) ? 9 : 6)) x[cam_xoff[c] + p] = xc[i];
-  }
-  if (i < n_pts) {
-    x[ncp + 3 * (size_t)i + 0] = xp4[4 * (size_t)i + 0];
-    x[ncp + 3 * (size_t)i + 1] = xp4[4 * (size_t)i + 1];
-    x[ncp + 3 * (size_t)i + 2] = xp4[4 * (size_t)i + 2];
   }
 }
 
@@ -77,6 +76,23 @@
 struct CPtr2 {
   const double* p[2];
 };
+
+__global__ void pack_x_kernel(double* __restrict__ x, const int* __restrict__ cam_xoff, const int* __restrict__ cam_flags,
+                              int n_cams, int P, int n_pts, int ncp, const LmState* __restrict__ st, CPtr2 xc2, CPtr2 xp2) {
+  const bool sel = st->cur != 0;
+  const double* __restrict__ xc = sel ? xc2.p[1] : xc2.p[0];
+  const double* __restrict__ xp4 = sel ? xp2.p[1] : xp2.p[0];
+  int i = blockIdx.x * blockDim.x + threadIdx.x;
+  if (i < n_cams * P) {
+    int c = i / P, p = i % P;
+    if (p < ((cam_flags[c] & 1) ? 9 : 6)) x[cam_xoff[c] + p] = xc[i];
+  }
+  if (i < n_pts) {
+    x[ncp + 3 * (size_t)i + 0] = xp4[4 * (size_t)i + 0];
+    x[ncp + 3 * (size_t)i + 1] = xp4[4 * (size_t)i + 1];
+    x[ncp + 3 * (size_t)i + 2] = xp4[4 * (size_t)i + 2];
+  }
+}
 
 __device__ __forceinline__ void cam_prep_rot(double r0, double r1, double r2, double* __restrict__ o) {
   const double th2 = r0 * r0 + r1 * r1 + r2 * r2, th = sqrt(th2);
diff --git a/caliscope_b200/problem.py b/caliscope_b200/problem.py
--- a/caliscope_b200/problem.py
+++ b/caliscope_b200/problem.py
@@ -339,7 +339,8 @@
     ) -> SolveResult:
         if loss not in L.LOSS_IDS:
             raise ValueError(f"`loss` must be one of {list(L.LOSS_IDS)}")
-        x = self._x(x0).copy()
+        x0 = self._x(x0)
+        x = np.empty_like(x0)
         opt = L.Options()
         self._lib.cb_ba_default_options(C.byref(opt))
         opt.ftol, opt.xtol, opt.gtol = float(ftol), float(xtol), float(gtol)
@@ -362,7 +363,8 @@
         opt.time_kernels = 1 if time_kernels else 0
         res = L.Result()
         try:
-            L.check(self._lib.cb_ba_solve(self._h, C.byref(opt), _ptr(x), C.byref(res), C.c_void_p(stream)), "solve")
+            L.check(self._lib.cb_ba_solve_from(self._h, C.byref(opt), _ptr(x0), _ptr(x), C.byref(res), C.c_void_p(stream)),
+                    "solve")
         except Exception:
             if peer_group is not None and hasattr(peer_group, "poisoned"):
                 peer_group.poisoned = True
diff --git a/include/caliscope_b200.h b/include/caliscope_b200.h
--- a/include/caliscope_b200.h
+++ b/include/caliscope_b200.h
@@ -105,6 +105,8 @@
 int cb_ba_constraint_rows(CbBaProblem* p, const double* x, double* r_out, double* dir_out, void* stream);
 
 int cb_ba_solve(CbBaProblem* p, const CbBaOptions* opt, double* x_inout, CbBaResult* result, void* stream);
+int cb_ba_solve_from(CbBaProblem* p, const CbBaOptions* opt, const double* x0, double* x_out, CbBaResult* result,
+                     void* stream);
 
 int cb_ba_residuals(CbBaProblem* p, const double* x, double* r_out, void* stream);
 
diff --git a/profiles/solve_tail.py b/profiles/solve_tail.py
--- /dev/null
+++ b/profiles/solve_tail.py
@@ -0,0 +1,136 @@
+import argparse
+import json
+import os
+import re
+import subprocess
+import sys
+import tempfile
+import time
+from collections import defaultdict
+from pathlib import Path
+
+import numpy as np
+
+sys.path.insert(0, str(Path(__file__).resolve().parent.parent))
+import caliscope_b200 as cb
+import bench
+
+HOST_SPANS = ("set_bounds", "init_state", "upload_x", "loop_and_download_until_sync")
+
+
+def card() -> str:
+    try:
+        out = subprocess.run(["nvidia-smi", "--query-gpu=name,power.limit,clocks.max.sm", "--format=csv,noheader"],
+                             capture_output=True, text=True, timeout=30).stdout.strip().splitlines()
+        return out[0] if out else "unknown card"
+    except (OSError, subprocess.SubprocessError):
+        return "unknown card"
+
+
+def short(name: str) -> str:
+    name = re.sub(r"^void\s+", "", name)
+    depth, cut = 0, len(name)
+    for i, ch in enumerate(name):
+        if ch == "<":
+            depth += 1
+        elif ch == ">":
+            depth -= 1
+        elif ch == "(" and depth == 0:
+            cut = i
+            break
+    return name[:cut].replace("cb::", "")
+
+
+def run(name: str, steps: int, warmup: int, trace_dir: str | None) -> dict:
+    import torch
+
+    rig = bench.make_workload(name)
+    n_c, n_p, n_o, refine = bench.WORKLOADS[name]
+    stream = torch.cuda.current_stream().cuda_stream
+    solve_kw = dict(ftol=1e-8, rank=0, world_size=1, stream=stream)
+    d_cam = torch.from_numpy(rig.obs_cam).cuda()
+    d_pt = torch.from_numpy(rig.obs_pt).cuda()
+    d_xy = torch.from_numpy(np.ascontiguousarray(rig.obs_xy)).cuda()
+    flush = None
+    if bench.needs_l2_flush(n_c, n_p, n_o, 9 if refine else 6, 1):
+        flush = torch.empty(bench.FLUSH_BYTES, dtype=torch.uint8, device="cuda")
+    out: dict = {"workload": name, "card": card(), "steps": steps, "l2_flush": flush is not None}
+    with cb.BAProblem(rig.cam_flags, rig.cam_const, rig.n_pts, d_cam, d_pt, d_xy, stream=stream) as prob:
+
+        def steps_run(k: int, host: np.ndarray | None = None):
+            ev = [(torch.cuda.Event(enable_timing=True), torch.cuda.Event(enable_timing=True)) for _ in range(k)]
+            res = None
+            for i in range(k):
+                if flush is not None:
+                    flush.fill_(i & 0x7F)
+                ev[i][0].record()
+                t0 = time.perf_counter()
+                res = prob.solve(rig.x0, **solve_kw)
+                t1 = time.perf_counter()
+                ev[i][1].record()
+                if host is not None:
+                    host += [prob.stat(14 + j) for j in range(len(HOST_SPANS))] + [1e6 * (t1 - t0)]
+            torch.cuda.synchronize()
+            return res, [a.elapsed_time(b) for a, b in ev]
+
+        steps_run(warmup)
+        host = np.zeros(len(HOST_SPANS) + 1)
+        res, ms = steps_run(steps, host)
+        host /= steps
+        l0 = cb._lib.load().cb_ba_launch_count()
+        steps_run(1)
+        launches = cb._lib.load().cb_ba_launch_count() - l0
+
+        acts = [torch.profiler.ProfilerActivity.CPU, torch.profiler.ProfilerActivity.CUDA]
+        with torch.profiler.profile(activities=acts) as prof:
+            steps_run(steps)
+        with tempfile.TemporaryDirectory() as tmp:
+            path = os.path.join(trace_dir or tmp, f"solve_tail_{name}.pt.trace.json")
+            if trace_dir:
+                os.makedirs(trace_dir, exist_ok=True)
+            prof.export_chrome_trace(path)
+            trace = json.loads(Path(path).read_text())
+
+    per = defaultdict(lambda: [0.0, 0])
+    for e in trace.get("traceEvents", []):
+        if e.get("ph") != "X" or e.get("cat") not in ("kernel", "gpu_memcpy", "gpu_memset"):
+            continue
+        n = short(e["name"]) if e["cat"] == "kernel" else e["name"]
+        if "at::native" in n:
+            continue
+        per[n][0] += float(e["dur"])
+        per[n][1] += 1
+    kernels = {n: {"us_per_solve": v[0] / steps, "launches_per_solve": v[1] / steps}
+               for n, v in sorted(per.items(), key=lambda kv: -kv[1][0])}
+    busy_ms = sum(v["us_per_solve"] for v in kernels.values()) / 1e3
+    big = sum(v["us_per_solve"] for n, v in kernels.items() if n.startswith(("pt_pass_kernel", "schur_syrk_kernel"))) / 1e3
+    step_ms = float(np.mean(ms))
+    out.update({
+        "nfev": int(res.nfev), "nit": int(res.nit), "status": int(res.status), "gpu_launches_per_solve": int(launches),
+        "step_ms": step_ms, "step_ms_min": float(np.min(ms)), "step_ms_max": float(np.max(ms)),
+        "device_busy_ms": busy_ms, "idle_ms": step_ms - busy_ms,
+        "point_pass_and_schur_ms": big, "tail_ms": step_ms - big,
+        "trials_per_solve": sum(v["launches_per_solve"] for n, v in kernels.items() if n.startswith("pt_pass_kernel")),
+        "host_us": dict(zip(HOST_SPANS + ("whole_solve_call",), map(float, host))),
+        "device_us_per_solve": kernels,
+    })
+    return out
+
+
+def main() -> None:
+    ap = argparse.ArgumentParser()
+    ap.add_argument("workloads", nargs="*", default=["cfg4", "cfg4_shard8"])
+    ap.add_argument("--steps", type=int, default=20)
+    ap.add_argument("--warmup", type=int, default=5)
+    ap.add_argument("--trace-dir", default=None, help="keep the chrome traces here (default: a temporary directory)")
+    args = ap.parse_args()
+    import torch
+
+    with torch.profiler.profile(activities=[torch.profiler.ProfilerActivity.CUDA]):
+        torch.zeros(1, device="cuda")
+    for name in args.workloads:
+        print(json.dumps(run(name, args.steps, args.warmup, args.trace_dir)), flush=True)
+
+
+if __name__ == "__main__":
+    main()
```

Measured after the change: 873.9, median of 6. 1.07x the previous value.
